# jerinphilip/whisper.tflite

Hardware: AMD Instinct MI355X
Metric: audio-sec/s (RTF) whisper-tiny 30s clips batch=32 at 1/2/4/8 MI355X (higher is better)
Workload: dtype f32 (operands as two fp16 planes, f16 MFMA, f32 accumulate); 1 GPU; whisper-tiny batch=32x30s synthetic mel U(-1,1.5), fp32, random-init weights (BASELINE.json configs[1]); mel resident in HBM -> token ids on host; clips_per_gpu=32, global_batch=32, decoder_positions=30, argmax_steps=27, parallelism=clip-parallel dp1, one RCCL all_gather of id records per 8 batches, pipelined=True, batches_in_flight=10, decoder=2 consecutive steps' batches share one decoder chain (dec_pair, dec_group), last_batches_announced=2, priming_batches=1

## Files before the change

include/wt_debug.h:

```cpp
#ifndef WT_DEBUG_H_
#define WT_DEBUG_H_
#include "wt_capi.h"
#ifdef __cplusplus
extern "C" {
#endif
int wt_dbg_gemm(wt_engine* h, int M, int N, int K, const float* A, const float* W, const float* bias,
                const float* R, const float* pos, int pos_period, int epi, float* C);
int wt_dbg_gemm_planes(wt_engine* h, int M, int N, int K, const float* A, const float* W, const float* bias,
                       const float* R, const float* pos, int pos_period, int epi, int planes_out, int iters, float* C,
                       float* avg_ms, int n_cu );
int wt_dbg_set_forced_ids(wt_engine* h, const int64_t* ids, int clips);
int wt_dbg_set_plane_gemm_mode(int mode);
int wt_dbg_gemm_planes_ln(wt_engine* h, int M, int K, const float* A, const float* W, const float* bias, const float* R,
                          const float* pos, int pos_period, int epi, const float* ln_g, const float* ln_b, int n_cu,
                          float* C, float* ln_out, float* ln_y32, int* fused);
int wt_dbg_encoder_attention_planes(wt_engine* h, int batch, int T, int heads, const float* qkv, int iters, float* out,
                                    float* avg_ms);
int wt_dbg_gemm_bench(wt_engine* h, int M, int N, int K, int epi, int variant, int iters, float* avg_ms);
int wt_dbg_interference(wt_engine* h, const float* d_mel, int batch, int n_enc, int chain_len, int blocks,
                        float* enc_ms, float* chain_ms);
int wt_dbg_concurrency(wt_engine* h, const float* d_mel, int batch, int n_dec, int n_enc, float* dec_ms,
                       float* enc_ms);
int wt_dbg_dec_gemm_bench(wt_engine* h, int kind, int B, int N, int K, int rows, int iters, float* avg_us);
int wt_dbg_dec_gemm(wt_engine* h, int mode, int B, int N, int K, const float* X, const float* W,
                    const float* bias, const float* R, float* Y, int64_t* argmax_out);
int wt_dbg_dec_ln_gemm(wt_engine* h, int B, int N, int K, const float* xin, const int64_t* ids, int pos,
                       const float* tok_emb, const float* pos_emb, int n_vocab, int n_pos,
                       const float* ln_g, const float* ln_b, const float* W, const float* bias,
                       int gelu, float* Y, float* xout);
int wt_dbg_layernorm(wt_engine* h, int M, int d, const float* x, const float* g, const float* b, float* y);
int wt_dbg_encoder_attention(wt_engine* h, int batch, int T, int heads, const float* qkv, float* out);
int wt_dbg_cross_attention(wt_engine* h, int batch, int heads, int T, int chunks, int nq, const float* x,
                           const float* ln_g, const float* ln_b, const float* wq, const float* bq, const float* kc,
                           const float* vc, float* out);
int wt_dbg_cross_absorbed(wt_engine* h, int batch, int heads, int T, int chunks, int nq, const float* qp, const float* E,
                          const float* wv, const float* bv, float* out, int iters, float* avg_us);
int wt_dbg_cross_absorbed_bf16(wt_engine* h, int batch, int heads, int T, int chunks, int nq, const float* qp, const float* E,
                               const float* wv, const float* bv, float* out, int iters, float* avg_us);
int wt_dbg_self_attention(wt_engine* h, int batch, int heads, int cap, int pos, int npos, const float* qkv,
                          float* kcache, float* vcache, float* out);
int wt_dbg_gemm_bf16(wt_engine* h, int M, int N, int K, const float* A, const float* W, const float* bias,
                     const float* R, const float* pos, int pos_period, int epi, int bf16_out, int iters, float* C,
                     float* avg_ms);
int wt_dbg_gemm_bf16_ln(wt_engine* h, int M, int N, int K, const float* A, const float* W, const float* bias, const float* R,
                        const float* ln_g, const float* ln_b, float* C, float* ln_out, float* ln_y32, int* fused);
int wt_dbg_encoder_attention_bf16(wt_engine* h, int batch, int T, int heads, const float* qkv, int iters, float* out,
                                  float* avg_ms);
int wt_dbg_dec_gemm_bf16(wt_engine* h, int mode, int B, int N, int K, const float* X, const float* W, const float* bias,
                         const float* R, float* Y, int64_t* argmax_out);
int wt_dbg_dec_ln_gemm_bf16(wt_engine* h, int B, int N, int K, const float* xin, const int64_t* ids, int pos,
                            const float* tok_emb, const float* pos_emb, int n_vocab, int n_pos, const float* ln_g,
                            const float* ln_b, const float* W, const float* bias, int gelu, float* Y, float* xout);
int wt_dbg_self_attention_bf16(wt_engine* h, int batch, int heads, int cap, int pos, int npos, const float* qkv,
                               float* kcache, float* vcache, float* out);
int wt_dbg_cross_attention_bf16(wt_engine* h, int batch, int heads, int T, int chunks, int nq, const float* x,
                                const float* ln_g, const float* ln_b, const float* wq, const float* bq, const float* kc,
                                const float* vc, float* out);
int wt_dbg_beam_topk(wt_engine* h, int rows, int V, int ldl, int kk, const float* logits, float* m, float* s,
                     uint64_t* keys);
int wt_dbg_beam_step(wt_engine* h, int K, int clips, int c0, int n_live, int pos, int n_prompt, int V, int64_t eot,
                     const float* logits, const int64_t* ids, float* live_sum, int32_t* fin_tok, float* fin_sum,
                     int32_t* fin_len, int32_t* n_fin, int32_t* done, int32_t* parent, int64_t* token, int64_t* ids_next);
int wt_dbg_beam_reorder(wt_engine* h, int src_rows, int dst_rows, int cap, int d, int slabs, int pos, int V,
                        const float* kv_src, float* kv_dst, const int64_t* ids_src, int64_t* ids_dst,
                        const int32_t* parent, const int64_t* token);
// ... 18 lines not shown
```

whisper.tflite_amd/__init__.py:

```python
from __future__ import annotations

import ctypes
import enum
import os
from ctypes import (POINTER, byref, c_char_p, c_float, c_int, c_int32, c_int64, c_long, c_size_t,
                    c_uint64, c_void_p)

import numpy as np

_HERE = os.path.dirname(os.path.abspath(__file__))
LIB_PATH = os.environ.get("WT_LIB_PATH") or os.path.join(_HERE, "lib", "libwhisper-tflite.so")

WT_OK = 0
WT_MAX_IDS = 32
WT_PIPELINE_DEPTH = 24
CHUNK_SAMPLES = 480000
STATUS_NAMES = {0: "WT_OK", 1: "WT_ERR_INVALID_ARG", 2: "WT_ERR_IO", 3: "WT_ERR_FORMAT",
                4: "WT_ERR_UNSUPPORTED", 5: "WT_ERR_DEVICE", 6: "WT_ERR_BUFFER"}

CAPI_SYMBOLS = [
    "wt_device_alloc", "wt_device_free", "wt_device_upload", "wt_device_download", "wt_device_synchronize",
    "wt_engine_create", "wt_engine_destroy", "wt_last_error", "wt_engine_dims",
    "wt_engine_set_option", "wt_engine_get_option", "wt_engine_set_prompt", "wt_transcribe_pcm", "wt_transcribe_long_pcm", "wt_transcribe_file",
    "wt_logmel_batch", "wt_logmel_batch_dev", "wt_encdec_tokens_batch",
    "wt_encdec_tokens_batch_dev", "wt_transcribe_tokens_batch_dev", "wt_pipeline_submit_dev", "wt_pipeline_submit_pcm_dev", "wt_pipeline_collect",
    "wt_encdec_debug_batch",
    "wt_last_timings", "wt_last_beam_scores", "wt_last_kernel_stats", "wt_decode_text", "wt_language_id", "wt_lang_code", "wt_wav_read_legacy",
    "wt_vocab_info", "wt_filters", "wt_write_synthetic_weights", "wt_write_synthetic_vocab",
    "wt_vocab_open", "wt_vocab_close", "wt_vocab_get_info", "wt_vocab_get_filters", "wt_vocab_size", "wt_vocab_token",
    "wt_vocab_decode", "wt_log_mel_spectrogram", "wt_convert_tflite", "wt_shutdown",
]
DEBUG_SYMBOLS = [
    "wt_dbg_cross_absorbed", "wt_dbg_cross_absorbed_bf16", "wt_dbg_gemm_planes_ln", "wt_dbg_gemm", "wt_dbg_gemm_bench", "wt_dbg_dec_gemm_bench", "wt_dbg_dec_gemm", "wt_dbg_dec_ln_gemm", "wt_dbg_layernorm", "wt_dbg_encoder_attention",
    "wt_dbg_cross_attention", "wt_dbg_self_attention", "wt_dbg_interference", "wt_dbg_concurrency",
    "wt_dbg_gemm_planes", "wt_dbg_set_plane_gemm_mode", "wt_dbg_set_forced_ids", "wt_dbg_dec_gemm_bf16", "wt_dbg_dec_ln_gemm_bf16",
    "wt_dbg_self_attention_bf16", "wt_dbg_cross_attention_bf16", "wt_dbg_encoder_attention_planes", "wt_dbg_gemm_bf16", "wt_dbg_gemm_bf16_ln", "wt_dbg_encoder_attention_bf16",
    "wt_dbg_beam_topk", "wt_dbg_beam_step", "wt_dbg_beam_reorder", "wt_dbg_beam_finalize",
    "wt_dbg_dec_gemm_ksplit", "wt_dbg_dec_ln_gemm_rows", "wt_dbg_dec_logits", "wt_dbg_select_token",
]


class WtError(RuntimeError):
    def __init__(self, code: int, message: str):
        super().__init__(f"{STATUS_NAMES.get(code, code)}: {message}")
        self.code = code


class EngineType(enum.IntEnum):
    Monolith = 0
    EncDec = 1


class Dims(ctypes.Structure):
    _fields_ = [(n, c_int32) for n in (
        "n_mels", "n_audio_ctx", "n_audio_state", "n_audio_head", "n_audio_layer",
        "n_vocab", "n_text_ctx", "n_text_state", "n_text_head", "n_text_layer")]


class Timings(ctypes.Structure):
    _fields_ = [("logmel_ms", c_float), ("encoder_ms", c_float), ("cross_kv_ms", c_float),
                ("decoder_ms", c_float), ("total_ms", c_float), ("batch", c_int32),
                ("decoder_steps", c_int32)]


class KernelStat(ctypes.Structure):
    _fields_ = [("name", ctypes.c_char * 48), ("launches", c_int32), ("reserved", c_int32),
                ("ms", ctypes.c_double), ("flops", ctypes.c_double), ("bytes", ctypes.c_double)]


_lib = None


def lib() -> ctypes.CDLL:
    global _lib
    if _lib is None:
        if not os.path.exists(LIB_PATH):
            raise ImportError(
                f"{LIB_PATH} is missing: build it with `make lib` (or __graft_entry__.build()); "
                "there is no Python/CPU fallback for the engine")
        L = ctypes.CDLL(LIB_PATH)
        fp, ip64, ip32 = POINTER(c_float), POINTER(c_int64), POINTER(c_int32)
        L.wt_engine_create.argtypes = [c_int, c_char_p, c_char_p, c_int, c_int, POINTER(c_void_p)]
        L.wt_engine_destroy.argtypes = [c_void_p]
        L.wt_engine_destroy.restype = None
        L.wt_last_error.argtypes = [c_void_p]
        L.wt_last_error.restype = c_char_p
        L.wt_engine_dims.argtypes = [c_void_p, POINTER(Dims)]
        L.wt_engine_set_option.argtypes = [c_void_p, c_char_p, c_long]
# ... 28 lines not shown
        L.wt_vocab_close.restype = None
        L.wt_vocab_get_info.argtypes = [c_void_p, ip32]
        L.wt_vocab_get_filters.argtypes = [c_void_p, fp, c_size_t, ip32, ip32]
        L.wt_vocab_size.argtypes = [c_void_p]
        L.wt_vocab_token.argtypes = [c_void_p, c_int, c_char_p, c_size_t, POINTER(c_size_t)]
        L.wt_vocab_decode.argtypes = [c_void_p, ip64, c_int, c_int, c_char_p, c_size_t, POINTER(c_size_t)]
        L.wt_log_mel_spectrogram.argtypes = [fp, c_int, fp, c_int, c_int, c_int, fp, c_size_t, POINTER(c_int)]
        L.wt_convert_tflite.argtypes = [c_char_p, c_char_p]
        L.wt_dbg_gemm.argtypes = [c_void_p, c_int, c_int, c_int, fp, fp, fp, fp, fp, c_int, c_int, fp]
        L.wt_dbg_gemm_planes.argtypes = [c_void_p, c_int, c_int, c_int, fp, fp, fp, fp, fp, c_int, c_int, c_int, c_int, fp,
                                         POINTER(c_float), c_int]
        L.wt_dbg_encoder_attention_planes.argtypes = [c_void_p, c_int, c_int, c_int, fp, c_int, fp, POINTER(c_float)]
        L.wt_dbg_cross_absorbed.argtypes = [c_void_p, c_int, c_int, c_int, c_int, c_int, fp, fp, fp, fp, fp, c_int, POINTER(c_float)]
        L.wt_dbg_cross_absorbed_bf16.argtypes = L.wt_dbg_cross_absorbed.argtypes
        L.wt_dbg_gemm_planes_ln.argtypes = [c_void_p, c_int, c_int, fp, fp, fp, fp, fp, c_int, c_int, fp, fp, c_int, fp, fp, fp,
                                            POINTER(c_int)]
        L.wt_dbg_gemm_bf16.argtypes = [c_void_p, c_int, c_int, c_int, fp, fp, fp, fp, fp, c_int, c_int, c_int, c_int, fp,
                                       POINTER(c_float)]
        L.wt_dbg_encoder_attention_bf16.argtypes = [c_void_p, c_int, c_int, c_int, fp, c_int, fp, POINTER(c_float)]
        L.wt_dbg_gemm_bf16_ln.argtypes = [c_void_p, c_int, c_int, c_int, fp, fp, fp, fp, fp, fp, fp, fp, fp, POINTER(c_int)]
        L.wt_dbg_gemm_bench.argtypes = [c_void_p, c_int, c_int, c_int, c_int, c_int, c_int, POINTER(c_float)]
        L.wt_dbg_dec_gemm_bench.argtypes = [c_void_p, c_int, c_int, c_int, c_int, c_int, c_int, POINTER(c_float)]
        L.wt_dbg_dec_gemm.argtypes = [c_void_p, c_int, c_int, c_int, c_int, fp, fp, fp, fp, fp, ip64]
        L.wt_dbg_dec_ln_gemm.argtypes = [c_void_p, c_int, c_int, c_int, fp, ip64, c_int, fp, fp,
                                         c_int, c_int, fp, fp, fp, fp, c_int, fp, fp]
        L.wt_dbg_layernorm.argtypes = [c_void_p, c_int, c_int, fp, fp, fp, fp]
        L.wt_device_alloc.argtypes = [c_void_p, ctypes.c_size_t, POINTER(c_void_p)]
        L.wt_device_free.argtypes = [c_void_p, c_void_p]
        L.wt_device_upload.argtypes = [c_void_p, c_void_p, ctypes.c_size_t, c_void_p, ctypes.c_size_t]
        L.wt_device_download.argtypes = [c_void_p, c_void_p, c_void_p, ctypes.c_size_t, ctypes.c_size_t]
        L.wt_device_synchronize.argtypes = [c_void_p]
        L.wt_dbg_set_forced_ids.argtypes = [c_void_p, POINTER(c_int64), c_int]
        L.wt_dbg_dec_gemm_bf16.argtypes = L.wt_dbg_dec_gemm.argtypes
        L.wt_dbg_dec_ln_gemm_bf16.argtypes = L.wt_dbg_dec_ln_gemm.argtypes
        L.wt_dbg_encoder_attention.argtypes = [c_void_p, c_int, c_int, c_int, fp, fp]
        L.wt_dbg_cross_attention.argtypes = [c_void_p, c_int, c_int, c_int, c_int, c_int, fp, fp, fp, fp, fp, fp, fp, fp]
        L.wt_dbg_self_attention.argtypes = [c_void_p, c_int, c_int, c_int, c_int, c_int, fp, fp, fp, fp]
        L.wt_dbg_self_attention_bf16.argtypes = L.wt_dbg_self_attention.argtypes
        L.wt_dbg_cross_attention_bf16.argtypes = L.wt_dbg_cross_attention.argtypes
        u64p = POINTER(c_uint64)
        L.wt_dbg_beam_topk.argtypes = [c_void_p, c_int, c_int, c_int, c_int, fp, fp, fp, u64p]
        L.wt_dbg_beam_step.argtypes = [c_void_p, c_int, c_int, c_int, c_int, c_int, c_int, c_int, c_int64, fp, ip64, fp, ip32,
                                       fp, ip32, ip32, ip32, ip32, ip64, ip64]
        L.wt_dbg_beam_reorder.argtypes = [c_void_p, c_int, c_int, c_int, c_int, c_int, c_int, c_int, fp, fp, ip64, ip64, ip32,
                                          ip64]
        L.wt_dbg_beam_finalize.argtypes = [c_void_p, c_int, c_int, c_int, c_int, c_int, ip64, fp, ip32, fp, ip32, ip32, ip32,
                                           ip64, ip32, fp, ip32]
        L.wt_dbg_dec_gemm_ksplit.argtypes = [c_void_p, c_int, c_int, c_int, c_int, c_int, fp, fp, fp, fp, fp, fp]
        L.wt_dbg_dec_ln_gemm_rows.argtypes = [c_void_p, c_int, c_int, c_int, c_int, c_int, fp, fp, ip64, c_int, c_int, fp, fp,
                                              c_int, c_int, fp, fp, fp, fp, c_int, fp, fp]
        L.wt_dbg_dec_logits.argtypes = [c_void_p, c_int, c_int, c_int, c_int, fp, fp, fp, fp, fp, c_int, fp, u64p]
        L.wt_dbg_select_token.argtypes = [c_void_p, c_int, c_int, u64p, ip64, c_int, c_int, ip32, ip32, c_int64, c_int,
                                          c_int]
        _lib = L
    return _lib


def _f32(a) -> np.ndarray:
    return np.ascontiguousarray(a, dtype=np.float32)


def _fp(a: np.ndarray):
    return a.ctypes.data_as(POINTER(c_float)) if a is not None else None


def _ip32(a: np.ndarray):
    if a.dtype != np.int32 or not a.flags.c_contiguous:
        raise ValueError("expected a contiguous int32 array")
    return a.ctypes.data_as(POINTER(c_int32))


def _ip64(a: np.ndarray):
    if a.dtype != np.int64 or not a.flags.c_contiguous:
        raise ValueError("expected a contiguous int64 array")
    return a.ctypes.data_as(POINTER(c_int64))


def write_synthetic_weights(path: str, arch: str = "tiny", seed: int = 0) -> None:
    rc = lib().wt_write_synthetic_weights(path.encode(), arch.encode(), seed)
    if rc != WT_OK:
        raise WtError(rc, lib().wt_last_error(None).decode())


def write_synthetic_vocab(path: str, n_tokens: int = 50257) -> None:
    rc = lib().wt_write_synthetic_vocab(path.encode(), n_tokens)
    if rc != WT_OK:
        raise WtError(rc, lib().wt_last_error(None).decode())


def language_id(code: str) -> int:
    return lib().wt_language_id(code.encode())


def lang_code(idx: int) -> str:
    return lib().wt_lang_code(idx).decode()


def wav_read_legacy(path: str) -> np.ndarray:
    n = c_size_t(0)
    rc = lib().wt_wav_read_legacy(path.encode(), None, 0, byref(n))
    if rc != WT_OK:
        return np.zeros(0, np.float32)
    out = np.zeros(n.value, np.float32)
    lib().wt_wav_read_legacy(path.encode(), _fp(out), out.size, byref(n))
    return out


class Vocab:

    INFO_KEYS = ("n_vocab", "eot", "sot", "translate", "transcribe", "prev", "solm", "not", "beg")

    def __init__(self, vocab_path: str, multilingual: bool = True):
        self._v = c_void_p()
        rc = lib().wt_vocab_open(os.fsencode(vocab_path), int(bool(multilingual)), byref(self._v))
        if rc != WT_OK:
            self._v = c_void_p()
            raise WtError(rc, lib().wt_last_error(None).decode())

    def close(self) -> None:
        if getattr(self, "_v", None) and self._v.value:
            lib().wt_vocab_close(self._v)
            self._v = c_void_p()

    def __del__(self):
        try:
            self.close()
        except Exception:
            pass
# ... 556 lines not shown
```

whisper.tflite_amd/csrc/capi.cpp:

```cpp
#include "wt_capi.h"

#include <hip/hip_runtime.h>

#include <functional>

#include <cstdio>
#include <cstdlib>
#include <sys/stat.h>
#include <unistd.h>
#include <cmath>
#include <cstring>
#include <memory>
#include <string>
#include <vector>

#include <mutex>

#include "engine.h"
#include "tflite_extract.h"
#include "weights_gen.h"
#include "wt_debug.h"
#include "kernels.h"

struct wt_engine {
// ... 740 lines not shown
}

int wt_write_synthetic_vocab(const char* path, int n_tokens) {
  if (!path || n_tokens < 0) return WT_ERR_INVALID_ARG;
  return guarded(nullptr, [&] {
    wt::write_vocab_file(path, wt::make_slaney_filterbank(80, 400, 16000), wt::make_synthetic_tokens(n_tokens));
  });
}


namespace {
struct DevBuf {
  float* p = nullptr;
  explicit DevBuf(size_t n) { hipchk(hipMalloc(reinterpret_cast<void**>(&p), std::max<size_t>(n, 1) * sizeof(float)), "hipMalloc"); }
  DevBuf(const float* host, size_t n) : DevBuf(n) {
    if (host && n) hipchk(hipMemcpy(p, host, n * sizeof(float), hipMemcpyHostToDevice), "H2D");
  }
  ~DevBuf() { (void)hipFree(p); }
  void to_host(float* host, size_t n) const { hipchk(hipMemcpy(host, p, n * sizeof(float), hipMemcpyDeviceToHost), "D2H"); }
};
}

namespace {
struct DevTiled {
  void* p = nullptr;
  float scale = 1.0f;
  DevTiled(const float* W, int N, int K, bool bf16 = false) {
    const std::vector<unsigned short> planes = bf16 ? wt::tile_weights_bf16(W, N, K) : wt::tile_weights_f16(W, N, K, &scale);
    hipchk(hipMalloc(&p, std::max<size_t>(planes.size(), 1) * 2), "hipMalloc");
    hipchk(hipMemcpy(p, planes.data(), planes.size() * 2, hipMemcpyHostToDevice), "H2D");
  }
  ~DevTiled() { (void)hipFree(p); }
  const unsigned short* w() const { return static_cast<const unsigned short*>(p); }
};
}

int wt_dbg_gemm(wt_engine* h, int M, int N, int K, const float* A, const float* W, const float* bias,
                const float* R, const float* pos, int pos_period, int epi, float* C) {
  if (!h || N % 128 || K % 32) return WT_ERR_INVALID_ARG;
  return guarded(h, [&] {
    DevBuf dA(A, size_t(M) * K), dW(W, size_t(N) * K), dB(bias, N), dC(R ? R : nullptr, size_t(M) * N),
        dP(pos, pos ? size_t(pos_period) * N : 0);
    wt::GemmArgs g;
    g.A = dA.p; g.lda = K; g.W = dW.p; g.bias = dB.p; g.C = dC.p; g.R = dC.p; g.ldc = N;
    g.pos = dP.p; g.pos_period = pos_period > 0 ? pos_period : 1;
    g.M = M; g.N = N; g.K = K; g.variant = int(h->impl->gemm_variant);
    wt::launch_gemm(g, epi, h->impl->stream());
    h->impl->sync();
    dC.to_host(C, size_t(M) * N);
  });
}

namespace {
struct DevPlanes {
  void* p = nullptr;
  long plane = 0;
  DevPlanes(const float* x, size_t n, float scale, size_t pad = 64) : plane(long(n + pad)) {
    std::vector<unsigned short> host(2 * (n + pad), 0);
    for (size_t i = 0; x && i < n; ++i) {
      const float v = x[i] * scale;
      const _Float16 hi = static_cast<_Float16>(v), lo = static_cast<_Float16>(v - static_cast<float>(hi));
      std::memcpy(&host[i], &hi, 2);
      std::memcpy(&host[n + pad + i], &lo, 2);
    }
    hipchk(hipMalloc(&p, host.size() * 2), "hipMalloc");
    hipchk(hipMemcpy(p, host.data(), host.size() * 2, hipMemcpyHostToDevice), "H2D");
  }
  ~DevPlanes() { (void)hipFree(p); }
  unsigned short* ptr() const { return static_cast<unsigned short*>(p); }
  void to_host(float* out, size_t n, float scale) const {
    std::vector<unsigned short> host(size_t(2) * plane);
    hipchk(hipMemcpy(host.data(), p, host.size() * 2, hipMemcpyDeviceToHost), "D2H");
    for (size_t i = 0; i < n; ++i) {
      _Float16 hi, lo;
      std::memcpy(&hi, &host[i], 2);
      std::memcpy(&lo, &host[size_t(plane) + i], 2);
      out[i] = (static_cast<float>(hi) + static_cast<float>(lo)) / scale;
    }
  }
};
struct DevWeightPlanes {
  void* p = nullptr;
  DevWeightPlanes(const float* W, int N, int K, float scale) {
    const std::vector<unsigned short> host = wt::split_weight_planes(W, N, K, K, scale);
    hipchk(hipMalloc(&p, host.size() * 2 + 256), "hipMalloc");
    hipchk(hipMemcpy(p, host.data(), host.size() * 2, hipMemcpyHostToDevice), "H2D");
  }
  ~DevWeightPlanes() { (void)hipFree(p); }
  unsigned short* ptr() const { return static_cast<unsigned short*>(p); }
};
float max_abs(const float* x, size_t n) {
  float m = 0.0f;
  for (size_t i = 0; i < n; ++i) m = std::max(m, std::fabs(x[i]));
  return m;
}
}

int wt_dbg_gemm_planes(wt_engine* h, int M, int N, int K, const float* A, const float* W, const float* bias,
                       const float* R, const float* pos, int pos_period, int epi, int planes_out, int iters, float* C,
                       float* avg_ms, int n_cu) {
  if (!h || !A || !W || !C || N % 128 || K % 32 || M < 1 || n_cu < 0) return WT_ERR_INVALID_ARG;
  return guarded(h, [&] {
    const float sa = wt::f16_scale_for(max_abs(A, size_t(M) * K)), sw = wt::f16_scale_for(max_abs(W, size_t(N) * K));
    const DevPlanes dA(A, size_t(M) * K, sa);
    const DevWeightPlanes dW(W, N, K, sw);
    DevBuf dB(bias, N), dC(R ? R : nullptr, size_t(M) * N), dP(pos, pos ? size_t(pos_period) * N : 0);
    const float out_bound = max_abs(A, size_t(M) * K) * max_abs(W, size_t(N) * K) * float(K) + (bias ? max_abs(bias, N) : 0.0f);
    const float so = wt::f16_scale_for(out_bound);
    DevPlanes dO(nullptr, size_t(M) * N, 1.0f);
    wt::PlaneGemmArgs g;
    g.A = dA.ptr(); g.a_plane = dA.plane; g.lda = K; g.W = dW.ptr(); g.bias = dB.p;
    g.C = dC.p; g.R = dC.p; g.ldc = N; g.pos = dP.p; g.pos_period = pos_period > 0 ? pos_period : 1;
    g.M = M; g.N = N; g.K = K; g.a_scale = sa; g.w_scale = sw; g.n_cu = n_cu;
    if (planes_out) { g.P = dO.ptr(); g.p_plane = dO.plane; g.out_scale[0] = so; }
    hipStream_t st = h->impl->stream();
    wt::launch_gemm_planes(g, epi, st);
    h->impl->sync();
    if (planes_out) dO.to_host(C, size_t(M) * N, so); else dC.to_host(C, size_t(M) * N);
    if (avg_ms && iters > 0) {
      hipEvent_t e0, e1;
      hipchk(hipEventCreate(&e0), "event");
      hipchk(hipEventCreate(&e1), "event");
      for (int i = 0; i < 3; ++i) wt::launch_gemm_planes(g, epi, st);
      hipchk(hipEventRecord(e0, st), "record");
      for (int i = 0; i < iters; ++i) wt::launch_gemm_planes(g, epi, st);
      hipchk(hipEventRecord(e1, st), "record");
      hipchk(hipEventSynchronize(e1), "sync");
      float ms = 0;
      hipchk(hipEventElapsedTime(&ms, e0, e1), "elapsed");
      *avg_ms = ms / iters;
      (void)hipEventDestroy(e0);
      (void)hipEventDestroy(e1);
    }
  });
}

int wt_dbg_set_forced_ids(wt_engine* h, const int64_t* ids, int clips) {
  if (!h || clips < 0 || clips > 4096 || (clips && !ids)) return WT_ERR_INVALID_ARG;
  return guarded(h, [&] {
    h->impl->forced_ids.assign(ids, ids + size_t(clips) * 32);
    for (long long v : h->impl->forced_ids)
      if (v < 0) throw wt::Error(wt::kErrInvalidArg, "forced ids must be token ids");
  });
}

int wt_dbg_set_plane_gemm_mode(int mode) {
  if (mode < 0 || mode > 4) return WT_ERR_INVALID_ARG;
  wt::set_plane_gemm_mode(mode);
  return WT_OK;
}

int wt_dbg_gemm_planes_ln(wt_engine* h, int M, int K, const float* A, const float* W, const float* bias, const float* R,
                          const float* pos, int pos_period, int epi, const float* ln_g, const float* ln_b, int n_cu,
                          float* C, float* ln_out, float* ln_y32, int* fused) {
  const int N = 384;
  if (!h || !A || !W || !C || !ln_g || !ln_b || !ln_out || !fused || K % 32 || M < 1 || n_cu < 0) return WT_ERR_INVALID_ARG;
  return guarded(h, [&] {
    const float sa = wt::f16_scale_for(max_abs(A, size_t(M) * K)), sw = wt::f16_scale_for(max_abs(W, size_t(N) * K));
    const DevPlanes dA(A, size_t(M) * K, sa);
    const DevWeightPlanes dW(W, N, K, sw);
    DevBuf dB(bias, N), dC(R ? R : nullptr, size_t(M) * N), dP(pos, pos ? size_t(pos_period) * N : 0), dG(ln_g, N), dS(ln_b, N),
        dY(size_t(M) * N), dF(1);
    hipchk(hipMemset(dF.p, 0, 4), "memset");
    const float so = 64.0f;
    DevPlanes dO(nullptr, size_t(M) * N, 1.0f);
    wt::PlaneGemmArgs g;
    g.A = dA.ptr(); g.a_plane = dA.plane; g.lda = K; g.W = dW.ptr(); g.bias = dB.p;
    g.C = dC.p; g.R = dC.p; g.ldc = N; g.pos = dP.p; g.pos_period = pos_period > 0 ? pos_period : 1;
    g.M = M; g.N = N; g.K = K; g.a_scale = sa; g.w_scale = sw; g.n_cu = n_cu;
    g.ln_g = dG.p; g.ln_b = dS.p; g.ln_P = dO.ptr(); g.ln_plane = dO.plane; g.ln_scale = so;
    g.ln_y32 = ln_y32 ? dY.p : nullptr; g.nonfinite = reinterpret_cast<int*>(dF.p);
    *fused = wt::launch_gemm_planes(g, epi, h->impl->stream()) ? 1 : 0;
    h->impl->sync();
    dC.to_host(C, size_t(M) * N);
    if (*fused) {
      dO.to_host(ln_out, size_t(M) * N, so);
      if (ln_y32) dY.to_host(ln_y32, size_t(M) * N);
    }
  });
}

int wt_dbg_encoder_attention_planes(wt_engine* h, int batch, int T, int heads, const float* qkv, int iters, float* out,
                                    float* avg_ms) {
  if (!h || !qkv || !out) return WT_ERR_INVALID_ARG;
  return guarded(h, [&] {
    const size_t d = size_t(heads) * 64, rows = size_t(batch) * T;
    float mq = 0.0f, mk = 0.0f, mv = 0.0f;
    for (size_t r = 0; r < rows; ++r) {
      const float* row = qkv + r * 3 * d;
      for (size_t c = 0; c < d; ++c) {
        mq = std::max(mq, std::fabs(row[c]));
        mk = std::max(mk, std::fabs(row[d + c]));
        mv = std::max(mv, std::fabs(row[2 * d + c]));
      }
    }
    constexpr float kQ = 0.125f * 1.44269504088896340736f;
    const float sq = wt::f16_scale_for(mq * kQ), sk = wt::f16_scale_for(mk), sv = wt::f16_scale_for(mv), so = wt::f16_scale_for(mv);
    std::vector<float> scaled(rows * 3 * d);
    for (size_t r = 0; r < rows; ++r)
      for (size_t c = 0; c < 3 * d; ++c)
        scaled[r * 3 * d + c] = qkv[r * 3 * d + c] * (c < d ? kQ * sq : c < 2 * d ? sk : sv);
    const DevPlanes dQ(scaled.data(), scaled.size(), 1.0f);
    DevPlanes dO(nullptr, rows * d, 1.0f);
    hipStream_t st = h->impl->stream();
    wt::launch_encoder_attention_planes(dQ.ptr(), dQ.plane, dO.ptr(), dO.plane, batch, T, heads, sq, sk, sv, so, st);
    h->impl->sync();
    dO.to_host(out, rows * d, so);
    if (avg_ms && iters > 0) {
      hipEvent_t e0, e1;
      hipchk(hipEventCreate(&e0), "event");
      hipchk(hipEventCreate(&e1), "event");
      hipchk(hipEventRecord(e0, st), "record");
      for (int i = 0; i < iters; ++i)
        wt::launch_encoder_attention_planes(dQ.ptr(), dQ.plane, dO.ptr(), dO.plane, batch, T, heads, sq, sk, sv, so, st);
      hipchk(hipEventRecord(e1, st), "record");
      hipchk(hipEventSynchronize(e1), "sync");
      float ms = 0;
      hipchk(hipEventElapsedTime(&ms, e0, e1), "elapsed");
      *avg_ms = ms / iters;
      (void)hipEventDestroy(e0);
      (void)hipEventDestroy(e1);
    }
  });
}

namespace {
struct DevBf16 {
  void* p = nullptr;
  size_t n = 0;
  static unsigned short rne(float f) {
    uint32_t u;
    std::memcpy(&u, &f, 4);
    if ((u & 0x7FFFFFFFu) > 0x7F800000u) return static_cast<unsigned short>((u >> 16) | 0x40u);
    u += 0x7FFFu + ((u >> 16) & 1u);
    return static_cast<unsigned short>(u >> 16);
  }
  DevBf16(const float* x, size_t n_, size_t pad = 256) : n(n_) {
    std::vector<unsigned short> host(n + pad, 0);
    for (size_t i = 0; x && i < n; ++i) host[i] = rne(x[i]);
    hipchk(hipMalloc(&p, host.size() * 2), "hipMalloc");
    hipchk(hipMemcpy(p, host.data(), host.size() * 2, hipMemcpyHostToDevice), "H2D");
  }
  ~DevBf16() { (void)hipFree(p); }
  unsigned short* ptr() const { return static_cast<unsigned short*>(p); }
  void to_host(float* out, size_t count) const {
    std::vector<unsigned short> host(count);
    hipchk(hipMemcpy(host.data(), p, count * 2, hipMemcpyDeviceToHost), "D2H");
    for (size_t i = 0; i < count; ++i) {
      const uint32_t u = uint32_t(host[i]) << 16;
      std::memcpy(&out[i], &u, 4);
    }
  }
};
float time_launches(hipStream_t st, int iters, const std::function<void()>& f) {
  hipEvent_t e0, e1;
  hipchk(hipEventCreate(&e0), "event");
  hipchk(hipEventCreate(&e1), "event");
  for (int i = 0; i < 3; ++i) f();
  hipchk(hipEventRecord(e0, st), "record");
  for (int i = 0; i < iters; ++i) f();
  hipchk(hipEventRecord(e1, st), "record");
  hipchk(hipEventSynchronize(e1), "sync");
  float ms = 0;
  hipchk(hipEventElapsedTime(&ms, e0, e1), "elapsed");
  (void)hipEventDestroy(e0);
  (void)hipEventDestroy(e1);
  return ms / iters;
// ... 673 lines not shown
```

whisper.tflite_amd/csrc/engine.cpp:

```cpp
#include "engine.h"

#include <fcntl.h>
#include <sys/mman.h>
#include <sys/stat.h>
#include <unistd.h>

#include <chrono>
#include <cmath>
#include <complex>
#include <cstdio>
#include <cstdlib>
#include <cstring>
#include <stdexcept>

#include "kernels.h"

namespace wt {

namespace {
void hip_check(hipError_t e, const char* what) {
  if (e != hipSuccess) {
    throw Error(5, std::string("HIP failure in ") + what + ": " + hipGetErrorString(e));
  }
}
// ... 1031 lines not shown
  for (auto& k : kstats_) k.launches = 0, k.ms = 0, k.flops = 0, k.bytes = 0;
  for (size_t i = 0; i < sl.kt_cls.size(); ++i) {
    float ms = 0;
    if (hipEventElapsedTime(&ms, sl.kt_events[2 * i], sl.kt_events[2 * i + 1]) != hipSuccess) continue;
    KernelStat& k = kstats_[sl.kt_cls[i]];
    k.launches += 1;
    k.ms += ms;
    k.flops += sl.kt_flops[i];
    k.bytes += sl.kt_bytes[i];
  }
}


void Engine::require_idle() const {
  if (!inflight_.empty()) throw Error(kErrInvalidArg, "collect the submitted batches before a synchronous call");
}

void Engine::encode(const float* d_mel, int batch) {
  require_idle();
  check_beam_call(false);
  select_stream(false);
  encode_enqueue(d_mel, batch);
}

void Engine::encode_enqueue(const float* d_mel, int batch) {
  if (dims_.n_audio_state == 0) throw Error(kErrUnsupported, "front-end-only engine: no model weights loaded");
  ensure_batch(batch);
  TimerDisarm disarm_on_exit;
  kt_on_ = kernel_timers > 0 && (enc_count_++ % kernel_timers) == 0;
  if (bf16) {
    encode_enqueue_bf16(d_mel, batch);
    return;
  }
  const wtw::Dims& c = dims_;
  const int T0 = mel_frames(), T = c.n_audio_ctx, d = c.n_audio_state, M = batch * T, nm = c.n_mels;
  const long Bw = ws_.batch;
  const int cus = (stream_ == stream_masked_ && stream_masked_) ? enc_cus_masked_ : n_cu_;
  Slot& slot = slots_[enc_slot_];
  if (slot.used) HIPCHK(hipStreamWaitEvent(stream_, slot.dec_done, 0));
  slot.kt_cls.clear();
  slot.kt_flops.clear();
  slot.kt_bytes.clear();
  slot.batch = batch;
  if (!trace_base_ && getenv("WT_TRACE_PIPELINE")) {
    HIPCHK(hipEventCreate(&trace_base_));
    HIPCHK(hipEventRecord(trace_base_, stream_));
  }
  HIPCHK(hipMemsetAsync(slot.d_flag, 0, sizeof(int), stream_));
  HIPCHK(hipEventRecord(slot.enc_begin, stream_));
  unsigned short* const lnp = reinterpret_cast<unsigned short*>(ws_.ln);
  unsigned short* const qkvp = reinterpret_cast<unsigned short*>(ws_.qkv);
  unsigned short* const attp = reinterpret_cast<unsigned short*>(ws_.att);
  unsigned short* const hidp = reinterpret_cast<unsigned short*>(ws_.hid);
  const long melT_plane = Bw * (T0 + 2) * nm + 128, h1p_plane = Bw * (T0 + 2) * d + 128;
  const long ln_plane = Bw * T * d, qkv_plane = Bw * T * 3 * d, hid_plane = Bw * T * 4 * d, cvt_plane = Bw * T * 4 * d;
  const long e_plane = Bw * T * d;
  const bool absorb = absorb_for(batch);
  const int alt = alt_gemm_variant();

  auto plane_gemm = [&](PlaneGemmArgs& g, const GemmScale& sc, int epi, double flops) {
    g.n_cu = cus; g.a_scale = sc.a; g.w_scale = sc.w;
    kt_begin(kKcGemm, flops, 0);
    const bool ln_fused = launch_gemm_planes(g, epi, stream_);
    kt_end();
    return ln_fused;
  };
  bool ln_done = false;
  static const bool no_ln_fuse = getenv("WT_NO_LN_FUSE") != nullptr;
  auto fuse_ln = [&](PlaneGemmArgs& g, const float* gain, const float* shift, float scale) {
    if (no_ln_fuse) return;
    g.ln_g = gain; g.ln_b = shift; g.ln_P = lnp; g.ln_plane = ln_plane; g.ln_scale = scale;
  };
  auto alt_gemm = [&](GemmArgs& g, const GemmScale& sc, int epi, double flops) {
    g.variant = alt; g.a_scale = sc.a; g.w_scale = sc.w;
    kt_begin(kKcGemmAlt, flops, 0);
    launch_gemm(g, epi, stream_);
    kt_end();
  };
  auto to_planes = [&](const float* src, unsigned short* dst, long plane, long rows, int ld, const float* scales, int seg) {
    kt_begin(kKcConvert, 0, 2.0 * rows * ld * 4);
    launch_f32_to_planes(src, dst, plane, rows, ld, scales, seg, stream_);
    kt_end();
  };

  const bool c1p = gemm_on_planes(sc_conv1_), c2p = gemm_on_planes(sc_conv2_);
  kt_begin(kKcTranspose, 0, 2.0 * batch * nm * T0 * 4);
  if (c1p) {
    launch_mel_transpose_planes(d_mel, ws_.melTp, melT_plane, sc_conv1_.a, batch, nm, T0, nm, stream_);
  } else {
    launch_mel_transpose(d_mel, ws_.melT, batch, nm, T0, stream_);
  }
  kt_end();
  if (c1p) {
    PlaneGemmArgs g;
    g.A = ws_.melTp; g.a_plane = melT_plane; g.a_rpb = T0; g.a_bs = long(T0 + 2) * nm; g.lda = nm;
    g.W = conv1_p_.w; g.bias = conv1_b;
    if (c2p) {
      g.P = ws_.h1pp + d; g.p_plane = h1p_plane; g.out_scale[0] = sc_conv2_.a;
    } else {
      g.C = ws_.h1p + d;
    }
    g.c_rpb = T0; g.c_bs = long(T0 + 2) * d; g.ldc = d;
    g.M = batch * T0; g.N = d; g.K = conv1_kpad_p_;
    plane_gemm(g, sc_conv1_, kEpiBias | kEpiGelu, 2.0 * g.M * g.N * (3.0 * nm));
  } else {
    GemmArgs g;
    g.A = ws_.melT; g.a_rpb = T0; g.a_bs = long(T0 + 2) * nm; g.lda = nm;
    g.W = conv1_w; g.bias = conv1_b;
    g.C = ws_.h1p + d; g.c_rpb = T0; g.c_bs = long(T0 + 2) * d; g.ldc = d;
    g.M = batch * T0; g.N = d; g.K = conv1_kpad;
    alt_gemm(g, sc_conv1_, kEpiBias | kEpiGelu, 2.0 * g.M * g.N * (3.0 * nm));
    if (c2p) to_planes(ws_.h1p, ws_.h1pp, h1p_plane, long(batch) * (T0 + 2), d, &sc_conv2_.a, 0);
  }
  if (c2p) {
    PlaneGemmArgs g;
    g.A = ws_.h1pp; g.a_plane = h1p_plane; g.a_rpb = T; g.a_bs = long(T0 + 2) * d; g.lda = 2 * d;
    g.W = conv2_p_.w; g.bias = conv2_b; g.pos = enc_pos; g.pos_period = T;
    g.C = ws_.x; g.ldc = d; g.M = M; g.N = d; g.K = 3 * d;
    if (gemm_on_planes(sc_layers_[0].qkv)) fuse_ln(g, enc_blocks_[0].attn_ln_g, enc_blocks_[0].attn_ln_b, sc_layers_[0].qkv.a);
    ln_done = plane_gemm(g, sc_conv2_, kEpiBias | kEpiGelu | kEpiPos, 2.0 * g.M * g.N * g.K);
  } else {
    GemmArgs g;
    g.A = ws_.h1p; g.a_rpb = T; g.a_bs = long(T0 + 2) * d; g.lda = 2 * d;
    g.W = conv2_w; g.bias = conv2_b; g.pos = enc_pos; g.pos_period = T;
    g.C = ws_.x; g.ldc = d; g.M = M; g.N = d; g.K = 3 * d;
    alt_gemm(g, sc_conv2_, kEpiBias | kEpiGelu | kEpiPos, 2.0 * g.M * g.N * g.K);
  }
  constexpr float kQScale = 0.125f * 1.44269504088896340736f;
  auto layernorm_for = [&](bool planes, float scale, const float* g, const float* b) {
    if (ln_done) {
      ln_done = false;
      return;
    }
    kt_begin(kKcLayerNorm, 0, 2.0 * M * d * 4);
    if (planes) {
      launch_layernorm_planes(ws_.x, lnp, ln_plane, scale, nullptr, g, b, M, d, stream_);
    } else {
      launch_layernorm(ws_.x, ws_.ln, g, b, M, d, stream_);
    }
    kt_end();
  };
  for (int l = 0; l < c.n_audio_layer; ++l) {
    const BlockWeights& w = enc_blocks_[l];
    const EncLayerPlanes& wp = enc_planes_[l];
    const EncLayerScales& sc = sc_layers_[l];
    const bool qp = gemm_on_planes(sc.qkv), op = gemm_on_planes(sc.out), f1p = gemm_on_planes(sc.fc1), f2p = gemm_on_planes(sc.fc2);
    const bool ap = gemm_variant < 0 && attn_variant == 4 && sc.attn_f16_ok && op;
    const int attn_alt = attn_variant == 4 ? 1 : int(attn_variant);

    layernorm_for(qp, sc.qkv.a, w.attn_ln_g, w.attn_ln_b);
    const float qkv_scales[3] = {kQScale * sc.q, sc.k, sc.v};
    const unsigned short* qkv_src = qkvp;
    long qkv_src_plane = qkv_plane;
    if (qp) {
      PlaneGemmArgs q;
      q.A = lnp; q.a_plane = ln_plane; q.lda = d; q.W = wp.qkv.w; q.bias = w.attn.bqkv;
      if (ap) {
        q.P = qkvp; q.p_plane = qkv_plane; q.seg = d;
        q.out_scale[0] = qkv_scales[0]; q.out_scale[1] = qkv_scales[1]; q.out_scale[2] = qkv_scales[2];
      } else {
        q.C = ws_.qkv;
      }
      q.ldc = 3 * d; q.M = M; q.N = 3 * d; q.K = d;
      plane_gemm(q, sc.qkv, kEpiBias, 2.0 * q.M * q.N * q.K);
    } else {
      GemmArgs q;
      q.A = ws_.ln; q.lda = d; q.W = w.attn.wqkv; q.bias = w.attn.bqkv; q.C = ws_.qkv; q.ldc = 3 * d;
      q.M = M; q.N = 3 * d; q.K = d;
      alt_gemm(q, sc.qkv, kEpiBias, 2.0 * q.M * q.N * q.K);
      if (ap) {
        to_planes(ws_.qkv, ws_.cvt, cvt_plane, M, 3 * d, qkv_scales, d);
        qkv_src = ws_.cvt; qkv_src_plane = cvt_plane;
      }
    }
    const unsigned short* att_src = attp;
    long att_src_plane = ln_plane;
    if (ap) {
      kt_begin(kKcEncAttn, 4.0 * batch * c.n_audio_head * double(T) * T * 64, 0);
      launch_encoder_attention_planes(qkv_src, qkv_src_plane, attp, ln_plane, batch, T, c.n_audio_head, sc.q, sc.k, sc.v,
                                      sc.out.a, stream_);
      kt_end();
    } else {
      kt_begin(kKcEncAttnAlt, 4.0 * batch * c.n_audio_head * double(T) * T * 64, 0);
      launch_encoder_attention(ws_.qkv, ws_.att, batch, T, c.n_audio_head, attn_alt, stream_);
      kt_end();
      if (op) {
        to_planes(ws_.att, ws_.cvt, cvt_plane, M, d, &sc.out.a, 0);
        att_src = ws_.cvt; att_src_plane = cvt_plane;
      }
    }
    if (op) {
      PlaneGemmArgs o;
      o.A = att_src; o.a_plane = att_src_plane; o.lda = d; o.W = wp.out.w; o.bias = w.attn.bo;
      o.C = ws_.x; o.R = ws_.x; o.ldc = d; o.M = M; o.N = d; o.K = d;
      if (f1p) fuse_ln(o, w.mlp_ln_g, w.mlp_ln_b, sc.fc1.a);
      ln_done = plane_gemm(o, sc.out, kEpiBias | kEpiResidual, 2.0 * o.M * o.N * o.K);
    } else {
      GemmArgs o;
      o.A = ws_.att; o.lda = d; o.W = w.attn.wo; o.bias = w.attn.bo; o.C = ws_.x; o.R = ws_.x; o.ldc = d;
      o.M = M; o.N = d; o.K = d;
      alt_gemm(o, sc.out, kEpiBias | kEpiResidual, 2.0 * o.M * o.N * o.K);
    }
    layernorm_for(f1p, sc.fc1.a, w.mlp_ln_g, w.mlp_ln_b);
    const unsigned short* hid_src = hidp;
    long hid_src_plane = hid_plane;
    if (f1p) {
      PlaneGemmArgs f1;
      f1.A = lnp; f1.a_plane = ln_plane; f1.lda = d; f1.W = wp.fc1.w; f1.bias = w.b1;
      if (f2p) {
        f1.P = hidp; f1.p_plane = hid_plane; f1.out_scale[0] = sc.fc2.a;
      } else {
        f1.C = ws_.hid;
      }
      f1.ldc = 4 * d; f1.M = M; f1.N = 4 * d; f1.K = d;
      plane_gemm(f1, sc.fc1, kEpiBias | kEpiGelu, 2.0 * f1.M * f1.N * f1.K);
    } else {
      GemmArgs f1;
      f1.A = ws_.ln; f1.lda = d; f1.W = w.w1; f1.bias = w.b1; f1.C = ws_.hid; f1.ldc = 4 * d;
      f1.M = M; f1.N = 4 * d; f1.K = d;
      alt_gemm(f1, sc.fc1, kEpiBias | kEpiGelu, 2.0 * f1.M * f1.N * f1.K);
      if (f2p) {
        to_planes(ws_.hid, ws_.cvt, cvt_plane, M, 4 * d, &sc.fc2.a, 0);
        hid_src = ws_.cvt; hid_src_plane = cvt_plane;
      }
    }
    if (f2p) {
      PlaneGemmArgs f2;
      f2.A = hid_src; f2.a_plane = hid_src_plane; f2.lda = 4 * d; f2.W = wp.fc2.w; f2.bias = w.b2;
      f2.C = ws_.x; f2.R = ws_.x; f2.ldc = d; f2.M = M; f2.N = d; f2.K = 4 * d;
      if (l + 1 < c.n_audio_layer) {
        if (gemm_on_planes(sc_layers_[l + 1].qkv)) fuse_ln(f2, enc_blocks_[l + 1].attn_ln_g, enc_blocks_[l + 1].attn_ln_b, sc_layers_[l + 1].qkv.a);
      } else if (gemm_on_planes(sc_cross_kv_)) {
        fuse_ln(f2, enc_ln_post_g, enc_ln_post_b, sc_cross_kv_.a);
        f2.ln_y32 = ws_.enc_out; f2.nonfinite = slot.d_flag;
        if (absorb && f2.ln_P) {
          f2.ln_P = slot.e_planes; f2.ln_plane = e_plane;
        }
        if (!f2.ln_P) f2.ln_y32 = nullptr, f2.nonfinite = nullptr;
      }
      ln_done = plane_gemm(f2, sc.fc2, kEpiBias | kEpiResidual, 2.0 * f2.M * f2.N * f2.K);
    } else {
      GemmArgs f2;
      f2.A = ws_.hid; f2.lda = 4 * d; f2.W = w.w2; f2.bias = w.b2; f2.C = ws_.x; f2.R = ws_.x; f2.ldc = d;
      f2.M = M; f2.N = d; f2.K = 4 * d;
      alt_gemm(f2, sc.fc2, kEpiBias | kEpiResidual, 2.0 * f2.M * f2.N * f2.K);
    }
  }
  const bool kp = gemm_on_planes(sc_cross_kv_);
  if (ln_done) {
    ln_done = false;
  } else {
    kt_begin(kKcLayerNorm, 0, 2.0 * M * d * 4);
    if (kp) {
      launch_layernorm_planes(ws_.x, absorb ? slot.e_planes : lnp, absorb ? e_plane : ln_plane, sc_cross_kv_.a, ws_.enc_out,
                              enc_ln_post_g, enc_ln_post_b, M, d, stream_, slot.d_flag);
    } else {
      launch_layernorm(ws_.x, ws_.enc_out, enc_ln_post_g, enc_ln_post_b, M, d, stream_, slot.d_flag);
    }
    kt_end();
  }
  HIPCHK(hipMemcpyAsync(slot.h_flag, slot.d_flag, sizeof(int), hipMemcpyDeviceToHost, stream_));
  HIPCHK(hipEventRecord(slot.enc_mid, stream_));
  slot.absorbed = absorb;
  if (absorb) {
  } else if (kp) {
    PlaneGemmArgs g;
    need_cross_kv(slot);
    g.A = lnp; g.a_plane = ln_plane; g.lda = d; g.W = cross_kv_p_.w; g.bias = cross_kv_b;
    g.C = slot.cross_kv; g.M = M; g.N = c.n_text_layer * 2 * d; g.K = d;
    g.c_rpb = T; g.kv_batch = batch; g.kv_heads = c.n_text_head; g.kv_dmodel = d;
    plane_gemm(g, sc_cross_kv_, kEpiBias | kEpiKvLayout, 2.0 * g.M * g.N * g.K);
  } else {
    GemmArgs g;
    need_cross_kv(slot);
    g.A = ws_.enc_out; g.lda = d; g.W = cross_kv_w; g.bias = cross_kv_b; g.C = slot.cross_kv;
    g.M = M; g.N = c.n_text_layer * 2 * d; g.K = d;
    g.c_rpb = T; g.kv_batch = batch; g.kv_heads = c.n_text_head; g.kv_dmodel = d;
    alt_gemm(g, sc_cross_kv_, kEpiBias | kEpiKvLayout, 2.0 * g.M * g.N * g.K);
  }
  HIPCHK(hipEventRecord(slot.enc_done, stream_));
  slot.used = true;
  last_enc_slot_ = enc_slot_;
  enc_slot_ = (enc_slot_ + 1) % kSlots;
}

void Engine::encode_enqueue_bf16(const float* d_mel, int batch) {
  const wtw::Dims& c = dims_;
  const int T0 = mel_frames(), T = c.n_audio_ctx, d = c.n_audio_state, M = batch * T, nm = c.n_mels;
  Slot& slot = slots_[enc_slot_];
  if (slot.used) HIPCHK(hipStreamWaitEvent(stream_, slot.dec_done, 0));
  slot.kt_cls.clear();
  slot.kt_flops.clear();
  slot.kt_bytes.clear();
  slot.batch = batch;
  HIPCHK(hipMemsetAsync(slot.d_flag, 0, sizeof(int), stream_));
  HIPCHK(hipEventRecord(slot.enc_begin, stream_));
  unsigned short* const lnp = reinterpret_cast<unsigned short*>(ws_.ln);
  unsigned short* const qkvp = reinterpret_cast<unsigned short*>(ws_.qkv);
  unsigned short* const attp = reinterpret_cast<unsigned short*>(ws_.att);
  unsigned short* const hidp = reinterpret_cast<unsigned short*>(ws_.hid);

  kt_begin(kKcTranspose, 0, 1.5 * batch * nm * T0 * 4);
  launch_mel_transpose_planes(d_mel, ws_.melTp, 0, 1.0f, batch, nm, T0, nm, stream_, true);
  kt_end();
  {
    PlaneGemmArgs g;
    g.A = ws_.melTp; g.a_rpb = T0; g.a_bs = long(T0 + 2) * nm; g.lda = nm;
    g.W = bf_.conv1; g.bias = conv1_b;
    g.P = ws_.h1pp + d;
    g.c_rpb = T0; g.c_bs = long(T0 + 2) * d; g.ldc = d;
    g.M = batch * T0; g.N = d; g.K = bf_.conv1_kpad;
    kt_begin(kKcGemm, 2.0 * g.M * g.N * (3.0 * nm), 0);
    launch_gemm_bf16_planes(g, kEpiBias | kEpiGelu, stream_);
    kt_end();
  }
  bool have_ln = false;
  {
    PlaneGemmArgs g;
    g.A = ws_.h1pp; g.a_rpb = T; g.a_bs = long(T0 + 2) * d; g.lda = 2 * d;
    g.W = bf_.conv2; g.bias = conv2_b; g.pos = enc_pos; g.pos_period = T;
    g.C = ws_.x; g.ldc = d;
// ... 786 lines not shown
```

whisper.tflite_amd/csrc/k_attention_planes.hip:

```cpp
#include <hip/hip_runtime.h>

#include <cstdlib>

#include "bf16_split.h"
#include "kernels.h"

namespace wt {
namespace {

using half8 = __attribute__((ext_vector_type(8))) _Float16;
using half4 = __attribute__((ext_vector_type(4))) _Float16;
using u32x4 = __attribute__((ext_vector_type(4))) unsigned;
typedef short i16x4 __attribute__((__vector_size__(4 * sizeof(short))));

constexpr int AK = 64;
constexpr int kPlaneBytes = AK * 128;

constexpr float kDefer = 3.0f;
constexpr float kPShift = 12.0f;


using f32x4 = __attribute__((ext_vector_type(4))) float;

template <bool BF>
__global__ __launch_bounds__(256, BF ? 4 : 3) void encoder_attention_planes(const _Float16* __restrict__ qkv, long plane,
                                                                     _Float16* __restrict__ out, long out_plane, int T,
                                                                     int heads, float s_inv, float o_scale) {
  constexpr int NP = BF ? 1 : 2;
  extern __shared__ __attribute__((aligned(16))) unsigned char lds[];
  constexpr int kVOff = 2 * NP * kPlaneBytes;
  using bf16x8 = __attribute__((ext_vector_type(8))) __bf16;

  const int d_model = heads * 64, ld = 3 * d_model;
  const int q_blocks = (T + 127) / 128;
  const int nb = gridDim.x, bid = blockIdx.x;
  const int q8 = nb >> 3, r8 = nb & 7, xcd = bid & 7;
  const int logical = (xcd < r8 ? xcd * (q8 + 1) : r8 * (q8 + 1) + (xcd - r8) * q8) + (bid >> 3);
  const int bh = logical / q_blocks, qb = logical % q_blocks;
  const int b = bh / heads, h = bh % heads;

  const int tid = threadIdx.x, lane = tid & 63, wid = __builtin_amdgcn_readfirstlane(tid >> 6);
  const int c = lane & 15, g = lane >> 4;
  const _Float16* base = qkv + (long)b * T * ld + h * 64;

  half8 qh[2][2], ql[2][2];
#pragma unroll
  for (int qa = 0; qa < 2; ++qa) {
    const int q_row = qb * 128 + wid * 32 + 16 * qa + c;
    const int q_ld = q_row < T ? q_row : T - 1;
#pragma unroll
    for (int ks = 0; ks < 2; ++ks) {
      qh[qa][ks] = *reinterpret_cast<const half8*>(base + (long)q_ld * ld + 32 * ks + 8 * g);
      if (!BF) ql[qa][ks] = *reinterpret_cast<const half8*>(base + plane + (long)q_ld * ld + 32 * ks + 8 * g);
    }
  }

  f32x4 o[4][2];
#pragma unroll
  for (int dg = 0; dg < 4; ++dg)
#pragma unroll
    for (int qa = 0; qa < 2; ++qa) o[dg][qa] = f32x4{0.0f, 0.0f, 0.0f, 0.0f};
  float m_run[2] = {0.0f, 0.0f}, l_run[2] = {0.0f, 0.0f};

  const int drow = 8 * wid + (lane >> 3);
  const int kch = (lane & 7) ^ ((drow >> 1) & 7);
  const int vch = (lane & 7) ^ (((drow >> 1) & 3) << 1);
  const unsigned row_b = 2u * (unsigned)ld;
  const unsigned offK0 = (unsigned)drow * row_b + 2u * (unsigned)(d_model + kch * 8), offK1 = offK0 + 32u * row_b;
  const unsigned offV0 = (unsigned)drow * row_b + 2u * (unsigned)(2 * d_model + vch * 8), offV1 = offV0 + 32u * row_b;
  const int last0 = ((T + AK - 1) / AK - 1) * AK;
  const unsigned c0r = (unsigned)((last0 + drow < T ? last0 + drow : T - 1) - last0);
  const unsigned c1r = (unsigned)((last0 + drow + 32 < T ? last0 + drow + 32 : T - 1) - last0);
  const unsigned offK0c = c0r * row_b + 2u * (unsigned)(d_model + kch * 8), offK1c = c1r * row_b + 2u * (unsigned)(d_model + kch * 8);
  const unsigned offV0c = c0r * row_b + 2u * (unsigned)(2 * d_model + vch * 8), offV1c = c1r * row_b + 2u * (unsigned)(2 * d_model + vch * 8);
  const unsigned lds0 = (unsigned)(size_t)(const __attribute__((address_space(3))) unsigned char*)lds;
  auto dma_tile = [&](const bool is_v, int kt, unsigned char* dst) {
    const unsigned long long sb = reinterpret_cast<unsigned long long>(base) + (unsigned long long)kt * (unsigned long long)(AK * 2) * (unsigned long long)ld;
    const unsigned d = lds0 + (unsigned)(dst - lds) + (unsigned)wid * 1024u;
    const bool lastp = kt * AK + AK > T;
#pragma unroll
// ... 126 lines not shown
          } else {
            split_f16x2(sp[2 * (e & 1)], sp[2 * (e & 1) + 1], &hh, &ll);
          }
          phu[e] = hh;
          plu[e] = ll;
        }
        ph[qa] = __builtin_bit_cast(half8, phu);
        pl[qa] = __builtin_bit_cast(half8, plu);
      }
#pragma unroll
      for (int dg = 0; dg < 4; ++dg) {
        half8 vh, vl;
#pragma unroll
        for (int hh2 = 0; hh2 < 2; ++hh2) {
          const unsigned char* r0 = vlane + (32 * kp + 16 * hh2) * 128 + (((2 * dg + vcp) ^ vsw) << 4);
          const i16x4 a0 = __builtin_amdgcn_ds_read_tr16_b64_v4i16((__attribute__((address_space(3))) i16x4*)(r0));
          const half4 a0h = __builtin_bit_cast(half4, a0);
#pragma unroll
          for (int e = 0; e < 4; ++e) vh[4 * hh2 + e] = a0h[e];
          if constexpr (!BF) {
            const i16x4 a1 = __builtin_amdgcn_ds_read_tr16_b64_v4i16((__attribute__((address_space(3))) i16x4*)(r0 + kPlaneBytes));
            const half4 a1h = __builtin_bit_cast(half4, a1);
#pragma unroll
            for (int e = 0; e < 4; ++e) vl[4 * hh2 + e] = a1h[e];
          }
        }
#pragma unroll
        for (int qa = 0; qa < 2; ++qa) {
          if constexpr (BF) {
            o[dg][qa] = __builtin_amdgcn_mfma_f32_16x16x32_bf16(__builtin_bit_cast(bf16x8, vh), __builtin_bit_cast(bf16x8, ph[qa]), o[dg][qa], 0, 0, 0);
          } else {
            o[dg][qa] = __builtin_amdgcn_mfma_f32_16x16x32_f16(vh, pl[qa], o[dg][qa], 0, 0, 0);
            o[dg][qa] = __builtin_amdgcn_mfma_f32_16x16x32_f16(vl, ph[qa], o[dg][qa], 0, 0, 0);
            o[dg][qa] = __builtin_amdgcn_mfma_f32_16x16x32_f16(vh, ph[qa], o[dg][qa], 0, 0, 0);
          }
        }
      }
    }
    asm volatile("s_waitcnt lgkmcnt(0)" ::: "memory");
    __builtin_amdgcn_s_barrier();
    __builtin_amdgcn_sched_barrier(0);
    if (kt + 1 < n_tiles) dma_tile(true, kt + 1, lds + kVOff);
    if (kt + 2 < n_tiles) dma_tile(false, kt + 2, lds + (kt & 1) * NP * kPlaneBytes);
  }

#pragma unroll
  for (int qa = 0; qa < 2; ++qa) {
    float l = l_run[qa];
    l += __shfl_xor(l, 16, 64);
    l += __shfl_xor(l, 32, 64);
    const int q_row = qb * 128 + wid * 32 + 16 * qa + c;
    if (q_row < T) {
      const float inv = o_scale / l;
      _Float16* orow = out + ((long)b * T + q_row) * d_model + h * 64;
      using u32x2 = __attribute__((ext_vector_type(2))) unsigned;
#pragma unroll
      for (int dg = 0; dg < 4; ++dg) {
        unsigned ah[2], al[2] = {0, 0};
#pragma unroll
        for (int j = 0; j < 2; ++j) {
          if constexpr (BF) {
            ah[j] = pack_bf16x2(o[dg][qa][2 * j] * inv, o[dg][qa][2 * j + 1] * inv);
          } else {
            split_f16x2(o[dg][qa][2 * j] * inv, o[dg][qa][2 * j + 1] * inv, &ah[j], &al[j]);
          }
        }
        *reinterpret_cast<u32x2*>(orow + 16 * dg + 4 * g) = u32x2{ah[0], ah[1]};
        if constexpr (!BF) *reinterpret_cast<u32x2*>(orow + out_plane + 16 * dg + 4 * g) = u32x2{al[0], al[1]};
      }
    }
  }
}

}

void launch_encoder_attention_planes(const unsigned short* qkv, long plane, unsigned short* out, long out_plane,
                                     int batch, int T, int heads, float q_scale, float k_scale, float v_scale,
                                     float out_scale, hipStream_t stream) {
  if (batch < 1 || T < 1 || heads < 1 || (3 * heads * 64) % 8 != 0) throw Error(kErrInvalidArg, "encoder attention: bad shape");
  const int q_blocks = (T + 127) / 128;
  WT_LAUNCH_TIMED(encoder_attention_planes<false>, dim3(batch * heads * q_blocks), dim3(256), 6 * kPlaneBytes, stream,
                     reinterpret_cast<const _Float16*>(qkv), plane, reinterpret_cast<_Float16*>(out), out_plane, T, heads,
                     1.0f / (q_scale * k_scale), out_scale / v_scale);
}

void launch_encoder_attention_bf16(const unsigned short* qkv, unsigned short* out, int batch, int T, int heads,
                                   hipStream_t stream) {
  if (batch < 1 || T < 1 || heads < 1) throw Error(kErrInvalidArg, "encoder attention: bad shape");
  const int q_blocks = (T + 127) / 128;
  WT_LAUNCH_TIMED(encoder_attention_planes<true>, dim3(batch * heads * q_blocks), dim3(256), 3 * kPlaneBytes, stream,
                     reinterpret_cast<const _Float16*>(qkv), 0L, reinterpret_cast<_Float16*>(out), 0L, T, heads,
                     0.125f * 1.44269504088896340736f, 1.0f);
}

}
```

whisper.tflite_amd/csrc/k_gemm_planes.hip:

```cpp
#include <hip/hip_runtime.h>

#include <algorithm>
#include <cstdlib>
#include <cstring>
#include <type_traits>

#include "bf16_split.h"
#include "kernels.h"

namespace wt {

static int g_plane_gemm_mode = -1;
int plane_gemm_mode() {
  if (g_plane_gemm_mode < 0) {
    const char* v = getenv("WT_PLANE_GEMM_MODE");
    g_plane_gemm_mode = v ? atoi(v) : 2;
  }
  return g_plane_gemm_mode;
}
void set_plane_gemm_mode(int m) { g_plane_gemm_mode = m; }

namespace {

using f32x16 = __attribute__((ext_vector_type(16))) float;
using f32x4 = __attribute__((ext_vector_type(4))) float;
using half8 = __attribute__((ext_vector_type(8))) _Float16;
using half4 = __attribute__((ext_vector_type(4))) _Float16;
using u32x4 = __attribute__((ext_vector_type(4))) unsigned;

constexpr int BK = 32;

struct PlaneGemmDev {
  const _Float16* A;
  long a_plane;
  const _Float16* W;
  float* C;
  _Float16* P;
  long p_plane;
  const float* bias;
  const float* R;
  const float* pos;
  int M, N, K;
  int a_rpb;
  long a_bs;
  int lda;
  int c_rpb;
  long c_bs;
  int ldc;
  int pos_period;
  int kv_batch, kv_heads, kv_dmodel;
  float descale;
  float out_scale[3];
  int seg;
  const float* ln_g;
  const float* ln_b;
  _Float16* ln_P;
  long ln_plane;
  float ln_scale;
  float* ln_y32;
  int* nonfinite;
};

__host__ __device__ __forceinline__ constexpr int chunk_swizzle(int row) { return (0 - (row >> 2)) & 3; }

template <int QA, int QW, int NW, int QPW>
__device__ __forceinline__ void setup_stage_dma(const PlaneGemmDev& g, int m0, int n0, int wid, int lane, unsigned (&voff)[QPW],
                                                const unsigned char* (&ubase)[QPW], unsigned (&kstep)[QPW]) {
  const int srow = lane >> 2;
  const int nkt = g.K / BK;
#pragma unroll
  for (int j = 0; j < QPW; ++j) {
    const int q = wid + NW * j;
    if (q < 2 * QA) {
      const bool lo = q >= QA;
      const int row = 16 * (lo ? q - QA : q) + srow;
      const int chunk = (lane & 3) ^ chunk_swizzle(row);
      int m = m0 + row;
      m = m < g.M ? m : g.M - 1;
      voff[j] = (unsigned)(2 * ((lo ? g.a_plane : 0) + (long)(m / g.a_rpb) * g.a_bs + (long)(m % g.a_rpb) * g.lda + chunk * 8));
      ubase[j] = reinterpret_cast<const unsigned char*>(g.A);
      kstep[j] = BK * 2;
    } else {
      const int wq = q - 2 * QA;
      const int rg = wq % QW, plane = wq / QW;
      voff[j] = (unsigned)(lane * 16);
      ubase[j] = reinterpret_cast<const unsigned char*>(g.W) + ((size_t)(n0 / 16 + rg) * nkt * 2 + plane) * 1024;
      kstep[j] = 2048;
    }
  }
}

template <int MI_, int NI_>
struct Acc32 {
  static constexpr int MI = MI_, NI = NI_;
  f32x16 t[MI_][NI_];
  __device__ __forceinline__ void zero() {
#pragma unroll
    for (int i = 0; i < MI_; ++i)
#pragma unroll
      for (int j = 0; j < NI_; ++j)
#pragma unroll
        for (int r = 0; r < 16; ++r) t[i][j][r] = 0.0f;
  }
  __device__ __forceinline__ float get(int mi, int ni, int i) const { return t[mi][ni][i]; }
  __device__ __forceinline__ void set(int mi, int ni, int i, float v) { t[mi][ni][i] = v; }
  __device__ __forceinline__ void stage_write(int mi, int ni, float* stage, int lane, float scale) const {
    const int l31 = lane & 31, lh = lane >> 5;
#pragma unroll
    for (int r = 0; r < 16; ++r) stage[((r & 3) + 8 * (r >> 2) + 4 * lh) * 32 + (l31 ^ (lh * 20))] = t[mi][ni][r] * scale;
  }
};
template <int MI_, int NI_>
struct Acc16 {
  static constexpr int MI = MI_, NI = NI_;
  f32x4 t[2 * MI_][2 * NI_];
  __device__ __forceinline__ void zero() {
#pragma unroll
    for (int i = 0; i < 2 * MI_; ++i)
#pragma unroll
      for (int j = 0; j < 2 * NI_; ++j)
#pragma unroll
        for (int r = 0; r < 4; ++r) t[i][j][r] = 0.0f;
  }
  __device__ __forceinline__ float get(int mi, int ni, int i) const { return t[2 * mi + (i >> 3)][2 * ni + ((i >> 2) & 1)][i & 3]; }
  __device__ __forceinline__ void set(int mi, int ni, int i, float v) { t[2 * mi + (i >> 3)][2 * ni + ((i >> 2) & 1)][i & 3] = v; }
  __device__ __forceinline__ void stage_write(int mi, int ni, float* stage, int lane, float scale) const {
// ... 41 lines not shown
    for (int ni = 0; ni < NI; ++ni)
#pragma unroll
      for (int e = 0; e < CPL; e += 4)
        asm volatile("" : "+v"(bias_all[ni][e]), "+v"(bias_all[ni][e + 1]), "+v"(bias_all[ni][e + 2]), "+v"(bias_all[ni][e + 3]));
    hook();
  }
#pragma unroll
  for (int ni = 0; ni < NI; ++ni) {
    const int n = n0 + (wn * NI + ni) * 32 + c0;
    float bias_v[CPL];
#pragma unroll
    for (int e = 0; e < CPL; ++e) bias_v[e] = bias_all[ni][e];
    const float oscale = PLANES_OUT ? g.out_scale[n / g.seg] : 1.0f;
    const int slab = (EPI & kEpiKvLayout) ? n / g.kv_dmodel : 0, rem = (EPI & kEpiKvLayout) ? n % g.kv_dmodel : 0;
    const int head = rem >> 6, dd = rem & 63;
#pragma unroll
    for (int mi = 0; mi < MI; ++mi) {
      acc.stage_write(mi, ni, stage, lane, g.descale);
      const int mbase = m0 + wm * (32 * MI) + mi * 32;
      const int mb0 = mbase / g.c_rpb, mt0 = mbase % g.c_rpb;
      const int mp0 = (EPI & kEpiPos) ? mbase % g.pos_period : 0;
#pragma unroll
      for (int p = 0; p < 32 / RPS; ++p) {
        const int row = p * RPS + prow;
        float v[CPL];
#pragma unroll
        for (int e = 0; e < CPL; e += 4) {
          const f32x4 t = *reinterpret_cast<const f32x4*>(&stage[row * SLD + ((c0 + e) ^ (((row >> 2) & 1) * 20))]);
          v[e] = t[0], v[e + 1] = t[1], v[e + 2] = t[2], v[e + 3] = t[3];
        }
        if (mbase + row < g.M) {
          int mb = mb0, mt = mt0 + row;
          if (mt >= g.c_rpb) mt -= g.c_rpb, mb += 1;
#pragma unroll
          for (int e = 0; e < CPL; e += 2) {
            v[e] += bias_v[e];
            v[e + 1] += bias_v[e + 1];
            if (EPI & kEpiGelu) {
              const f32x2_t gl = gelu_erf2(f32x2_t{v[e], v[e + 1]});
              v[e] = gl[0];
              v[e + 1] = gl[1];
            }
          }
          if (EPI & kEpiPos) {
            int mp = mp0 + row;
            if (mp >= g.pos_period) mp -= g.pos_period;
#pragma unroll
            for (int e = 0; e < CPL; e += 4) {
              const f32x4 t = *reinterpret_cast<const f32x4*>(g.pos + (long)mp * g.N + n + e);
              v[e] += t[0], v[e + 1] += t[1], v[e + 2] += t[2], v[e + 3] += t[3];
            }
          }
          if (PLANES_OUT) {
            const long o = (long)mb * g.c_bs + (long)mt * g.ldc + n;
            u32x4 hi, lo;
#pragma unroll
            for (int e = 0; e < CPL; e += 2) {
              unsigned h, l;
              split_f16x2(v[e] * oscale, v[e + 1] * oscale, &h, &l);
              hi[e / 2] = h;
              lo[e / 2] = l;
            }
            *reinterpret_cast<u32x4*>(g.P + o) = hi;
            *reinterpret_cast<u32x4*>(g.P + g.p_plane + o) = lo;
          } else if (EPI & kEpiKvLayout) {
            const long o = (((long)slab * g.kv_batch + mb) * g.kv_heads + head) * (long)g.c_rpb * 64 + (long)mt * 64 + dd;
            __builtin_nontemporal_store(f32x4{v[0], v[1], v[2], v[3]}, reinterpret_cast<f32x4*>(g.C + o));
          } else if constexpr ((EPI & kEpiPower) != 0) {
            using f32x2 = __attribute__((ext_vector_type(2))) float;
            const long o = (long)mb * g.c_bs + (long)mt * g.ldc + (n >> 1);
            *reinterpret_cast<f32x2*>(g.C + o) = f32x2{v[0] * v[0] + v[1] * v[1], v[2] * v[2] + v[3] * v[3]};
          } else {
            const long o = (long)mb * g.c_bs + (long)mt * g.ldc + n;
            f32x4 out = {v[0], v[1], v[2], v[3]};
            if (EPI & kEpiResidual) out += *reinterpret_cast<const f32x4*>(g.R + o);
            *reinterpret_cast<f32x4*>(g.C + o) = out;
            if constexpr (LN) {
#pragma unroll
              for (int e = 0; e < 4; ++e) acc.set(mi, ni, 4 * p + e, out[e]);
            }
          }
        } else if constexpr (LN) {
#pragma unroll
          for (int e = 0; e < 4; ++e) acc.set(mi, ni, 4 * p + e, 0.0f);
        }
      }
    }
  }
  if constexpr (LN) {
    float* const part = reinterpret_cast<float*>(smem) + NW * (32 * SLD);
    const int rbase = wm * (32 * MI) + prow;
    float mean[MI][4], rstd[MI][4];
#pragma unroll
    for (int pass = 0; pass < 2; ++pass) {
#pragma unroll
      for (int mi = 0; mi < MI; ++mi)
#pragma unroll
        for (int p = 0; p < 4; ++p) {
          float t = 0.0f;
#pragma unroll
          for (int ni = 0; ni < NI; ++ni)
#pragma unroll
            for (int e = 0; e < 4; ++e) {
              const float x = acc.get(mi, ni, 4 * p + e) - (pass ? mean[mi][p] : 0.0f);
              t += pass ? x * x : x;
            }
          t += __shfl_xor(t, 1, 64);
          t += __shfl_xor(t, 2, 64);
          t += __shfl_xor(t, 4, 64);
          if ((lane & 7) == 0) part[pass * (BM * 4) + (rbase + mi * 32 + p * 8) * 4 + wn] = t;
        }
      __syncthreads();
#pragma unroll
      for (int mi = 0; mi < MI; ++mi)
#pragma unroll
        for (int p = 0; p < 4; ++p) {
          const f32x4 q = *reinterpret_cast<const f32x4*>(&part[pass * (BM * 4) + (rbase + mi * 32 + p * 8) * 4]);
          const float tot = ((q[0] + q[1]) + (q[2] + q[3])) * (1.0f / (float)BN);
          if (pass == 0) {
            mean[mi][p] = tot;
          } else {
            if (g.nonfinite != nullptr && (lane & 7) == 0 && wn == 0 && !(fabsf(mean[mi][p]) <= 3.0e38f && tot <= 3.0e38f)) atomicOr(g.nonfinite, 1);
            rstd[mi][p] = rsqrtf(tot + 1e-5f);
          }
        }
    }
#pragma unroll
    for (int ni = 0; ni < NI; ++ni) {
      const int n = n0 + (wn * NI + ni) * 32 + c0;
      const f32x4 gg = *reinterpret_cast<const f32x4*>(g.ln_g + n), bb = *reinterpret_cast<const f32x4*>(g.ln_b + n);
#pragma unroll
      for (int mi = 0; mi < MI; ++mi)
#pragma unroll
        for (int p = 0; p < 4; ++p) {
          const int m = m0 + rbase + mi * 32 + p * 8;
          if (m >= g.M) continue;
          f32x4 y;
#pragma unroll
          for (int e = 0; e < 4; ++e) y[e] = (acc.get(mi, ni, 4 * p + e) - mean[mi][p]) * rstd[mi][p] * gg[e] + bb[e];
          const long o = (long)m * BN + n;
          if (g.ln_y32 != nullptr) __builtin_nontemporal_store(y, reinterpret_cast<f32x4*>(g.ln_y32 + o));
          unsigned h0, l0, h1, l1;
          split_f16x2(y[0] * g.ln_scale, y[1] * g.ln_scale, &h0, &l0);
          split_f16x2(y[2] * g.ln_scale, y[3] * g.ln_scale, &h1, &l1);
          using u32x2 = __attribute__((ext_vector_type(2))) unsigned;
          *reinterpret_cast<u32x2*>(g.ln_P + o) = u32x2{h0, h1};
          *reinterpret_cast<u32x2*>(g.ln_P + g.ln_plane + o) = u32x2{l0, l1};
        }
    }
  }
}

template <int EPI, bool PLANES_OUT, int WN, int NI, int MI, bool LN = false>
__global__ __launch_bounds__(128 * WN, WN == 2 ? 2 : 2) void gemm_planes_tile(PlaneGemmDev g) {
  static_assert(!LN || (!PLANES_OUT && WN == 4 && NI == 3), "LayerNorm fusion: fp32 output, 384-column tile");
  constexpr int BN = WN * NI * 32, NW = 2 * WN, BM = 64 * MI;
  constexpr int kAPlane = BM * BK * 2, kWPlane = BN * BK * 2;
  constexpr int kStage = 2 * kAPlane + 2 * kWPlane;
  constexpr int QA = BM / 16, QW = BN / 16;
  constexpr int QT = 2 * QA + 2 * QW, QPW = QT / NW;
  static_assert(QT % NW == 0, "whole instructions per wavefront");
  extern __shared__ __attribute__((aligned(16))) unsigned char smem[];

  const int nb = gridDim.x, bid = blockIdx.x;
  const int q8 = nb >> 3, r8 = nb & 7, xcd = bid & 7;
  const int logical = (xcd < r8 ? xcd * (q8 + 1) : r8 * (q8 + 1) + (xcd - r8) * q8) + (bid >> 3);
  const int n_tiles = g.N / BN;
  const int m0 = (logical / n_tiles) * BM;
  const int n0 = (logical % n_tiles) * BN;

  const int tid = threadIdx.x;
  const int lane = tid & 63, wid = __builtin_amdgcn_readfirstlane(tid >> 6);
  const int wm = wid / WN, wn = wid % WN;
  const int l31 = lane & 31, lh = lane >> 5;

  unsigned voff[QPW], kstep[QPW];
  const unsigned char* ubase[QPW];
  const unsigned lds_base = (unsigned)(size_t)(const __attribute__((address_space(3))) unsigned char*)smem;
  setup_stage_dma<QA, QW, NW, QPW>(g, m0, n0, wid, lane, voff, ubase, kstep);
  auto issue_stage = [&](int kt, int buf) {
#pragma unroll
    for (int j = 0; j < QPW; ++j) {
      const unsigned long long sb = reinterpret_cast<unsigned long long>(ubase[j]) + (size_t)kt * kstep[j];
      const unsigned dst = lds_base + (unsigned)(buf * kStage + (wid + NW * j) * 1024);
      lds_dma16_sgpr(voff[j], sb, dst);
    }
  };

  Acc32<MI, NI> accs;
  accs.zero();
  auto& acc = accs.t;

  const int swz = chunk_swizzle(l31);
  const int a_off = (wm * (32 * MI) + l31) * 64, b_off = 2 * kAPlane + (wn * NI * 32 + l31) * 64;
  auto compute = [&](int buf) {
    const unsigned char* base = smem + buf * kStage;
#pragma unroll
    for (int ks = 0; ks < BK / 16; ++ks) {
      const int slot = ((ks * 2 + lh) ^ swz) * 16;
      half8 ah[MI], al[MI], bh[NI], bl[NI];
#pragma unroll
      for (int i = 0; i < MI; ++i) {
        ah[i] = *reinterpret_cast<const half8*>(base + a_off + i * 32 * 64 + slot);
        al[i] = *reinterpret_cast<const half8*>(base + kAPlane + a_off + i * 32 * 64 + slot);
      }
#pragma unroll
      for (int j = 0; j < NI; ++j) {
        bh[j] = *reinterpret_cast<const half8*>(base + b_off + j * 32 * 64 + slot);
        bl[j] = *reinterpret_cast<const half8*>(base + kWPlane + b_off + j * 32 * 64 + slot);
      }
#pragma unroll
      for (int i = 0; i < MI; ++i)
#pragma unroll
        for (int j = 0; j < NI; ++j) acc[i][j] = __builtin_amdgcn_mfma_f32_32x32x16_f16(ah[i], bl[j], acc[i][j], 0, 0, 0);
#pragma unroll
      for (int i = 0; i < MI; ++i)
#pragma unroll
        for (int j = 0; j < NI; ++j) acc[i][j] = __builtin_amdgcn_mfma_f32_32x32x16_f16(al[i], bh[j], acc[i][j], 0, 0, 0);
#pragma unroll
      for (int i = 0; i < MI; ++i)
#pragma unroll
        for (int j = 0; j < NI; ++j) acc[i][j] = __builtin_amdgcn_mfma_f32_32x32x16_f16(ah[i], bh[j], acc[i][j], 0, 0, 0);
    }
  };

  const int nkt = g.K / BK;
  issue_stage(0, 0);
  for (int kt = 0; kt < nkt; ++kt) {
    asm volatile("s_waitcnt vmcnt(0)" ::: "memory");
    __builtin_amdgcn_s_barrier();
    if (kt + 1 < nkt) issue_stage(kt + 1, (kt + 1) & 1);
    compute(kt & 1);
  }
  planes_epilogue<EPI, PLANES_OUT, WN, LN>(g, accs, smem, m0, n0, wid, wm, wn, lane);
}

#ifdef WT_PP_STAMPS
__device__ long long g_pp_stamps[1024 * 8 * 9];
#define PP_STAMP(i)                                  \
  do {                                               \
    const long long t_ = __builtin_readcyclecounter(); \
    st_[i] += t_ - tl_;                              \
    tl_ = t_;                                        \
  } while (0)
#else
#define PP_STAMP(i) \
  do {              \
  } while (0)
#endif

template <int EPI, bool PLANES_OUT, int MI, bool LN = false>
__global__ __launch_bounds__(512, 2) void gemm_planes_pp(PlaneGemmDev g) {
  constexpr int WN = 4, NI = 3;
  static_assert(!LN || !PLANES_OUT, "LayerNorm fusion: fp32 output");
  constexpr int BN = WN * NI * 32, NW = 2 * WN, BM = 64 * MI;
  constexpr int kAPlane = BM * BK * 2, kWPlane = BN * BK * 2;
  constexpr int kStage = 2 * kAPlane + 2 * kWPlane;
  constexpr int QA = BM / 16, QW = BN / 16;
  constexpr int QT = 2 * QA + 2 * QW, QPW = QT / NW;
  static_assert(QT % NW == 0, "whole instructions per wavefront");
#ifdef WT_PP_STAMPS
  const long long t_kernel_ = __builtin_readcyclecounter();
  const long long r_kernel_ = (long long)__builtin_amdgcn_s_memrealtime();
#endif
  extern __shared__ __attribute__((aligned(16))) unsigned char smem[];

  const int nb = gridDim.x, bid = blockIdx.x;
  const int q8 = nb >> 3, r8 = nb & 7, xcd = bid & 7;
  const int logical = (xcd < r8 ? xcd * (q8 + 1) : r8 * (q8 + 1) + (xcd - r8) * q8) + (bid >> 3);
  const int n_tiles = g.N / BN;
  const int m0 = (logical / n_tiles) * BM;
  const int n0 = (logical % n_tiles) * BN;

  const int tid = threadIdx.x;
  const int lane = tid & 63, wid = __builtin_amdgcn_readfirstlane(tid >> 6);
  const int wm = wid / WN, wn = wid % WN;
  const int l31 = lane & 31, lh = lane >> 5;

  unsigned voff[QPW], kstep[QPW];
  const unsigned char* ubase[QPW];
  const unsigned lds_base = (unsigned)(size_t)(const __attribute__((address_space(3))) unsigned char*)smem;
  setup_stage_dma<QA, QW, NW, QPW>(g, m0, n0, wid, lane, voff, ubase, kstep);
  auto issue_stage = [&](int kt, int buf) {
#pragma unroll
    for (int j = 0; j < QPW; ++j) {
      const unsigned long long sb = reinterpret_cast<unsigned long long>(ubase[j]) + (size_t)kt * kstep[j];
      const unsigned dst = lds_base + (unsigned)(buf * kStage + (wid + NW * j) * 1024);
      lds_dma16_sgpr(voff[j], sb, dst);
    }
  };

  Acc32<MI, NI> accs;
  accs.zero();
  auto& acc = accs.t;

  const int swz = chunk_swizzle(l31);
  const int a_off = (wm * (32 * MI) + l31) * 64, b_off = 2 * kAPlane + (wn * NI * 32 + l31) * 64;
  half8 ah[MI], al[MI], bh[NI], bl[NI];
  auto load_frags = [&](int buf, int ks) {
    const unsigned char* base = smem + buf * kStage;
    const int slot = ((ks * 2 + lh) ^ swz) * 16;
#pragma unroll
    for (int i = 0; i < MI; ++i) {
      ah[i] = *reinterpret_cast<const half8*>(base + a_off + i * 32 * 64 + slot);
      al[i] = *reinterpret_cast<const half8*>(base + kAPlane + a_off + i * 32 * 64 + slot);
    }
#pragma unroll
    for (int j = 0; j < NI; ++j) {
      bh[j] = *reinterpret_cast<const half8*>(base + b_off + j * 32 * 64 + slot);
      bl[j] = *reinterpret_cast<const half8*>(base + kWPlane + b_off + j * 32 * 64 + slot);
    }
  };
  auto compute = [&]() {
#pragma unroll
    for (int i = 0; i < MI; ++i)
#pragma unroll
      for (int j = 0; j < NI; ++j) acc[i][j] = __builtin_amdgcn_mfma_f32_32x32x16_f16(ah[i], bl[j], acc[i][j], 0, 0, 0);
#pragma unroll
    for (int i = 0; i < MI; ++i)
#pragma unroll
      for (int j = 0; j < NI; ++j) acc[i][j] = __builtin_amdgcn_mfma_f32_32x32x16_f16(al[i], bh[j], acc[i][j], 0, 0, 0);
#pragma unroll
    for (int i = 0; i < MI; ++i)
#pragma unroll
      for (int j = 0; j < NI; ++j) acc[i][j] = __builtin_amdgcn_mfma_f32_32x32x16_f16(ah[i], bh[j], acc[i][j], 0, 0, 0);
  };
  auto phase_end = [&]() {
    __builtin_amdgcn_sched_barrier(0);
    __builtin_amdgcn_s_barrier();
    __builtin_amdgcn_sched_barrier(0);
  };
  auto reads_done = [&]() { asm volatile("s_waitcnt lgkmcnt(0)" ::: "memory"); };
  auto dma_done = [&]() { asm volatile("s_waitcnt vmcnt(0)" ::: "memory"); };

  const int nkt = g.K / BK;
  issue_stage(0, 0);
  if (nkt > 1) {
    issue_stage(1, 1);
    asm volatile("s_waitcnt vmcnt(%0)" ::"n"(QPW) : "memory");
  } else {
    dma_done();
  }
  phase_end();
  if (wm == 1) phase_end();
  load_frags(0, 0);
  reads_done();
  phase_end();
#ifdef WT_PP_STAMPS
  long long st_[9] = {0, 0, 0, 0, 0, 0, 0, 0, 0};
  long long tl_ = __builtin_readcyclecounter();
  const long long t_begin_ = tl_;
  st_[5] = tl_ - t_kernel_;
#endif
  for (int kt = 0; kt < nkt; ++kt) {
    compute();
    phase_end();
    PP_STAMP(0);
    load_frags(kt & 1, 1);
    reads_done();
    if (wm == 1) dma_done();
    phase_end();
    PP_STAMP(1);
    compute();
    if (wm == 0) dma_done();
    phase_end();
    PP_STAMP(2);
    if (kt + 1 < nkt) {
      if (kt + 2 < nkt) issue_stage(kt + 2, kt & 1);
      load_frags((kt + 1) & 1, 0);
      reads_done();
    }
    phase_end();
    PP_STAMP(3);
  }
  if (wm == 0) phase_end();
#ifdef WT_PP_STAMPS
  const long long t_loop_end_ = __builtin_readcyclecounter();
  st_[4] = t_loop_end_ - t_begin_;
#endif
  planes_epilogue<EPI, PLANES_OUT, WN, LN>(g, accs, smem, m0, n0, wid, wm, wn, lane);
#ifdef WT_PP_STAMPS
  {
    const long long t_end_ = __builtin_readcyclecounter();
    st_[6] = t_end_ - t_loop_end_;
    st_[7] = t_end_ - t_kernel_;
    st_[8] = (long long)__builtin_amdgcn_s_memrealtime() - r_kernel_;
    if (lane == 0 && blockIdx.x < 1024)
      for (int i = 0; i < 9; ++i) g_pp_stamps[(blockIdx.x * 8 + wid) * 9 + i] = st_[i];
  }
#endif
}

template <int EPI, bool PLANES_OUT, bool LN = false>
__global__ __launch_bounds__(512, 2) void gemm_planes_pp16(PlaneGemmDev g) {
  constexpr int WN = 4, NI = 3, MI = 3;
  static_assert(!LN || !PLANES_OUT, "LayerNorm fusion: fp32 output");
  constexpr int BN = WN * NI * 32, NW = 2 * WN, BM = 64 * MI;
  constexpr int kAPlane = BM * BK * 2, kWPlane = BN * BK * 2;
  constexpr int kStage = 2 * kAPlane + 2 * kWPlane;
  constexpr int QA = BM / 16, QW = BN / 16;
  constexpr int QT = 2 * QA + 2 * QW, QPW = QT / NW;
  static_assert(QT % NW == 0, "whole instructions per wavefront");
#ifdef WT_PP_STAMPS
  const long long t_kernel_ = __builtin_readcyclecounter();
  const long long r_kernel_ = (long long)__builtin_amdgcn_s_memrealtime();
#endif
  extern __shared__ __attribute__((aligned(16))) unsigned char smem[];

  const int nb = gridDim.x, bid = blockIdx.x;
  const int q8 = nb >> 3, r8 = nb & 7, xcd = bid & 7;
  const int logical = (xcd < r8 ? xcd * (q8 + 1) : r8 * (q8 + 1) + (xcd - r8) * q8) + (bid >> 3);
  const int n_tiles = g.N / BN;
  const int m0 = (logical / n_tiles) * BM;
  const int n0 = (logical % n_tiles) * BN;

  const int tid = threadIdx.x;
  const int lane = tid & 63, wid = __builtin_amdgcn_readfirstlane(tid >> 6);
  const int wm = wid / WN, wn = wid % WN;

  unsigned voff[QPW], kstep[QPW];
  const unsigned char* ubase[QPW];
  const unsigned lds_base = (unsigned)(size_t)(const __attribute__((address_space(3))) unsigned char*)smem;
  setup_stage_dma<QA, QW, NW, QPW>(g, m0, n0, wid, lane, voff, ubase, kstep);
  auto issue_stage = [&](int kt, int buf) {
#pragma unroll
    for (int j = 0; j < QPW; ++j) {
      const unsigned long long sb = reinterpret_cast<unsigned long long>(ubase[j]) + (size_t)kt * kstep[j];
      const unsigned dst = lds_base + (unsigned)(buf * kStage + (wid + NW * j) * 1024);
      lds_dma16_sgpr(voff[j], sb, dst);
    }
  };

  Acc16<MI, NI> accs;
  accs.zero();
  auto& acc = accs.t;

  const int fc = lane & 15, fq = lane >> 4;
  const int frag = fc * 64 + ((fq ^ chunk_swizzle(fc)) * 16);
  const int a_off = wm * (32 * MI) * 64 + frag, b_off = 2 * kAPlane + wn * (NI * 32) * 64 + frag;
  half8 ah[3], al[3], bh[6], bl[6];
  auto load_b = [&](int buf) {
    const unsigned char* base = smem + buf * kStage + b_off;
#pragma unroll
    for (int j = 0; j < 6; ++j) {
      bh[j] = *reinterpret_cast<const half8*>(base + j * 1024);
      bl[j] = *reinterpret_cast<const half8*>(base + kWPlane + j * 1024);
    }
  };
  auto load_a = [&](int buf, int half) {
    const unsigned char* base = smem + buf * kStage + a_off + half * 3 * 1024;
#pragma unroll
    for (int i = 0; i < 3; ++i) {
      ah[i] = *reinterpret_cast<const half8*>(base + i * 1024);
      al[i] = *reinterpret_cast<const half8*>(base + kAPlane + i * 1024);
    }
  };
  auto compute = [&](auto half_c) {
    constexpr int H = decltype(half_c)::value;
#pragma unroll
    for (int i = 0; i < 3; ++i)
#pragma unroll
      for (int j = 0; j < 6; ++j) acc[3 * H + i][j] = __builtin_amdgcn_mfma_f32_16x16x32_f16(ah[i], bl[j], acc[3 * H + i][j], 0, 0, 0);
#pragma unroll
    for (int i = 0; i < 3; ++i)
#pragma unroll
      for (int j = 0; j < 6; ++j) acc[3 * H + i][j] = __builtin_amdgcn_mfma_f32_16x16x32_f16(al[i], bh[j], acc[3 * H + i][j], 0, 0, 0);
#pragma unroll
    for (int i = 0; i < 3; ++i)
#pragma unroll
      for (int j = 0; j < 6; ++j) acc[3 * H + i][j] = __builtin_amdgcn_mfma_f32_16x16x32_f16(ah[i], bh[j], acc[3 * H + i][j], 0, 0, 0);
  };
  using H0 = std::integral_constant<int, 0>;
  using H1 = std::integral_constant<int, 1>;
  auto phase_end = [&]() {
    __builtin_amdgcn_sched_barrier(0);
    __builtin_amdgcn_s_barrier();
    __builtin_amdgcn_sched_barrier(0);
  };
  auto reads_done = [&]() { asm volatile("s_waitcnt lgkmcnt(0)" ::: "memory"); };
  auto dma_done = [&]() { asm volatile("s_waitcnt vmcnt(0)" ::: "memory"); };

  const int nkt = g.K / BK;
  issue_stage(0, 0);
  if (nkt > 1) {
    issue_stage(1, 1);
    asm volatile("s_waitcnt vmcnt(%0)" ::"n"(QPW) : "memory");
  } else {
    dma_done();
  }
  phase_end();
  if (wm == 1) phase_end();
  load_b(0);
  load_a(0, 0);
  reads_done();
  phase_end();
#ifdef WT_PP_STAMPS
  long long st_[9] = {0, 0, 0, 0, 0, 0, 0, 0, 0};
  long long tl_ = __builtin_readcyclecounter();
  const long long t_begin_ = tl_;
  st_[5] = tl_ - t_kernel_;
#endif
  for (int kt = 0; kt < nkt; ++kt) {
    compute(H0{});
    phase_end();
    PP_STAMP(0);
    load_a(kt & 1, 1);
    reads_done();
    if (wm == 1) dma_done();
    phase_end();
    PP_STAMP(1);
    compute(H1{});
    if (wm == 0) dma_done();
    phase_end();
    PP_STAMP(2);
    if (kt + 1 < nkt) {
      if (kt + 2 < nkt) issue_stage(kt + 2, kt & 1);
      load_b((kt + 1) & 1);
      load_a((kt + 1) & 1, 0);
      reads_done();
    }
    phase_end();
    PP_STAMP(3);
  }
  if (wm == 0) phase_end();
#ifdef WT_PP_STAMPS
  const long long t_loop_end_ = __builtin_readcyclecounter();
  st_[4] = t_loop_end_ - t_begin_;
#endif
  planes_epilogue<EPI, PLANES_OUT, WN, LN>(g, accs, smem, m0, n0, wid, wm, wn, lane);
#ifdef WT_PP_STAMPS
  {
    const long long t_end_ = __builtin_readcyclecounter();
    st_[6] = t_end_ - t_loop_end_;
    st_[7] = t_end_ - t_kernel_;
    st_[8] = (long long)__builtin_amdgcn_s_memrealtime() - r_kernel_;
    if (lane == 0 && blockIdx.x < 1024)
      for (int i = 0; i < 9; ++i) g_pp_stamps[(blockIdx.x * 8 + wid) * 9 + i] = st_[i];
  }
#endif
}

template <int EPI>
__global__ __launch_bounds__(512, 2) void gemm_planes_pp16_persist(PlaneGemmDev g, int total_tiles) {
  constexpr int WN = 4, NI = 3, MI = 3;
  constexpr bool PLANES_OUT = true;
  static_assert((EPI & ~(kEpiBias | kEpiGelu)) == 0, "bias / GELU epilogues with plane output");
  constexpr int BN = WN * NI * 32, NW = 2 * WN, BM = 64 * MI;
  constexpr int kAPlane = BM * BK * 2, kWPlane = BN * BK * 2;
  constexpr int kStage = 2 * kAPlane + 2 * kWPlane;
  constexpr int QA = BM / 16, QW = BN / 16;
  constexpr int QT = 2 * QA + 2 * QW, QPW = QT / NW;
  constexpr int kEpiStores = MI * NI * 4;
  extern __shared__ __attribute__((aligned(16))) unsigned char smem[];

  const int grid = gridDim.x, bid = blockIdx.x;
  const int q8 = total_tiles >> 3, r8 = total_tiles & 7;
  const int n_tiles = g.N / BN;
  const int tid = threadIdx.x;
  const int lane = tid & 63, wid = __builtin_amdgcn_readfirstlane(tid >> 6);
  const int wm = wid / WN, wn = wid % WN;

  unsigned voff[QPW], kstep[QPW];
  const unsigned char* ubase[QPW];
  const unsigned lds_base = (unsigned)(size_t)(const __attribute__((address_space(3))) unsigned char*)smem;
  int m0 = 0, n0 = 0;
  auto set_tile = [&](int vid) {
    const int xcd = vid & 7;
    const int logical = (xcd < r8 ? xcd * (q8 + 1) : r8 * (q8 + 1) + (xcd - r8) * q8) + (vid >> 3);
    m0 = (logical / n_tiles) * BM;
    n0 = (logical % n_tiles) * BN;
    setup_stage_dma<QA, QW, NW, QPW>(g, m0, n0, wid, lane, voff, ubase, kstep);
  };
  auto issue_stage = [&](int kt) {
    const int buf = (kt + 1) & 1;
#pragma unroll
    for (int j = 0; j < QPW; ++j) {
      const unsigned long long sb = reinterpret_cast<unsigned long long>(ubase[j]) + (size_t)kt * kstep[j];
      lds_dma16_sgpr(voff[j], sb, lds_base + (unsigned)(buf * kStage + (wid + NW * j) * 1024));
    }
  };

  Acc16<MI, NI> accs;
  auto& acc = accs.t;
  const int fc = lane & 15, fq = lane >> 4;
  const int frag = fc * 64 + ((fq ^ chunk_swizzle(fc)) * 16);
  const int a_off = wm * (32 * MI) * 64 + frag, b_off = 2 * kAPlane + wn * (NI * 32) * 64 + frag;
  half8 ah[3], al[3], bh[6], bl[6];
  auto load_b = [&](int kt) {
    const unsigned char* base = smem + ((kt + 1) & 1) * kStage + b_off;
#pragma unroll
    for (int j = 0; j < 6; ++j) {
      bh[j] = *reinterpret_cast<const half8*>(base + j * 1024);
      bl[j] = *reinterpret_cast<const half8*>(base + kWPlane + j * 1024);
    }
  };
  auto load_a = [&](int kt, int half) {
    const unsigned char* base = smem + ((kt + 1) & 1) * kStage + a_off + half * 3 * 1024;
#pragma unroll
    for (int i = 0; i < 3; ++i) {
      ah[i] = *reinterpret_cast<const half8*>(base + i * 1024);
      al[i] = *reinterpret_cast<const half8*>(base + kAPlane + i * 1024);
    }
  };
  auto compute = [&](auto half_c) {
    constexpr int H = decltype(half_c)::value;
#pragma unroll
    for (int i = 0; i < 3; ++i)
#pragma unroll
      for (int j = 0; j < 6; ++j) acc[3 * H + i][j] = __builtin_amdgcn_mfma_f32_16x16x32_f16(ah[i], bl[j], acc[3 * H + i][j], 0, 0, 0);
#pragma unroll
    for (int i = 0; i < 3; ++i)
#pragma unroll
      for (int j = 0; j < 6; ++j) acc[3 * H + i][j] = __builtin_amdgcn_mfma_f32_16x16x32_f16(al[i], bh[j], acc[3 * H + i][j], 0, 0, 0);
#pragma unroll
    for (int i = 0; i < 3; ++i)
#pragma unroll
      for (int j = 0; j < 6; ++j) acc[3 * H + i][j] = __builtin_amdgcn_mfma_f32_16x16x32_f16(ah[i], bh[j], acc[3 * H + i][j], 0, 0, 0);
  };
  using H0 = std::integral_constant<int, 0>;
  using H1 = std::integral_constant<int, 1>;
  auto phase_end = [&]() {
    __builtin_amdgcn_sched_barrier(0);
    __builtin_amdgcn_s_barrier();
    __builtin_amdgcn_sched_barrier(0);
  };
  auto reads_done = [&]() { asm volatile("s_waitcnt lgkmcnt(0)" ::: "memory"); };
  auto dma_done = [&]() { asm volatile("s_waitcnt vmcnt(0)" ::: "memory"); };

  const int nkt = g.K / BK;
  int vid = bid;
  set_tile(vid);
  issue_stage(0);
  issue_stage(1);
  asm volatile("s_waitcnt vmcnt(%0)" ::"n"(QPW) : "memory");
  phase_end();
  for (;;) {
    if (wm == 1) phase_end();
    accs.zero();
    load_b(0);
    load_a(0, 0);
    reads_done();
    phase_end();
    for (int kt = 0; kt < nkt; ++kt) {
      compute(H0{});
      phase_end();
      load_a(kt, 1);
      reads_done();
      if (wm == 1) dma_done();
      phase_end();
      compute(H1{});
      if (wm == 0) dma_done();
      phase_end();
      if (kt + 1 < nkt) {
        if (kt + 2 < nkt) issue_stage(kt + 2);
        load_b(kt + 1);
        load_a(kt + 1, 0);
        reads_done();
      }
      phase_end();
    }
    if (wm == 0) phase_end();
    const int m_cur = m0, n_cur = n0;
    const int next = vid + grid;
    const bool has_next = next < total_tiles;
    const bool whole = m_cur + BM <= g.M;
    auto prefetch = [&]() {
      if (has_next) {
        set_tile(next);
        issue_stage(0);
      }
    };
    planes_epilogue<EPI, PLANES_OUT, WN, false>(g, accs, smem, m_cur, n_cur, wid, wm, wn, lane, ActiveEpilogueHook<decltype(prefetch)>{prefetch});
    if (!has_next) break;
    if (whole) {
      asm volatile("s_waitcnt vmcnt(%0)" ::"n"(kEpiStores) : "memory");
    } else {
      dma_done();
    }
    phase_end();
    issue_stage(1);
    vid = next;
  }
}

template <int EPI, bool PLANES_OUT, int WN, int NI, int MI = 3, bool LN = false>
void launch_planes_shape(const PlaneGemmDev& g, hipStream_t s, int n_cu = 0) {
  constexpr int BN = WN * NI * 32, BM = 64 * MI;
  const int blocks = ((g.M + BM - 1) / BM) * (g.N / BN);
  constexpr size_t smem = 2 * (2 * BM * BK * 2 + 2 * BN * BK * 2);
  static const bool raised = [] {
    (void)hipFuncSetAttribute(reinterpret_cast<const void*>(&gemm_planes_tile<EPI, PLANES_OUT, WN, NI, MI, LN>),
                              hipFuncAttributeMaxDynamicSharedMemorySize, 160 * 1024);
    return true;
  }();
  (void)raised;
  if constexpr (WN == 4 && NI == 3 && MI == 3) {
    if constexpr (PLANES_OUT && !LN && (EPI & ~(kEpiBias | kEpiGelu)) == 0) {
      const int cu = n_cu > 0 ? n_cu : 256;
      if (plane_gemm_mode() == 2 && cu % 8 == 0 && blocks >= 2 * cu && (g.K / BK) % 2 == 0 && g.K / BK >= 4) {
        static const bool raised_p = [] {
          (void)hipFuncSetAttribute(reinterpret_cast<const void*>(&gemm_planes_pp16_persist<EPI>), hipFuncAttributeMaxDynamicSharedMemorySize,
                                    160 * 1024);
          return true;
        }();
        (void)raised_p;
        WT_LAUNCH_TIMED((gemm_planes_pp16_persist<EPI>), dim3(cu), dim3(512), smem, s, g, blocks);
        return;
      }
    }
    if (plane_gemm_mode() == 2 || plane_gemm_mode() == 4) {
      static const bool raised_pp16 = [] {
        (void)hipFuncSetAttribute(reinterpret_cast<const void*>(&gemm_planes_pp16<EPI, PLANES_OUT, LN>),
                                  hipFuncAttributeMaxDynamicSharedMemorySize, 160 * 1024);
        return true;
      }();
      (void)raised_pp16;
      WT_LAUNCH_TIMED((gemm_planes_pp16<EPI, PLANES_OUT, LN>), dim3(blocks), dim3(512), smem, s, g);
      return;
    }
    if (plane_gemm_mode() == 1) {
      static const bool raised_pp = [] {
        (void)hipFuncSetAttribute(reinterpret_cast<const void*>(&gemm_planes_pp<EPI, PLANES_OUT, MI, LN>),
                                  hipFuncAttributeMaxDynamicSharedMemorySize, 160 * 1024);
        return true;
      }();
      (void)raised_pp;
      WT_LAUNCH_TIMED((gemm_planes_pp<EPI, PLANES_OUT, MI, LN>), dim3(blocks), dim3(512), smem, s, g);
      return;
    }
  }
  WT_LAUNCH_TIMED((gemm_planes_tile<EPI, PLANES_OUT, WN, NI, MI, LN>), dim3(blocks), dim3(128 * WN), smem, s, g);
}

template <int EPI, bool PLANES_OUT>
bool launch_planes(const PlaneGemmDev& g, int n_cu, hipStream_t s) {
  static const int forced = [] {
    const char* v = getenv("WT_PLANE_TILE");
    return v ? atoi(v) : 0;
  }();
  const int cu = n_cu > 0 ? n_cu : 256;
  auto rounds = [&](long tiles) { return (tiles + cu - 1) / cu; };
  const long rt192 = (g.M + 191) / 192, rt256 = (g.M + 255) / 256;
  const bool can_wide = g.N % 384 == 0;
  const double c_wide = can_wide ? 192.0 * 3 * rounds(rt192 * (g.N / 384)) : 1e30;
  const double c_tall = can_wide ? 256.0 * 3 * 1.08 * rounds(rt256 * (g.N / 384)) : 1e30;
  const double c_narrow = 192.0 * 1.1 * rounds(rt192 * (g.N / 128));
  int pick = c_wide <= c_narrow ? (c_tall < c_wide ? 2 : 1) : (c_tall < c_narrow ? 2 : 0);
  if (forced == 128) pick = 0;
  if (forced == 384 && can_wide) pick = 1;
  if (forced == 256 && can_wide) pick = 2;
  if constexpr (!PLANES_OUT && (EPI == (kEpiBias | kEpiResidual) || EPI == (kEpiBias | kEpiGelu | kEpiPos))) {
    if (g.ln_P != nullptr && g.N == 384 && pick != 0) {
      if (pick == 2) {
        launch_planes_shape<EPI, false, 4, 3, 4, true>(g, s);
      } else {
        launch_planes_shape<EPI, false, 4, 3, 3, true>(g, s);
      }
      return true;
    }
  }
  if (pick == 2) {
    launch_planes_shape<EPI, PLANES_OUT, 4, 3, 4>(g, s);
  } else if (pick == 1) {
    launch_planes_shape<EPI, PLANES_OUT, 4, 3, 3>(g, s, n_cu);
  } else {
    launch_planes_shape<EPI, PLANES_OUT, 2, 2, 3>(g, s);
  }
  return false;
}

}

std::vector<unsigned short> split_weight_planes(const float* W, int N, int K, int Kpad, float scale) {
  if (N % 16 != 0 || Kpad % 32 != 0 || K > Kpad) throw Error(kErrInvalidArg, "split_weight_planes: N % 16, Kpad % 32");
  std::vector<unsigned short> out(size_t(2) * N * Kpad, 0);
  const int nkt = Kpad / 32;
  for (int n = 0; n < N; ++n) {
    const int rg = n / 16, r = n % 16;
    for (int k = 0; k < K; ++k) {
      const float v = W[size_t(n) * K + k] * scale;
      const _Float16 h = static_cast<_Float16>(v);
      const _Float16 l = static_cast<_Float16>(v - static_cast<float>(h));
      const int kt = k / 32, c = (k % 32) / 8, e = k % 8;
      const size_t blk = (size_t(rg) * nkt + kt) * 2 * 512;
      const size_t at = size_t(r * 4 + (c ^ chunk_swizzle(r))) * 8 + e;
      std::memcpy(out.data() + blk + at, &h, 2);
      std::memcpy(out.data() + blk + 512 + at, &l, 2);
    }
  }
  return out;
}

bool launch_gemm_planes(const PlaneGemmArgs& a, int epi, hipStream_t s) {
  PlaneGemmDev g{};
  g.A = reinterpret_cast<const _Float16*>(a.A); g.a_plane = a.a_plane;
  g.W = reinterpret_cast<const _Float16*>(a.W);
  g.C = a.C; g.P = reinterpret_cast<_Float16*>(a.P); g.p_plane = a.p_plane;
  g.bias = a.bias; g.R = a.R; g.pos = a.pos;
  g.M = a.M; g.N = a.N; g.K = a.K;
  g.a_rpb = a.a_rpb; g.a_bs = a.a_bs; g.lda = a.lda;
  g.c_rpb = a.c_rpb; g.c_bs = a.c_bs; g.ldc = a.ldc;
  g.pos_period = a.pos_period;
  g.kv_batch = a.kv_batch; g.kv_heads = a.kv_heads; g.kv_dmodel = a.kv_dmodel;
  g.descale = 1.0f / (a.a_scale * a.w_scale);
  g.out_scale[0] = a.out_scale[0]; g.out_scale[1] = a.out_scale[1]; g.out_scale[2] = a.out_scale[2];
  g.seg = a.seg > 0 ? a.seg : a.N;
  g.ln_g = a.ln_g; g.ln_b = a.ln_b; g.ln_P = reinterpret_cast<_Float16*>(a.ln_P); g.ln_plane = a.ln_plane;
  g.ln_scale = a.ln_scale; g.ln_y32 = a.ln_y32; g.nonfinite = a.nonfinite;
  if (a.ln_P && (!a.ln_g || !a.ln_b || a.P || a.c_rpb < a.M || a.ldc != a.N || !(a.ln_scale > 0.0f))) {
    throw Error(kErrInvalidArg, "plane GEMM LayerNorm fusion: needs gain and shift, fp32 output, contiguous [M][N] rows");
  }
  const bool planes = a.P != nullptr;
  if (a.N % 128 != 0 || a.K % BK != 0 || a.M < 1 || a.c_rpb < 32 || a.pos_period < (epi & kEpiPos ? 32 : 1) || a.lda % 8 != 0 ||
      a.a_bs % 8 != 0 || a.ldc % 8 != 0 || a.c_bs % 8 != 0 || (planes && (g.seg % 8 != 0 || (a.N + g.seg - 1) / g.seg > 3)) ||
      (!planes && !a.C) || !(a.a_scale > 0.0f) || !(a.w_scale > 0.0f)) {
    throw Error(kErrInvalidArg, "plane GEMM shape outside the kernel contract");
  }
  {
    const long a_span = a.a_plane + (long)((a.M - 1) / a.a_rpb) * a.a_bs + (long)std::min(a.a_rpb, a.M) * a.lda + a.K + 64;
    if (a.a_plane < 0 || a.a_bs < 0 || 2 * a_span >= (1L << 32)) {
      throw Error(kErrInvalidArg, "plane GEMM operand spans more than the 4 GiB its 32-bit offsets reach");
    }
  }
  switch (epi | (planes ? 256 : 0)) {
    case kEpiBias: return launch_planes<kEpiBias, false>(g, a.n_cu, s);
    case kEpiBias | kEpiGelu: return launch_planes<kEpiBias | kEpiGelu, false>(g, a.n_cu, s);
    case kEpiBias | kEpiResidual: return launch_planes<kEpiBias | kEpiResidual, false>(g, a.n_cu, s);
    case kEpiBias | kEpiGelu | kEpiPos: return launch_planes<kEpiBias | kEpiGelu | kEpiPos, false>(g, a.n_cu, s);
    case kEpiBias | kEpiKvLayout: return launch_planes<kEpiBias | kEpiKvLayout, false>(g, a.n_cu, s);
    case kEpiBias | kEpiPower: return launch_planes<kEpiBias | kEpiPower, false>(g, a.n_cu, s);
    case kEpiBias | 256: return launch_planes<kEpiBias, true>(g, a.n_cu, s);
    case kEpiBias | kEpiGelu | 256: return launch_planes<kEpiBias | kEpiGelu, true>(g, a.n_cu, s);
    default: throw Error(kErrInvalidArg, "unsupported plane GEMM epilogue combination");
  }
}

}
```

whisper.tflite_amd/csrc/k_misc.hip:

```cpp
#include <hip/hip_runtime.h>

#include <algorithm>

#include "bf16_split.h"
#include "kernels.h"

namespace wt {
namespace {

__device__ __forceinline__ float wave_sum(float v) {
#pragma unroll
  for (int off = 32; off >= 1; off >>= 1) v += __shfl_xor(v, off, 64);
  return v;
}

template <int PER>
__global__ __launch_bounds__(256) void layernorm_rows(const float* __restrict__ x,
                                                      float* __restrict__ y,
                                                      const float* __restrict__ g,
                                                      const float* __restrict__ b, int M, int d,
                                                      int* __restrict__ nonfinite) {
  const int lane = threadIdx.x & 63;
  const long row = (long)blockIdx.x * 4 + (threadIdx.x >> 6);
  if (row >= M) return;
  const float* xr = x + row * d;
  float v[PER];
  float s = 0.0f;
#pragma unroll
  for (int i = 0; i < PER; ++i) {
    const int c = lane + 64 * i;
    v[i] = c < d ? xr[c] : 0.0f;
    s += v[i];
  }
  const float mean = wave_sum(s) / (float)d;
  float q = 0.0f;
#pragma unroll
  for (int i = 0; i < PER; ++i) {
    const int c = lane + 64 * i;
    const float t = c < d ? v[i] - mean : 0.0f;
    q += t * t;
  }
  const float var = wave_sum(q) / (float)d;
  if (nonfinite != nullptr && lane == 0 && !(fabsf(mean) <= 3.0e38f && var <= 3.0e38f)) atomicOr(nonfinite, 1);
  const float rstd = rsqrtf(var + 1e-5f);
  float* yr = y + row * d;
#pragma unroll
  for (int i = 0; i < PER; ++i) {
    const int c = lane + 64 * i;
    if (c < d) yr[c] = (v[i] - mean) * rstd * g[c] + b[c];
  }
}

template <int PER, bool BF>
__global__ __launch_bounds__(256) void layernorm_rows_planes(const float* __restrict__ x, _Float16* __restrict__ yp,
                                                             long plane, float scale, float* __restrict__ y32,
                                                             const float* __restrict__ g, const float* __restrict__ b,
                                                             int M, int d, int* __restrict__ nonfinite) {
  using f32x4 = __attribute__((ext_vector_type(4))) float;
  using half4 = __attribute__((ext_vector_type(4))) _Float16;
  const int l32 = threadIdx.x & 31;
  const long row = (long)blockIdx.x * 8 + (threadIdx.x >> 5);
  if (row >= M) return;
  const float* xr = x + row * d;
  f32x4 v[PER], gg[PER], bb[PER];
  float s = 0.0f;
#pragma unroll
  for (int i = 0; i < PER; ++i) {
    const int c = (l32 + 32 * i) * 4;
    v[i] = *reinterpret_cast<const f32x4*>(xr + c);
    gg[i] = *reinterpret_cast<const f32x4*>(g + c);
    bb[i] = *reinterpret_cast<const f32x4*>(b + c);
    s += (v[i][0] + v[i][1]) + (v[i][2] + v[i][3]);
  }
#pragma unroll
  for (int off = 16; off >= 1; off >>= 1) s += __shfl_xor(s, off, 64);
  const float mean = s / (float)d;
  float q = 0.0f;
#pragma unroll
  for (int i = 0; i < PER; ++i)
#pragma unroll
    for (int e = 0; e < 4; ++e) {
      const float t = v[i][e] - mean;
      q += t * t;
    }
#pragma unroll
  for (int off = 16; off >= 1; off >>= 1) q += __shfl_xor(q, off, 64);
  const float var = q / (float)d;
  if (nonfinite != nullptr && l32 == 0 && !(fabsf(mean) <= 3.0e38f && var <= 3.0e38f)) atomicOr(nonfinite, 1);
  const float rstd = rsqrtf(var + 1e-5f);
#pragma unroll
  for (int i = 0; i < PER; ++i) {
    const int c = (l32 + 32 * i) * 4;
    f32x4 y;
    half4 hi, lo;
#pragma unroll
    for (int e = 0; e < 4; ++e) {
      y[e] = (v[i][e] - mean) * rstd * gg[i][e] + bb[i][e];
      if (!BF) {
        _Float16 h, l;
        split_f16(y[e] * scale, &h, &l);
        hi[e] = h;
        lo[e] = l;
      }
    }
    if (y32 != nullptr) __builtin_nontemporal_store(y, reinterpret_cast<f32x4*>(y32 + row * d + c));
    if (BF) {
      using u32x2 = __attribute__((ext_vector_type(2))) unsigned;
      *reinterpret_cast<u32x2*>(yp + row * d + c) = u32x2{pack_bf16x2(y[0], y[1]), pack_bf16x2(y[2], y[3])};
    } else {
      *reinterpret_cast<half4*>(yp + row * d + c) = hi;
      *reinterpret_cast<half4*>(yp + plane + row * d + c) = lo;
    }
  }
}

struct SegScales {
  float s[3];
};
__global__ __launch_bounds__(256) void f32_to_planes(const float* __restrict__ x, _Float16* __restrict__ yp, long plane,
                                                     SegScales sc, int seg, int ld, long n4) {
  using f32x4 = __attribute__((ext_vector_type(4))) float;
  using u32x2 = __attribute__((ext_vector_type(2))) unsigned;
  for (long i = (long)blockIdx.x * 256 + threadIdx.x; i < n4; i += (long)gridDim.x * 256) {
    const f32x4 v = *reinterpret_cast<const f32x4*>(x + 4 * i);
    const int col = (int)((4 * i) % ld);
    const float s = sc.s[col / seg];
    unsigned h0, l0, h1, l1;
    split_f16x2(v[0] * s, v[1] * s, &h0, &l0);
    split_f16x2(v[2] * s, v[3] * s, &h1, &l1);
    *reinterpret_cast<u32x2*>(yp + 4 * i) = u32x2{h0, h1};
    *reinterpret_cast<u32x2*>(yp + plane + 4 * i) = u32x2{l0, l1};
  }
}

__global__ __launch_bounds__(256) void pcm_to_planes(const float* __restrict__ x, _Float16* __restrict__ yp, long plane, float scale,
                                                     float limit, long n4_per_clip, long out_stride, long total4) {
  using f32x4 = __attribute__((ext_vector_type(4))) float;
  using u32x2 = __attribute__((ext_vector_type(2))) unsigned;
  for (long i = (long)blockIdx.x * 256 + threadIdx.x; i < total4; i += (long)gridDim.x * 256) {
    const long b = i / n4_per_clip, j = i - b * n4_per_clip;
    f32x4 v = *reinterpret_cast<const f32x4*>(x + 4 * i);
#pragma unroll
    for (int e = 0; e < 4; ++e) {
      const float c = fminf(fmaxf(v[e], -limit), limit);
      v[e] = (v[e] != v[e] ? v[e] : c) * scale;
    }
    unsigned h0, l0, h1, l1;
    split_f16x2(v[0], v[1], &h0, &l0);
    split_f16x2(v[2], v[3], &h1, &l1);
    const long o = b * out_stride + 4 * j;
    *reinterpret_cast<u32x2*>(yp + o) = u32x2{h0, h1};
    *reinterpret_cast<u32x2*>(yp + plane + o) = u32x2{l0, l1};
  }
}

template <bool BF>
__global__ __launch_bounds__(256) void mel_transpose_planes(const float* __restrict__ mel, _Float16* __restrict__ out,
                                                            long plane, float scale, int C, int T, int ld) {
  __shared__ float tile[32][33];
  const int b = blockIdx.z, t0 = blockIdx.x * 32, c0 = blockIdx.y * 32;
  const int tx = threadIdx.x & 31, ty = threadIdx.x >> 5;
  const float* src = mel + (long)b * C * T;
  _Float16* dst = out + (long)b * (T + 2) * ld;
#pragma unroll
  for (int i = 0; i < 4; ++i) {
    const int c = c0 + ty + 8 * i, t = t0 + tx;
    tile[ty + 8 * i][tx] = (c < C && t < T) ? src[(long)c * T + t] : 0.0f;
  }
  __syncthreads();
#pragma unroll
  for (int i = 0; i < 4; ++i) {
    const int t = t0 + ty + 8 * i, c = c0 + tx;
    if (c < C && t < T) {
      if (BF) {
        const unsigned pk = pack_bf16x2(tile[tx][ty + 8 * i], 0.0f);
        reinterpret_cast<unsigned short*>(dst)[(long)(t + 1) * ld + c] = (unsigned short)(pk & 0xFFFFu);
      } else {
        _Float16 h, l;
        split_f16(tile[tx][ty + 8 * i] * scale, &h, &l);
        dst[(long)(t + 1) * ld + c] = h;
        dst[plane + (long)(t + 1) * ld + c] = l;
      }
    }
  }
// ... 89 lines not shown
  for (long i = (long)blockIdx.x * 256 + threadIdx.x; i < per_clip; i += (long)gridDim.x * 256) {
    float v = p[i];
    if ((double)v < floor_v) v = (float)floor_v;
    p[i] = (float)(((double)v + 4.0) / 4.0);
  }
}

__global__ __launch_bounds__(256) void select_token(const unsigned long long* __restrict__ best,
                                                    int n_tiles, long long* ids, int ids_stride,
                                                    int pos, int* n_ids, int* finished, long long eot,
                                                    int stop_at_eot, int keep_ids) {
  __shared__ unsigned long long wmax[4];
  const int b = blockIdx.x;
  unsigned long long p = 0ull;
  for (int t = threadIdx.x; t < n_tiles; t += 256) {
    const unsigned long long v = best[(long)b * n_tiles + t];
    p = v > p ? v : p;
  }
#pragma unroll
  for (int off = 32; off >= 1; off >>= 1) {
    const unsigned long long o = __shfl_xor(p, off, 64);
    p = o > p ? o : p;
  }
  if ((threadIdx.x & 63) == 0) wmax[threadIdx.x >> 6] = p;
  __syncthreads();
  if (threadIdx.x != 0) return;
  for (int w = 1; w < 4; ++w) p = wmax[w] > p ? wmax[w] : p;
  const long long tok = (long long)(unsigned)(p & 0xffffffffull);
  if (!keep_ids) ids[(long)b * ids_stride + pos + 1] = tok;
  if (!finished[b]) {
    n_ids[b] = pos + 2;
    if (stop_at_eot && tok == eot) finished[b] = 1;
  }
}

}

void launch_layernorm(const float* x, float* y, const float* g, const float* b, int M, int d,
                      hipStream_t s, int* nonfinite) {
  const int blocks = (M + 3) / 4;
  if (d <= 128) {
    hipLaunchKernelGGL(layernorm_rows<2>, dim3(blocks), dim3(256), 0, s, x, y, g, b, M, d, nonfinite);
  } else if (d <= 384) {
    hipLaunchKernelGGL(layernorm_rows<6>, dim3(blocks), dim3(256), 0, s, x, y, g, b, M, d, nonfinite);
  } else if (d <= 512) {
    hipLaunchKernelGGL(layernorm_rows<8>, dim3(blocks), dim3(256), 0, s, x, y, g, b, M, d, nonfinite);
  } else {
    throw Error(kErrFormat, "LayerNorm kernel supports rows of at most 512 elements");
  }
}

template <bool BF>
static void launch_ln_planes(const float* x, _Float16* y, long plane, float scale, float* y32, const float* g, const float* b,
                             int M, int d, hipStream_t s, int* nonfinite) {
  const int blocks = (M + 7) / 8;
  if (d == 128) {
    hipLaunchKernelGGL((layernorm_rows_planes<1, BF>), dim3(blocks), dim3(256), 0, s, x, y, plane, scale, y32, g, b, M, d, nonfinite);
  } else if (d == 384) {
    hipLaunchKernelGGL((layernorm_rows_planes<3, BF>), dim3(blocks), dim3(256), 0, s, x, y, plane, scale, y32, g, b, M, d, nonfinite);
  } else if (d == 512) {
    hipLaunchKernelGGL((layernorm_rows_planes<4, BF>), dim3(blocks), dim3(256), 0, s, x, y, plane, scale, y32, g, b, M, d, nonfinite);
  } else {
    throw Error(kErrFormat, "LayerNorm plane kernel supports rows of 128, 384 or 512 elements");
  }
}

void launch_layernorm_planes(const float* x, unsigned short* yp, long plane, float scale, float* y32, const float* g,
                             const float* b, int M, int d, hipStream_t s, int* nonfinite, bool bf16) {
  _Float16* y = reinterpret_cast<_Float16*>(yp);
  if (bf16) {
    launch_ln_planes<true>(x, y, plane, scale, y32, g, b, M, d, s, nonfinite);
  } else {
    launch_ln_planes<false>(x, y, plane, scale, y32, g, b, M, d, s, nonfinite);
  }
}

void launch_f32_to_planes(const float* x, unsigned short* yp, long plane, long M, int ld, const float* scales, int seg,
                          hipStream_t s) {
  if (seg <= 0) seg = ld;
  if (M < 1 || ld % 4 != 0 || seg % 4 != 0 || (ld + seg - 1) / seg > 3) throw Error(kErrInvalidArg, "f32_to_planes: bad shape");
  SegScales sc{{scales[0], (ld + seg - 1) / seg > 1 ? scales[1] : 1.0f, (ld + seg - 1) / seg > 2 ? scales[2] : 1.0f}};
  const long n4 = M * ld / 4;
  const unsigned blocks = (unsigned)std::min<long>((n4 + 255) / 256, 256 * 32);
  hipLaunchKernelGGL(f32_to_planes, dim3(blocks), dim3(256), 0, s, x, reinterpret_cast<_Float16*>(yp), plane, sc, seg, ld, n4);
}

void launch_pcm_to_planes(const float* pcm, unsigned short* yp, long plane, float scale, float limit, int batch, long n,
                          long out_stride, hipStream_t s) {
  if (batch < 1 || n < 4 || n % 4 != 0 || out_stride % 8 != 0 || out_stride < n || !(scale > 0.0f) || !(limit > 0.0f)) {
    throw Error(kErrInvalidArg, "pcm_to_planes: bad shape");
  }
  const long total4 = (long)batch * (n / 4);
  const unsigned blocks = (unsigned)std::min<long>((total4 + 255) / 256, 256 * 32);
  hipLaunchKernelGGL(pcm_to_planes, dim3(blocks), dim3(256), 0, s, pcm, reinterpret_cast<_Float16*>(yp), plane, scale, limit, n / 4,
                     out_stride, total4);
}

void launch_mel_transpose_planes(const float* mel, unsigned short* out, long plane, float scale, int batch, int n_mels,
                                 int T, int ld, hipStream_t s, bool bf16) {
  const dim3 grid((T + 31) / 32, (n_mels + 31) / 32, batch);
  if (bf16) {
    hipLaunchKernelGGL(mel_transpose_planes<true>, grid, dim3(256), 0, s, mel, reinterpret_cast<_Float16*>(out), plane, scale,
                       n_mels, T, ld);
  } else {
    hipLaunchKernelGGL(mel_transpose_planes<false>, grid, dim3(256), 0, s, mel, reinterpret_cast<_Float16*>(out), plane, scale,
                       n_mels, T, ld);
  }
}

__global__ void chain_probe(float* p) {
  if (threadIdx.x == 0) p[blockIdx.x] += 1.0f;
}

void launch_chain_probe(float* p, int blocks, hipStream_t stream) {
  hipLaunchKernelGGL(chain_probe, dim3(blocks), dim3(64), 0, stream, p);
}

void launch_mel_transpose(const float* mel, float* melT, int batch, int n_mels, int T,
                          hipStream_t s) {
  hipLaunchKernelGGL(mel_transpose, dim3((T + 31) / 32, (n_mels + 31) / 32, batch), dim3(256), 0, s,
                     mel, melT, n_mels, T);
}

void launch_log_clipmax(const float* melacc, int ld, float* logmel, unsigned* clip_max, int batch,
                        int n_mel, int T, hipStream_t s, int t_valid) {
  hipLaunchKernelGGL(log_clipmax, dim3((T + 31) / 32, (n_mel + 31) / 32, batch), dim3(256), 0, s,
                     melacc, ld, logmel, clip_max, n_mel, T, t_valid < 0 ? T : t_valid);
}

void launch_mel_normalize(float* logmel, const unsigned* clip_max, int batch, int n_mel, int T,
                          hipStream_t s) {
  hipLaunchKernelGGL(mel_normalize, dim3(64, batch), dim3(256), 0, s, logmel, clip_max,
                     (long)n_mel * T);
}

void launch_select_token(const unsigned long long* best, int n_tiles, long long* ids, int ids_stride,
                         int pos, int* n_ids, int* finished, long long eot, int stop_at_eot, int batch,
// ... 20 lines not shown
```

whisper.tflite_amd/csrc/kernels.h:

```cpp
#pragma once
#include <hip/hip_runtime.h>
#include <hip/hip_ext.h>

#include <cstdint>
#include <vector>

#include "error.h"

namespace wt {

struct LaunchTimer {
  hipEvent_t start = nullptr, stop = nullptr;
};
extern thread_local LaunchTimer g_launch_timer;

#define WT_LAUNCH_TIMED(kernel, grid, block, smem, stream, ...)                                                      \
  do {                                                                                                                \
    if (::wt::g_launch_timer.start) {                                                                                 \
      hipExtLaunchKernelGGL(kernel, grid, block, smem, stream, ::wt::g_launch_timer.start, ::wt::g_launch_timer.stop, \
                            0, __VA_ARGS__);                                                                          \
    } else {                                                                                                          \
      hipLaunchKernelGGL(kernel, grid, block, smem, stream, __VA_ARGS__);                                             \
    }                                                                                                                 \
  } while (0)

enum GemmEpi : int {
  kEpiBias = 1,
  kEpiGelu = 2,
  kEpiResidual = 4,
  kEpiPos = 8,
  kEpiKvLayout = 16,
  kEpiPower = 32
};

struct GemmArgs {
  const float* A = nullptr;
  const float* W = nullptr;
  float* C = nullptr;
  const float* bias = nullptr;
  const float* R = nullptr;
  const float* pos = nullptr;
  int M = 0, N = 0, K = 0;
  int a_rpb = 1 << 30;
  long a_bs = 0;
  int lda = 0;
  int c_rpb = 1 << 30;
  long c_bs = 0;
  int ldc = 0;
  int pos_period = 1;
  int kv_batch = 0, kv_heads = 0, kv_dmodel = 0;
  int variant = -1;
  float a_scale = 1.0f, w_scale = 64.0f;
};
void launch_gemm(const GemmArgs& a, int epi, hipStream_t s);
float f16_scale_for(float bound);
int gemm_occupancy(int variant);
bool gemm_variant_supported(int variant);

struct PlaneGemmArgs {
  const unsigned short* A = nullptr;
  long a_plane = 0;
  const unsigned short* W = nullptr;
  float* C = nullptr;
  unsigned short* P = nullptr;
  long p_plane = 0;
  const float* bias = nullptr;
  const float* R = nullptr;
  const float* pos = nullptr;
  int M = 0, N = 0, K = 0;
  int a_rpb = 1 << 30;
  long a_bs = 0;
  int lda = 0;
  int c_rpb = 1 << 30;
  long c_bs = 0;
  int ldc = 0;
  int pos_period = 1;
  int kv_batch = 0, kv_heads = 0, kv_dmodel = 0;
  float a_scale = 1.0f, w_scale = 1.0f;
  float out_scale[3] = {1.0f, 1.0f, 1.0f};
  int seg = 0;
  int n_cu = 256;
  const float *ln_g = nullptr, *ln_b = nullptr;
  unsigned short* ln_P = nullptr;
  long ln_plane = 0;
  float ln_scale = 1.0f;
  float* ln_y32 = nullptr;
  int* nonfinite = nullptr;
};
bool launch_gemm_planes(const PlaneGemmArgs& a, int epi, hipStream_t s);
int plane_gemm_mode();
void set_plane_gemm_mode(int m);
bool launch_gemm_bf16_planes(const PlaneGemmArgs& a, int epi, hipStream_t s);
std::vector<unsigned short> round_weights_bf16(const float* W, int N, int K, int Kpad);
std::vector<unsigned short> split_weight_planes(const float* W, int N, int K, int Kpad, float scale);

enum DecPro : int {
  kProNone = 0,
  kProLn = 1,
  kProCombine = 2
};
enum DecEpi : int {
  kDecResid = 0,
  kDecBias = 1,
  kDecBiasGelu = 2,
  kDecLogits = 3
};
struct DecGemmArgs {
  int logits_blocks = 0;
  const unsigned short* Wt = nullptr;
  float w_scale = 1.0f;
  int N = 0, K = 0, B = 0;
  int M = 0;
  const float* X = nullptr;
  int ldx = 0;
  const float* xin = nullptr;
  float* xout = nullptr;
  const float* ln_g = nullptr;
  const float* ln_b = nullptr;
  const long long* ids = nullptr;
  int ids_stride = 0, pos = 0;
  const float* tok_emb = nullptr;
  const float* pos_emb = nullptr;
  int n_vocab = 0;
  const float* cross_ws = nullptr;
  int heads = 0, chunks = 0;
  const float* bias = nullptr;
  const float* R = nullptr;
  float* Y = nullptr;
  int ldy = 0;
  unsigned long long* best = nullptr;
  int best_stride = 0;
  int ksplit = 1;
  float* part = nullptr;
  const float* xpart = nullptr;
  bool bf16 = false;
};
void launch_dec_gemm(const DecGemmArgs& a, int pro, int epi, hipStream_t s);
void launch_dec_finalize_ln(const float* xin, const float* g, const float* b, float* y, int B, int K,
                            hipStream_t s, const float* xpart = nullptr);

void launch_layernorm(const float* x, float* y, const float* g, const float* b, int M, int d,
                      hipStream_t s, int* nonfinite = nullptr);
void launch_layernorm_planes(const float* x, unsigned short* yp, long plane, float scale, float* y32, const float* g,
                             const float* b, int M, int d, hipStream_t s, int* nonfinite = nullptr, bool bf16 = false);

void launch_spin(int microseconds, hipStream_t s);

void launch_f32_to_planes(const float* x, unsigned short* yp, long plane, long M, int ld, const float* scales, int seg,
                          hipStream_t s);
void launch_pcm_to_planes(const float* pcm, unsigned short* yp, long plane, float scale, float limit, int batch, long n,
                          long out_stride, hipStream_t s);

void launch_encoder_attention(const float* qkv, float* out, int batch, int T, int heads, int variant,
                              hipStream_t stream, float q_scale = 1.0f, float k_scale = 1.0f, float v_scale = 1.0f);
void launch_encoder_attention_planes(const unsigned short* qkv, long plane, unsigned short* out, long out_plane,
                                     int batch, int T, int heads, float q_scale, float k_scale, float v_scale,
                                     float out_scale, hipStream_t stream);
void launch_encoder_attention_bf16(const unsigned short* qkv, unsigned short* out, int batch, int T, int heads,
                                   hipStream_t stream);

void launch_chain_probe(float* p, int blocks, hipStream_t stream);
void launch_mel_transpose(const float* mel, float* melT, int batch, int n_mels, int T,
                          hipStream_t s);
void launch_mel_transpose_planes(const float* mel, unsigned short* out, long plane, float scale, int batch, int n_mels,
                                 int T, int ld, hipStream_t s, bool bf16 = false);
constexpr int kClipMaxStride = 32, kClipMaxWays = 4;
void launch_log_clipmax(const float* melacc, int ld, float* logmel, unsigned* clip_max, int batch,
                        int n_mel, int T, hipStream_t s, int t_valid = -1);
void launch_mel_normalize(float* logmel, const unsigned* clip_max, int batch, int n_mel, int T,
                          hipStream_t s);

void launch_self_attention(const float* qkv, void* kcache, void* vcache, int cap, int pos0, int npos, float* out,
                           int batch, int heads, hipStream_t s, bool bf16 = false);
struct CrossAttnArgs {
  const float* x = nullptr;
  const float *ln_g = nullptr, *ln_b = nullptr, *wq_t = nullptr, *bq = nullptr;
  const void *kc = nullptr, *vc = nullptr;
  float* ws = nullptr;
  int batch = 0, heads = 0, T = 0, chunks = 1, nq = 1;
  bool bf16 = false;
};
void launch_cross_attention(const CrossAttnArgs& a, hipStream_t s);
struct CrossAbsorbedArgs {
  const float* qp = nullptr;
  const unsigned short* e = nullptr;
  const unsigned short* e2 = nullptr;
  const unsigned short* e3 = nullptr;
  const unsigned short* e4 = nullptr;
  int split = 0;
  long e_plane = 0;
  float e_scale = 1.0f;
  float* ws = nullptr;
  int batch = 0, heads = 0, d_model = 0, T = 0, chunks = 1, nq = 1, p0 = 0;
  bool bf16 = false;
};
void launch_cross_absorbed(const CrossAbsorbedArgs& a, hipStream_t s);
int cross_absorbed_max_nq(int heads);
void launch_cross_absorbed_combine(const float* ws, const float* wv_t, const float* bv, float* out, int rows, int heads,
                                   int chunks, int d_model, hipStream_t s);
void launch_select_token(const unsigned long long* best, int n_tiles, long long* ids, int ids_stride,
                         int pos, int* n_ids, int* finished, long long eot, int stop_at_eot, int batch,
                         hipStream_t s, bool keep_ids = false);

constexpr int kBeamMax = 8;
constexpr int kBeamChunk = 4096;
constexpr int kBeamMaxChunks = 16;
constexpr int kBeamClipsMax = 64;
struct BeamPart {
  float m, s;
  unsigned long long key[kBeamMax + 1];
// ... 48 lines not shown
```

Measured before the change: 148,300 audio-sec/s.

## Interleave fp16 hi/lo planes in 32-element lines for encoder activations

Changes the storage of the two fp16 planes (hi and lo) for several encoder activation buffers from two separate planes to an interleaved layout, where each 32-element hi line is followed by its matching lo line. The writers (LayerNorm, conversion, conv GEMM epilogue, attention output) and the GEMM A-operand readers are updated to use this layout. The aim is to improve locality so that one contiguous fetch brings both planes, cutting separate memory streams and TLB/cache pressure. It adds offset arithmetic and requires row lengths that are multiples of 32, and it extends the debug API with pack/unpack helpers.

```diff
diff --git a/include/wt_debug.h b/include/wt_debug.h
--- a/include/wt_debug.h
+++ b/include/wt_debug.h
@@ -11,6 +11,9 @@
                        float* avg_ms, int n_cu );
 int wt_dbg_set_forced_ids(wt_engine* h, const int64_t* ids, int clips);
 int wt_dbg_set_plane_gemm_mode(int mode);
+int wt_dbg_set_plane_layout(int interleaved);
+int wt_dbg_planes_pack(const float* x, size_t n, float scale, int interleaved, uint16_t* out);
+int wt_dbg_planes_unpack(const uint16_t* planes, size_t n, float scale, int interleaved, float* out);
 int wt_dbg_gemm_planes_ln(wt_engine* h, int M, int K, const float* A, const float* W, const float* bias, const float* R,
                           const float* pos, int pos_period, int epi, const float* ln_g, const float* ln_b, int n_cu,
                           float* C, float* ln_out, float* ln_y32, int* fused);
diff --git a/whisper.tflite_amd/__init__.py b/whisper.tflite_amd/__init__.py
--- a/whisper.tflite_amd/__init__.py
+++ b/whisper.tflite_amd/__init__.py
@@ -33,7 +33,8 @@
 DEBUG_SYMBOLS = [
     "wt_dbg_cross_absorbed", "wt_dbg_cross_absorbed_bf16", "wt_dbg_gemm_planes_ln", "wt_dbg_gemm", "wt_dbg_gemm_bench", "wt_dbg_dec_gemm_bench", "wt_dbg_dec_gemm", "wt_dbg_dec_ln_gemm", "wt_dbg_layernorm", "wt_dbg_encoder_attention",
     "wt_dbg_cross_attention", "wt_dbg_self_attention", "wt_dbg_interference", "wt_dbg_concurrency",
-    "wt_dbg_gemm_planes", "wt_dbg_set_plane_gemm_mode", "wt_dbg_set_forced_ids", "wt_dbg_dec_gemm_bf16", "wt_dbg_dec_ln_gemm_bf16",
+    "wt_dbg_gemm_planes", "wt_dbg_set_plane_gemm_mode", "wt_dbg_set_plane_layout", "wt_dbg_planes_pack", "wt_dbg_planes_unpack",
+    "wt_dbg_set_forced_ids", "wt_dbg_dec_gemm_bf16", "wt_dbg_dec_ln_gemm_bf16",
     "wt_dbg_self_attention_bf16", "wt_dbg_cross_attention_bf16", "wt_dbg_encoder_attention_planes", "wt_dbg_gemm_bf16", "wt_dbg_gemm_bf16_ln", "wt_dbg_encoder_attention_bf16",
     "wt_dbg_beam_topk", "wt_dbg_beam_step", "wt_dbg_beam_reorder", "wt_dbg_beam_finalize",
     "wt_dbg_dec_gemm_ksplit", "wt_dbg_dec_ln_gemm_rows", "wt_dbg_dec_logits", "wt_dbg_select_token",
@@ -168,6 +169,10 @@
         L.wt_dbg_dec_logits.argtypes = [c_void_p, c_int, c_int, c_int, c_int, fp, fp, fp, fp, fp, c_int, fp, u64p]
         L.wt_dbg_select_token.argtypes = [c_void_p, c_int, c_int, u64p, ip64, c_int, c_int, ip32, ip32, c_int64, c_int,
                                           c_int]
+        L.wt_dbg_set_plane_layout.argtypes = [c_int]
+        u16p = POINTER(ctypes.c_uint16)
+        L.wt_dbg_planes_pack.argtypes = [fp, c_size_t, c_float, c_int, u16p]
+        L.wt_dbg_planes_unpack.argtypes = [u16p, c_size_t, c_float, c_int, fp]
         _lib = L
     return _lib
 
@@ -190,6 +195,32 @@
     if a.dtype != np.int64 or not a.flags.c_contiguous:
         raise ValueError("expected a contiguous int64 array")
     return a.ctypes.data_as(POINTER(c_int64))
+
+
+def set_plane_layout(interleaved: bool) -> None:
+    rc = lib().wt_dbg_set_plane_layout(int(bool(interleaved)))
+    if rc != WT_OK:
+        raise WtError(rc, "wt_dbg_set_plane_layout")
+
+
+def planes_pack(x, scale: float, interleaved: bool) -> np.ndarray:
+    x = _f32(x).ravel()
+    out = np.zeros(2 * x.size + 128, np.uint16)
+    rc = lib().wt_dbg_planes_pack(_fp(x), x.size, scale, int(bool(interleaved)), out.ctypes.data_as(POINTER(ctypes.c_uint16)))
+    if rc != WT_OK:
+        raise WtError(rc, "wt_dbg_planes_pack")
+    return out
+
+
+def planes_unpack(planes: np.ndarray, n: int, scale: float, interleaved: bool) -> np.ndarray:
+    planes = np.ascontiguousarray(planes, dtype=np.uint16)
+    if planes.size < 2 * n + 128:
+        raise ValueError("planes_unpack: buffer shorter than 2 n + 128")
+    out = np.zeros(n, np.float32)
+    rc = lib().wt_dbg_planes_unpack(planes.ctypes.data_as(POINTER(ctypes.c_uint16)), n, scale, int(bool(interleaved)), _fp(out))
+    if rc != WT_OK:
+        raise WtError(rc, "wt_dbg_planes_unpack")
+    return out
 
 
 def write_synthetic_weights(path: str, arch: str = "tiny", seed: int = 0) -> None:
diff --git a/whisper.tflite_amd/csrc/capi.cpp b/whisper.tflite_amd/csrc/capi.cpp
--- a/whisper.tflite_amd/csrc/capi.cpp
+++ b/whisper.tflite_amd/csrc/capi.cpp
@@ -816,31 +816,56 @@
 }
 
 namespace {
+bool g_dbg_planes_il = true;
+struct PlaneIndex {
+  size_t n, pad;
+  bool il;
+  size_t hi(size_t i) const { return il ? size_t(wt::il_offset(long(i))) : i; }
+  size_t lo(size_t i) const { return il ? hi(i) + 32 : n + pad + i; }
+};
+void pack_planes(const float* x, size_t n, float scale, bool il, size_t pad, unsigned short* host ) {
+  const PlaneIndex ix{n, pad, il};
+  for (size_t i = 0; x && i < n; ++i) {
+    const float v = x[i] * scale;
+    const _Float16 hi = static_cast<_Float16>(v), lo = static_cast<_Float16>(v - static_cast<float>(hi));
+    std::memcpy(&host[ix.hi(i)], &hi, 2);
+    std::memcpy(&host[ix.lo(i)], &lo, 2);
+  }
+}
+void unpack_planes(const unsigned short* host, size_t n, float scale, bool il, size_t pad, float* out) {
+  const PlaneIndex ix{n, pad, il};
+  for (size_t i = 0; i < n; ++i) {
+    _Float16 hi, lo;
+    std::memcpy(&hi, &host[ix.hi(i)], 2);
+    std::memcpy(&lo, &host[ix.lo(i)], 2);
+    out[i] = (static_cast<float>(hi) + static_cast<float>(lo)) / scale;
+  }
+}
 struct DevPlanes {
   void* p = nullptr;
   long plane = 0;
-  DevPlanes(const float* x, size_t n, float scale, size_t pad = 64) : plane(long(n + pad)) {
+  size_t n = 0, pad = 0;
+  bool il = false;
+  DevPlanes(const float* x, size_t n_, float scale, bool il_ = false, size_t pad_ = 64)
+      : plane(long(n_ + pad_)), n(n_), pad(pad_), il(il_) {
+    if (il && n % 32 != 0) throw wt::Error(wt::kErrInvalidArg, "interleaved planes: whole 32-element lines");
     std::vector<unsigned short> host(2 * (n + pad), 0);
-    for (size_t i = 0; x && i < n; ++i) {
-      const float v = x[i] * scale;
-      const _Float16 hi = static_cast<_Float16>(v), lo = static_cast<_Float16>(v - static_cast<float>(hi));
-      std::memcpy(&host[i], &hi, 2);
-      std::memcpy(&host[n + pad + i], &lo, 2);
-    }
+    pack_planes(x, n, scale, il, pad, host.data());
     hipchk(hipMalloc(&p, host.size() * 2), "hipMalloc");
     hipchk(hipMemcpy(p, host.data(), host.size() * 2, hipMemcpyHostToDevice), "H2D");
   }
   ~DevPlanes() { (void)hipFree(p); }
   unsigned short* ptr() const { return static_cast<unsigned short*>(p); }
-  void to_host(float* out, size_t n, float scale) const {
-    std::vector<unsigned short> host(size_t(2) * plane);
+  void to_host(float* out, size_t m, float scale) const {
+    std::vector<unsigned short> host(2 * (n + pad));
     hipchk(hipMemcpy(host.data(), p, host.size() * 2, hipMemcpyDeviceToHost), "D2H");
-    for (size_t i = 0; i < n; ++i) {
-      _Float16 hi, lo;
-      std::memcpy(&hi, &host[i], 2);
-      std::memcpy(&lo, &host[size_t(plane) + i], 2);
-      out[i] = (static_cast<float>(hi) + static_cast<float>(lo)) / scale;
-    }
+    for (size_t i = 0; i < pad; ++i) {
+      const size_t a = il ? 2 * n + i : n + i, b = il ? 2 * n + pad + i : 2 * n + pad + i;
+      if (host[a] != 0 || host[b] != 0) throw wt::Error(wt::kErrDevice, "a kernel wrote past the end of its output planes");
+    }
+    std::vector<float> all(n);
+    unpack_planes(host.data(), n, scale, il, pad, all.data());
+    std::copy(all.begin(), all.begin() + std::min(m, n), out);
   }
 };
 struct DevWeightPlanes {
@@ -866,17 +891,18 @@
   if (!h || !A || !W || !C || N % 128 || K % 32 || M < 1 || n_cu < 0) return WT_ERR_INVALID_ARG;
   return guarded(h, [&] {
     const float sa = wt::f16_scale_for(max_abs(A, size_t(M) * K)), sw = wt::f16_scale_for(max_abs(W, size_t(N) * K));
-    const DevPlanes dA(A, size_t(M) * K, sa);
+    const bool il = g_dbg_planes_il;
+    const DevPlanes dA(A, size_t(M) * K, sa, il);
     const DevWeightPlanes dW(W, N, K, sw);
     DevBuf dB(bias, N), dC(R ? R : nullptr, size_t(M) * N), dP(pos, pos ? size_t(pos_period) * N : 0);
     const float out_bound = max_abs(A, size_t(M) * K) * max_abs(W, size_t(N) * K) * float(K) + (bias ? max_abs(bias, N) : 0.0f);
     const float so = wt::f16_scale_for(out_bound);
-    DevPlanes dO(nullptr, size_t(M) * N, 1.0f);
+    DevPlanes dO(nullptr, size_t(M) * N, 1.0f, il);
     wt::PlaneGemmArgs g;
-    g.A = dA.ptr(); g.a_plane = dA.plane; g.lda = K; g.W = dW.ptr(); g.bias = dB.p;
+    g.A = dA.ptr(); g.a_plane = dA.plane; g.a_il = il; g.lda = K; g.W = dW.ptr(); g.bias = dB.p;
     g.C = dC.p; g.R = dC.p; g.ldc = N; g.pos = dP.p; g.pos_period = pos_period > 0 ? pos_period : 1;
     g.M = M; g.N = N; g.K = K; g.a_scale = sa; g.w_scale = sw; g.n_cu = n_cu;
-    if (planes_out) { g.P = dO.ptr(); g.p_plane = dO.plane; g.out_scale[0] = so; }
+    if (planes_out) { g.P = dO.ptr(); g.p_plane = dO.plane; g.p_il = il; g.out_scale[0] = so; }
     hipStream_t st = h->impl->stream();
     wt::launch_gemm_planes(g, epi, st);
     h->impl->sync();
@@ -914,6 +940,25 @@
   return WT_OK;
 }
 
+int wt_dbg_set_plane_layout(int interleaved) {
+  if (interleaved != 0 && interleaved != 1) return WT_ERR_INVALID_ARG;
+  g_dbg_planes_il = interleaved != 0;
+  return WT_OK;
+}
+
+int wt_dbg_planes_pack(const float* x, size_t n, float scale, int interleaved, uint16_t* out) {
+  if (!x || !out || (interleaved && n % 32 != 0) || !(scale > 0.0f)) return WT_ERR_INVALID_ARG;
+  std::fill(out, out + 2 * n + 128, uint16_t(0));
+  pack_planes(x, n, scale, interleaved != 0, 64, out);
+  return WT_OK;
+}
+
+int wt_dbg_planes_unpack(const uint16_t* planes, size_t n, float scale, int interleaved, float* out) {
+  if (!planes || !out || (interleaved && n % 32 != 0) || !(scale > 0.0f)) return WT_ERR_INVALID_ARG;
+  unpack_planes(planes, n, scale, interleaved != 0, 64, out);
+  return WT_OK;
+}
+
 int wt_dbg_gemm_planes_ln(wt_engine* h, int M, int K, const float* A, const float* W, const float* bias, const float* R,
                           const float* pos, int pos_period, int epi, const float* ln_g, const float* ln_b, int n_cu,
                           float* C, float* ln_out, float* ln_y32, int* fused) {
@@ -921,18 +966,19 @@
   if (!h || !A || !W || !C || !ln_g || !ln_b || !ln_out || !fused || K % 32 || M < 1 || n_cu < 0) return WT_ERR_INVALID_ARG;
   return guarded(h, [&] {
     const float sa = wt::f16_scale_for(max_abs(A, size_t(M) * K)), sw = wt::f16_scale_for(max_abs(W, size_t(N) * K));
-    const DevPlanes dA(A, size_t(M) * K, sa);
+    const bool il = g_dbg_planes_il;
+    const DevPlanes dA(A, size_t(M) * K, sa, il);
     const DevWeightPlanes dW(W, N, K, sw);
     DevBuf dB(bias, N), dC(R ? R : nullptr, size_t(M) * N), dP(pos, pos ? size_t(pos_period) * N : 0), dG(ln_g, N), dS(ln_b, N),
         dY(size_t(M) * N), dF(1);
     hipchk(hipMemset(dF.p, 0, 4), "memset");
     const float so = 64.0f;
-    DevPlanes dO(nullptr, size_t(M) * N, 1.0f);
+    DevPlanes dO(nullptr, size_t(M) * N, 1.0f, il);
     wt::PlaneGemmArgs g;
-    g.A = dA.ptr(); g.a_plane = dA.plane; g.lda = K; g.W = dW.ptr(); g.bias = dB.p;
+    g.A = dA.ptr(); g.a_plane = dA.plane; g.a_il = il; g.lda = K; g.W = dW.ptr(); g.bias = dB.p;
     g.C = dC.p; g.R = dC.p; g.ldc = N; g.pos = dP.p; g.pos_period = pos_period > 0 ? pos_period : 1;
     g.M = M; g.N = N; g.K = K; g.a_scale = sa; g.w_scale = sw; g.n_cu = n_cu;
-    g.ln_g = dG.p; g.ln_b = dS.p; g.ln_P = dO.ptr(); g.ln_plane = dO.plane; g.ln_scale = so;
+    g.ln_g = dG.p; g.ln_b = dS.p; g.ln_P = dO.ptr(); g.ln_plane = dO.plane; g.ln_il = il; g.ln_scale = so;
     g.ln_y32 = ln_y32 ? dY.p : nullptr; g.nonfinite = reinterpret_cast<int*>(dF.p);
     *fused = wt::launch_gemm_planes(g, epi, h->impl->stream()) ? 1 : 0;
     h->impl->sync();
@@ -965,9 +1011,9 @@
       for (size_t c = 0; c < 3 * d; ++c)
         scaled[r * 3 * d + c] = qkv[r * 3 * d + c] * (c < d ? kQ * sq : c < 2 * d ? sk : sv);
     const DevPlanes dQ(scaled.data(), scaled.size(), 1.0f);
-    DevPlanes dO(nullptr, rows * d, 1.0f);
+    DevPlanes dO(nullptr, rows * d, 1.0f, g_dbg_planes_il);
     hipStream_t st = h->impl->stream();
-    wt::launch_encoder_attention_planes(dQ.ptr(), dQ.plane, dO.ptr(), dO.plane, batch, T, heads, sq, sk, sv, so, st);
+    wt::launch_encoder_attention_planes(dQ.ptr(), dQ.plane, dO.ptr(), dO.plane, batch, T, heads, sq, sk, sv, so, st, dO.il);
     h->impl->sync();
     dO.to_host(out, rows * d, so);
     if (avg_ms && iters > 0) {
@@ -976,7 +1022,7 @@
       hipchk(hipEventCreate(&e1), "event");
       hipchk(hipEventRecord(e0, st), "record");
       for (int i = 0; i < iters; ++i)
-        wt::launch_encoder_attention_planes(dQ.ptr(), dQ.plane, dO.ptr(), dO.plane, batch, T, heads, sq, sk, sv, so, st);
+        wt::launch_encoder_attention_planes(dQ.ptr(), dQ.plane, dO.ptr(), dO.plane, batch, T, heads, sq, sk, sv, so, st, dO.il);
       hipchk(hipEventRecord(e1, st), "record");
       hipchk(hipEventSynchronize(e1), "sync");
       float ms = 0;
diff --git a/whisper.tflite_amd/csrc/engine.cpp b/whisper.tflite_amd/csrc/engine.cpp
--- a/whisper.tflite_amd/csrc/engine.cpp
+++ b/whisper.tflite_amd/csrc/engine.cpp
@@ -1107,8 +1107,8 @@
   unsigned short* const qkvp = reinterpret_cast<unsigned short*>(ws_.qkv);
   unsigned short* const attp = reinterpret_cast<unsigned short*>(ws_.att);
   unsigned short* const hidp = reinterpret_cast<unsigned short*>(ws_.hid);
-  const long melT_plane = Bw * (T0 + 2) * nm + 128, h1p_plane = Bw * (T0 + 2) * d + 128;
-  const long ln_plane = Bw * T * d, qkv_plane = Bw * T * 3 * d, hid_plane = Bw * T * 4 * d, cvt_plane = Bw * T * 4 * d;
+  const long melT_plane = Bw * (T0 + 2) * nm + 128;
+  const long qkv_plane = Bw * T * 3 * d, cvt_plane = Bw * T * 4 * d;
   const long e_plane = Bw * T * d;
   const bool absorb = absorb_for(batch);
   const int alt = alt_gemm_variant();
@@ -1124,7 +1124,7 @@
   static const bool no_ln_fuse = getenv("WT_NO_LN_FUSE") != nullptr;
   auto fuse_ln = [&](PlaneGemmArgs& g, const float* gain, const float* shift, float scale) {
     if (no_ln_fuse) return;
-    g.ln_g = gain; g.ln_b = shift; g.ln_P = lnp; g.ln_plane = ln_plane; g.ln_scale = scale;
+    g.ln_g = gain; g.ln_b = shift; g.ln_P = lnp; g.ln_il = true; g.ln_scale = scale;
   };
   auto alt_gemm = [&](GemmArgs& g, const GemmScale& sc, int epi, double flops) {
     g.variant = alt; g.a_scale = sc.a; g.w_scale = sc.w;
@@ -1132,9 +1132,10 @@
     launch_gemm(g, epi, stream_);
     kt_end();
   };
-  auto to_planes = [&](const float* src, unsigned short* dst, long plane, long rows, int ld, const float* scales, int seg) {
+  auto to_planes = [&](const float* src, unsigned short* dst, long plane, long rows, int ld, const float* scales, int seg,
+                       bool il) {
     kt_begin(kKcConvert, 0, 2.0 * rows * ld * 4);
-    launch_f32_to_planes(src, dst, plane, rows, ld, scales, seg, stream_);
+    launch_f32_to_planes(src, dst, plane, rows, ld, scales, seg, stream_, il);
     kt_end();
   };
 
@@ -1151,7 +1152,7 @@
     g.A = ws_.melTp; g.a_plane = melT_plane; g.a_rpb = T0; g.a_bs = long(T0 + 2) * nm; g.lda = nm;
     g.W = conv1_p_.w; g.bias = conv1_b;
     if (c2p) {
-      g.P = ws_.h1pp + d; g.p_plane = h1p_plane; g.out_scale[0] = sc_conv2_.a;
+      g.P = ws_.h1pp + il_offset(d); g.p_il = true; g.out_scale[0] = sc_conv2_.a;
     } else {
       g.C = ws_.h1p + d;
     }
@@ -1165,11 +1166,11 @@
     g.C = ws_.h1p + d; g.c_rpb = T0; g.c_bs = long(T0 + 2) * d; g.ldc = d;
     g.M = batch * T0; g.N = d; g.K = conv1_kpad;
     alt_gemm(g, sc_conv1_, kEpiBias | kEpiGelu, 2.0 * g.M * g.N * (3.0 * nm));
-    if (c2p) to_planes(ws_.h1p, ws_.h1pp, h1p_plane, long(batch) * (T0 + 2), d, &sc_conv2_.a, 0);
+    if (c2p) to_planes(ws_.h1p, ws_.h1pp, 0, long(batch) * (T0 + 2), d, &sc_conv2_.a, 0, true);
   }
   if (c2p) {
     PlaneGemmArgs g;
-    g.A = ws_.h1pp; g.a_plane = h1p_plane; g.a_rpb = T; g.a_bs = long(T0 + 2) * d; g.lda = 2 * d;
+    g.A = ws_.h1pp; g.a_il = true; g.a_rpb = T; g.a_bs = long(T0 + 2) * d; g.lda = 2 * d;
     g.W = conv2_p_.w; g.bias = conv2_b; g.pos = enc_pos; g.pos_period = T;
     g.C = ws_.x; g.ldc = d; g.M = M; g.N = d; g.K = 3 * d;
     if (gemm_on_planes(sc_layers_[0].qkv)) fuse_ln(g, enc_blocks_[0].attn_ln_g, enc_blocks_[0].attn_ln_b, sc_layers_[0].qkv.a);
@@ -1189,7 +1190,7 @@
     }
     kt_begin(kKcLayerNorm, 0, 2.0 * M * d * 4);
     if (planes) {
-      launch_layernorm_planes(ws_.x, lnp, ln_plane, scale, nullptr, g, b, M, d, stream_);
+      launch_layernorm_planes(ws_.x, lnp, 0, scale, nullptr, g, b, M, d, stream_, nullptr, false, true);
     } else {
       launch_layernorm(ws_.x, ws_.ln, g, b, M, d, stream_);
     }
@@ -1209,7 +1210,7 @@
     long qkv_src_plane = qkv_plane;
     if (qp) {
       PlaneGemmArgs q;
-      q.A = lnp; q.a_plane = ln_plane; q.lda = d; q.W = wp.qkv.w; q.bias = w.attn.bqkv;
+      q.A = lnp; q.a_il = true; q.lda = d; q.W = wp.qkv.w; q.bias = w.attn.bqkv;
       if (ap) {
         q.P = qkvp; q.p_plane = qkv_plane; q.seg = d;
         q.out_scale[0] = qkv_scales[0]; q.out_scale[1] = qkv_scales[1]; q.out_scale[2] = qkv_scales[2];
@@ -1224,29 +1225,28 @@
       q.M = M; q.N = 3 * d; q.K = d;
       alt_gemm(q, sc.qkv, kEpiBias, 2.0 * q.M * q.N * q.K);
       if (ap) {
-        to_planes(ws_.qkv, ws_.cvt, cvt_plane, M, 3 * d, qkv_scales, d);
+        to_planes(ws_.qkv, ws_.cvt, cvt_plane, M, 3 * d, qkv_scales, d, false);
         qkv_src = ws_.cvt; qkv_src_plane = cvt_plane;
       }
     }
     const unsigned short* att_src = attp;
-    long att_src_plane = ln_plane;
     if (ap) {
       kt_begin(kKcEncAttn, 4.0 * batch * c.n_audio_head * double(T) * T * 64, 0);
-      launch_encoder_attention_planes(qkv_src, qkv_src_plane, attp, ln_plane, batch, T, c.n_audio_head, sc.q, sc.k, sc.v,
-                                      sc.out.a, stream_);
+      launch_encoder_attention_planes(qkv_src, qkv_src_plane, attp, 0, batch, T, c.n_audio_head, sc.q, sc.k, sc.v,
+                                      sc.out.a, stream_, true);
       kt_end();
     } else {
       kt_begin(kKcEncAttnAlt, 4.0 * batch * c.n_audio_head * double(T) * T * 64, 0);
       launch_encoder_attention(ws_.qkv, ws_.att, batch, T, c.n_audio_head, attn_alt, stream_);
       kt_end();
       if (op) {
-        to_planes(ws_.att, ws_.cvt, cvt_plane, M, d, &sc.out.a, 0);
-        att_src = ws_.cvt; att_src_plane = cvt_plane;
+        to_planes(ws_.att, ws_.cvt, 0, M, d, &sc.out.a, 0, true);
+        att_src = ws_.cvt;
       }
     }
     if (op) {
       PlaneGemmArgs o;
-      o.A = att_src; o.a_plane = att_src_plane; o.lda = d; o.W = wp.out.w; o.bias = w.attn.bo;
+      o.A = att_src; o.a_il = true; o.lda = d; o.W = wp.out.w; o.bias = w.attn.bo;
       o.C = ws_.x; o.R = ws_.x; o.ldc = d; o.M = M; o.N = d; o.K = d;
       if (f1p) fuse_ln(o, w.mlp_ln_g, w.mlp_ln_b, sc.fc1.a);
       ln_done = plane_gemm(o, sc.out, kEpiBias | kEpiResidual, 2.0 * o.M * o.N * o.K);
@@ -1258,12 +1258,11 @@
     }
     layernorm_for(f1p, sc.fc1.a, w.mlp_ln_g, w.mlp_ln_b);
     const unsigned short* hid_src = hidp;
-    long hid_src_plane = hid_plane;
     if (f1p) {
       PlaneGemmArgs f1;
-      f1.A = lnp; f1.a_plane = ln_plane; f1.lda = d; f1.W = wp.fc1.w; f1.bias = w.b1;
+      f1.A = lnp; f1.a_il = true; f1.lda = d; f1.W = wp.fc1.w; f1.bias = w.b1;
       if (f2p) {
-        f1.P = hidp; f1.p_plane = hid_plane; f1.out_scale[0] = sc.fc2.a;
+        f1.P = hidp; f1.p_il = true; f1.out_scale[0] = sc.fc2.a;
       } else {
         f1.C = ws_.hid;
       }
@@ -1275,13 +1274,13 @@
       f1.M = M; f1.N = 4 * d; f1.K = d;
       alt_gemm(f1, sc.fc1, kEpiBias | kEpiGelu, 2.0 * f1.M * f1.N * f1.K);
       if (f2p) {
-        to_planes(ws_.hid, ws_.cvt, cvt_plane, M, 4 * d, &sc.fc2.a, 0);
-        hid_src = ws_.cvt; hid_src_plane = cvt_plane;
+        to_planes(ws_.hid, ws_.cvt, 0, M, 4 * d, &sc.fc2.a, 0, true);
+        hid_src = ws_.cvt;
       }
     }
     if (f2p) {
       PlaneGemmArgs f2;
-      f2.A = hid_src; f2.a_plane = hid_src_plane; f2.lda = 4 * d; f2.W = wp.fc2.w; f2.bias = w.b2;
+      f2.A = hid_src; f2.a_il = true; f2.lda = 4 * d; f2.W = wp.fc2.w; f2.bias = w.b2;
       f2.C = ws_.x; f2.R = ws_.x; f2.ldc = d; f2.M = M; f2.N = d; f2.K = 4 * d;
       if (l + 1 < c.n_audio_layer) {
         if (gemm_on_planes(sc_layers_[l + 1].qkv)) fuse_ln(f2, enc_blocks_[l + 1].attn_ln_g, enc_blocks_[l + 1].attn_ln_b, sc_layers_[l + 1].qkv.a);
@@ -1289,7 +1288,7 @@
         fuse_ln(f2, enc_ln_post_g, enc_ln_post_b, sc_cross_kv_.a);
         f2.ln_y32 = ws_.enc_out; f2.nonfinite = slot.d_flag;
         if (absorb && f2.ln_P) {
-          f2.ln_P = slot.e_planes; f2.ln_plane = e_plane;
+          f2.ln_P = slot.e_planes; f2.ln_plane = e_plane; f2.ln_il = false;
         }
         if (!f2.ln_P) f2.ln_y32 = nullptr, f2.nonfinite = nullptr;
       }
@@ -1307,8 +1306,8 @@
   } else {
     kt_begin(kKcLayerNorm, 0, 2.0 * M * d * 4);
     if (kp) {
-      launch_layernorm_planes(ws_.x, absorb ? slot.e_planes : lnp, absorb ? e_plane : ln_plane, sc_cross_kv_.a, ws_.enc_out,
-                              enc_ln_post_g, enc_ln_post_b, M, d, stream_, slot.d_flag);
+      launch_layernorm_planes(ws_.x, absorb ? slot.e_planes : lnp, absorb ? e_plane : 0, sc_cross_kv_.a, ws_.enc_out,
+                              enc_ln_post_g, enc_ln_post_b, M, d, stream_, slot.d_flag, false, !absorb);
     } else {
       launch_layernorm(ws_.x, ws_.enc_out, enc_ln_post_g, enc_ln_post_b, M, d, stream_, slot.d_flag);
     }
@@ -1321,7 +1320,7 @@
   } else if (kp) {
     PlaneGemmArgs g;
     need_cross_kv(slot);
-    g.A = lnp; g.a_plane = ln_plane; g.lda = d; g.W = cross_kv_p_.w; g.bias = cross_kv_b;
+    g.A = lnp; g.a_il = true; g.lda = d; g.W = cross_kv_p_.w; g.bias = cross_kv_b;
     g.C = slot.cross_kv; g.M = M; g.N = c.n_text_layer * 2 * d; g.K = d;
     g.c_rpb = T; g.kv_batch = batch; g.kv_heads = c.n_text_head; g.kv_dmodel = d;
     plane_gemm(g, sc_cross_kv_, kEpiBias | kEpiKvLayout, 2.0 * g.M * g.N * g.K);
diff --git a/whisper.tflite_amd/csrc/k_attention_planes.hip b/whisper.tflite_amd/csrc/k_attention_planes.hip
--- a/whisper.tflite_amd/csrc/k_attention_planes.hip
+++ b/whisper.tflite_amd/csrc/k_attention_planes.hip
@@ -25,7 +25,7 @@
 template <bool BF>
 __global__ __launch_bounds__(256, BF ? 4 : 3) void encoder_attention_planes(const _Float16* __restrict__ qkv, long plane,
                                                                      _Float16* __restrict__ out, long out_plane, int T,
-                                                                     int heads, float s_inv, float o_scale) {
+                                                                     int heads, float s_inv, float o_scale, long out_ilmask) {
   constexpr int NP = BF ? 1 : 2;
   extern __shared__ __attribute__((aligned(16))) unsigned char lds[];
   constexpr int kVOff = 2 * NP * kPlaneBytes;
@@ -258,7 +258,7 @@
     const int q_row = qb * 128 + wid * 32 + 16 * qa + c;
     if (q_row < T) {
       const float inv = o_scale / l;
-      _Float16* orow = out + ((long)b * T + q_row) * d_model + h * 64;
+      const long orow = ((long)b * T + q_row) * d_model + h * 64;
       using u32x2 = __attribute__((ext_vector_type(2))) unsigned;
 #pragma unroll
       for (int dg = 0; dg < 4; ++dg) {
@@ -271,8 +271,9 @@
             split_f16x2(o[dg][qa][2 * j] * inv, o[dg][qa][2 * j + 1] * inv, &ah[j], &al[j]);
           }
         }
-        *reinterpret_cast<u32x2*>(orow + 16 * dg + 4 * g) = u32x2{ah[0], ah[1]};
-        if constexpr (!BF) *reinterpret_cast<u32x2*>(orow + out_plane + 16 * dg + 4 * g) = u32x2{al[0], al[1]};
+        const long f = orow + 16 * dg + 4 * g, o = f + (f & out_ilmask);
+        *reinterpret_cast<u32x2*>(out + o) = u32x2{ah[0], ah[1]};
+        if constexpr (!BF) *reinterpret_cast<u32x2*>(out + out_plane + o) = u32x2{al[0], al[1]};
       }
     }
   }
@@ -282,12 +283,12 @@
 
 void launch_encoder_attention_planes(const unsigned short* qkv, long plane, unsigned short* out, long out_plane,
                                      int batch, int T, int heads, float q_scale, float k_scale, float v_scale,
-                                     float out_scale, hipStream_t stream) {
+                                     float out_scale, hipStream_t stream, bool out_il) {
   if (batch < 1 || T < 1 || heads < 1 || (3 * heads * 64) % 8 != 0) throw Error(kErrInvalidArg, "encoder attention: bad shape");
   const int q_blocks = (T + 127) / 128;
   WT_LAUNCH_TIMED(encoder_attention_planes<false>, dim3(batch * heads * q_blocks), dim3(256), 6 * kPlaneBytes, stream,
-                     reinterpret_cast<const _Float16*>(qkv), plane, reinterpret_cast<_Float16*>(out), out_plane, T, heads,
-                     1.0f / (q_scale * k_scale), out_scale / v_scale);
+                     reinterpret_cast<const _Float16*>(qkv), plane, reinterpret_cast<_Float16*>(out), out_il ? 32L : out_plane, T,
+                     heads, 1.0f / (q_scale * k_scale), out_scale / v_scale, out_il ? ~31L : 0L);
 }
 
 void launch_encoder_attention_bf16(const unsigned short* qkv, unsigned short* out, int batch, int T, int heads,
@@ -296,7 +297,7 @@
   const int q_blocks = (T + 127) / 128;
   WT_LAUNCH_TIMED(encoder_attention_planes<true>, dim3(batch * heads * q_blocks), dim3(256), 3 * kPlaneBytes, stream,
                      reinterpret_cast<const _Float16*>(qkv), 0L, reinterpret_cast<_Float16*>(out), 0L, T, heads,
-                     0.125f * 1.44269504088896340736f, 1.0f);
-}
-
-}
+                     0.125f * 1.44269504088896340736f, 1.0f, 0L);
+}
+
+}
diff --git a/whisper.tflite_amd/csrc/k_gemm_planes.hip b/whisper.tflite_amd/csrc/k_gemm_planes.hip
--- a/whisper.tflite_amd/csrc/k_gemm_planes.hip
+++ b/whisper.tflite_amd/csrc/k_gemm_planes.hip
@@ -37,6 +37,7 @@
   float* C;
   _Float16* P;
   long p_plane;
+  long p_ilmask;
   const float* bias;
   const float* R;
   const float* pos;
@@ -56,14 +57,16 @@
   const float* ln_b;
   _Float16* ln_P;
   long ln_plane;
+  long ln_ilmask;
   float ln_scale;
   float* ln_y32;
   int* nonfinite;
 };
 
 __host__ __device__ __forceinline__ constexpr int chunk_swizzle(int row) { return (0 - (row >> 2)) & 3; }
-
-template <int QA, int QW, int NW, int QPW>
+__host__ __device__ __forceinline__ constexpr int il_chunk_swizzle(int row) { return (row >> 1) & 7; }
+
+template <int QA, int QW, int NW, int QPW, bool AIL>
 __device__ __forceinline__ void setup_stage_dma(const PlaneGemmDev& g, int m0, int n0, int wid, int lane, unsigned (&voff)[QPW],
                                                 const unsigned char* (&ubase)[QPW], unsigned (&kstep)[QPW]) {
   const int srow = lane >> 2;
@@ -71,7 +74,15 @@
 #pragma unroll
   for (int j = 0; j < QPW; ++j) {
     const int q = wid + NW * j;
-    if (q < 2 * QA) {
+    if (AIL && q < 2 * QA) {
+      const int row = 8 * q + (lane >> 3);
+      const int chunk = (lane & 7) ^ il_chunk_swizzle(row);
+      int m = m0 + row;
+      m = m < g.M ? m : g.M - 1;
+      voff[j] = (unsigned)(2 * (2 * ((long)(m / g.a_rpb) * g.a_bs + (long)(m % g.a_rpb) * g.lda) + chunk * 8));
+      ubase[j] = reinterpret_cast<const unsigned char*>(g.A);
+      kstep[j] = 2 * BK * 2;
+    } else if (q < 2 * QA) {
       const bool lo = q >= QA;
       const int row = 16 * (lo ? q - QA : q) + srow;
       const int chunk = (lane & 3) ^ chunk_swizzle(row);
@@ -219,7 +230,7 @@
             }
           }
           if (PLANES_OUT) {
-            const long o = (long)mb * g.c_bs + (long)mt * g.ldc + n;
+            const long f = (long)mb * g.c_bs + (long)mt * g.ldc + n, o = f + (f & g.p_ilmask);
             u32x4 hi, lo;
 #pragma unroll
             for (int e = 0; e < CPL; e += 2) {
@@ -305,20 +316,20 @@
           f32x4 y;
 #pragma unroll
           for (int e = 0; e < 4; ++e) y[e] = (acc.get(mi, ni, 4 * p + e) - mean[mi][p]) * rstd[mi][p] * gg[e] + bb[e];
-          const long o = (long)m * BN + n;
+          const long o = (long)m * BN + n, op = o + (o & g.ln_ilmask);
           if (g.ln_y32 != nullptr) __builtin_nontemporal_store(y, reinterpret_cast<f32x4*>(g.ln_y32 + o));
           unsigned h0, l0, h1, l1;
           split_f16x2(y[0] * g.ln_scale, y[1] * g.ln_scale, &h0, &l0);
           split_f16x2(y[2] * g.ln_scale, y[3] * g.ln_scale, &h1, &l1);
           using u32x2 = __attribute__((ext_vector_type(2))) unsigned;
-          *reinterpret_cast<u32x2*>(g.ln_P + o) = u32x2{h0, h1};
-          *reinterpret_cast<u32x2*>(g.ln_P + g.ln_plane + o) = u32x2{l0, l1};
+          *reinterpret_cast<u32x2*>(g.ln_P + op) = u32x2{h0, h1};
+          *reinterpret_cast<u32x2*>(g.ln_P + g.ln_plane + op) = u32x2{l0, l1};
         }
     }
   }
 }
 
-template <int EPI, bool PLANES_OUT, int WN, int NI, int MI, bool LN = false>
+template <int EPI, bool PLANES_OUT, int WN, int NI, int MI, bool LN = false, bool AIL = false>
 __global__ __launch_bounds__(128 * WN, WN == 2 ? 2 : 2) void gemm_planes_tile(PlaneGemmDev g) {
   static_assert(!LN || (!PLANES_OUT && WN == 4 && NI == 3), "LayerNorm fusion: fp32 output, 384-column tile");
   constexpr int BN = WN * NI * 32, NW = 2 * WN, BM = 64 * MI;
@@ -344,7 +355,7 @@
   unsigned voff[QPW], kstep[QPW];
   const unsigned char* ubase[QPW];
   const unsigned lds_base = (unsigned)(size_t)(const __attribute__((address_space(3))) unsigned char*)smem;
-  setup_stage_dma<QA, QW, NW, QPW>(g, m0, n0, wid, lane, voff, ubase, kstep);
+  setup_stage_dma<QA, QW, NW, QPW, AIL>(g, m0, n0, wid, lane, voff, ubase, kstep);
   auto issue_stage = [&](int kt, int buf) {
 #pragma unroll
     for (int j = 0; j < QPW; ++j) {
@@ -358,18 +369,21 @@
   accs.zero();
   auto& acc = accs.t;
 
-  const int swz = chunk_swizzle(l31);
-  const int a_off = (wm * (32 * MI) + l31) * 64, b_off = 2 * kAPlane + (wn * NI * 32 + l31) * 64;
+  constexpr int kARow = AIL ? 128 : 64;
+  const int swz = chunk_swizzle(l31), swz8 = il_chunk_swizzle(l31);
+  const int a_off = (wm * (32 * MI) + l31) * kARow, b_off = 2 * kAPlane + (wn * NI * 32 + l31) * 64;
   auto compute = [&](int buf) {
     const unsigned char* base = smem + buf * kStage;
 #pragma unroll
     for (int ks = 0; ks < BK / 16; ++ks) {
       const int slot = ((ks * 2 + lh) ^ swz) * 16;
+      const int a_hi = AIL ? ((ks * 2 + lh) ^ swz8) * 16 : slot;
+      const int a_lo = AIL ? a_hi ^ 64 : kAPlane + slot;
       half8 ah[MI], al[MI], bh[NI], bl[NI];
 #pragma unroll
       for (int i = 0; i < MI; ++i) {
-        ah[i] = *reinterpret_cast<const half8*>(base + a_off + i * 32 * 64 + slot);
-        al[i] = *reinterpret_cast<const half8*>(base + kAPlane + a_off + i * 32 * 64 + slot);
+        ah[i] = *reinterpret_cast<const half8*>(base + a_off + i * 32 * kARow + a_hi);
+        al[i] = *reinterpret_cast<const half8*>(base + a_off + i * 32 * kARow + a_lo);
       }
 #pragma unroll
       for (int j = 0; j < NI; ++j) {
@@ -416,7 +430,7 @@
   } while (0)
 #endif
 
-template <int EPI, bool PLANES_OUT, int MI, bool LN = false>
+template <int EPI, bool PLANES_OUT, int MI, bool LN = false, bool AIL = false>
 __global__ __launch_bounds__(512, 2) void gemm_planes_pp(PlaneGemmDev g) {
   constexpr int WN = 4, NI = 3;
   static_assert(!LN || !PLANES_OUT, "LayerNorm fusion: fp32 output");
@@ -447,7 +461,7 @@
   unsigned voff[QPW], kstep[QPW];
   const unsigned char* ubase[QPW];
   const unsigned lds_base = (unsigned)(size_t)(const __attribute__((address_space(3))) unsigned char*)smem;
-  setup_stage_dma<QA, QW, NW, QPW>(g, m0, n0, wid, lane, voff, ubase, kstep);
+  setup_stage_dma<QA, QW, NW, QPW, AIL>(g, m0, n0, wid, lane, voff, ubase, kstep);
   auto issue_stage = [&](int kt, int buf) {
 #pragma unroll
     for (int j = 0; j < QPW; ++j) {
@@ -461,16 +475,19 @@
   accs.zero();
   auto& acc = accs.t;
 
-  const int swz = chunk_swizzle(l31);
-  const int a_off = (wm * (32 * MI) + l31) * 64, b_off = 2 * kAPlane + (wn * NI * 32 + l31) * 64;
+  constexpr int kARow = AIL ? 128 : 64;
+  const int swz = chunk_swizzle(l31), swz8 = il_chunk_swizzle(l31);
+  const int a_off = (wm * (32 * MI) + l31) * kARow, b_off = 2 * kAPlane + (wn * NI * 32 + l31) * 64;
   half8 ah[MI], al[MI], bh[NI], bl[NI];
   auto load_frags = [&](int buf, int ks) {
     const unsigned char* base = smem + buf * kStage;
     const int slot = ((ks * 2 + lh) ^ swz) * 16;
+    const int a_hi = AIL ? ((ks * 2 + lh) ^ swz8) * 16 : slot;
+    const int a_lo = AIL ? a_hi ^ 64 : kAPlane + slot;
 #pragma unroll
     for (int i = 0; i < MI; ++i) {
-      ah[i] = *reinterpret_cast<const half8*>(base + a_off + i * 32 * 64 + slot);
-      al[i] = *reinterpret_cast<const half8*>(base + kAPlane + a_off + i * 32 * 64 + slot);
+      ah[i] = *reinterpret_cast<const half8*>(base + a_off + i * 32 * kARow + a_hi);
+      al[i] = *reinterpret_cast<const half8*>(base + a_off + i * 32 * kARow + a_lo);
     }
 #pragma unroll
     for (int j = 0; j < NI; ++j) {
@@ -558,7 +575,7 @@
 #endif
 }
 
-template <int EPI, bool PLANES_OUT, bool LN = false>
+template <int EPI, bool PLANES_OUT, bool LN = false, bool AIL = false>
 __global__ __launch_bounds__(512, 2) void gemm_planes_pp16(PlaneGemmDev g) {
   constexpr int WN = 4, NI = 3, MI = 3;
   static_assert(!LN || !PLANES_OUT, "LayerNorm fusion: fp32 output");
@@ -588,7 +605,7 @@
   unsigned voff[QPW], kstep[QPW];
   const unsigned char* ubase[QPW];
   const unsigned lds_base = (unsigned)(size_t)(const __attribute__((address_space(3))) unsigned char*)smem;
-  setup_stage_dma<QA, QW, NW, QPW>(g, m0, n0, wid, lane, voff, ubase, kstep);
+  setup_stage_dma<QA, QW, NW, QPW, AIL>(g, m0, n0, wid, lane, voff, ubase, kstep);
   auto issue_stage = [&](int kt, int buf) {
 #pragma unroll
     for (int j = 0; j < QPW; ++j) {
@@ -604,7 +621,9 @@
 
   const int fc = lane & 15, fq = lane >> 4;
   const int frag = fc * 64 + ((fq ^ chunk_swizzle(fc)) * 16);
-  const int a_off = wm * (32 * MI) * 64 + frag, b_off = 2 * kAPlane + wn * (NI * 32) * 64 + frag;
+  constexpr int kARow = AIL ? 128 : 64;
+  const int a_hi = AIL ? fc * 128 + ((fq ^ il_chunk_swizzle(fc)) * 16) : frag, a_lo = AIL ? a_hi ^ 64 : frag + kAPlane;
+  const int a_off = wm * (32 * MI) * kARow, b_off = 2 * kAPlane + wn * (NI * 32) * 64 + frag;
   half8 ah[3], al[3], bh[6], bl[6];
   auto load_b = [&](int buf) {
     const unsigned char* base = smem + buf * kStage + b_off;
@@ -615,11 +634,11 @@
     }
   };
   auto load_a = [&](int buf, int half) {
-    const unsigned char* base = smem + buf * kStage + a_off + half * 3 * 1024;
+    const unsigned char* base = smem + buf * kStage + a_off + half * 3 * 16 * kARow;
 #pragma unroll
     for (int i = 0; i < 3; ++i) {
-      ah[i] = *reinterpret_cast<const half8*>(base + i * 1024);
-      al[i] = *reinterpret_cast<const half8*>(base + kAPlane + i * 1024);
+      ah[i] = *reinterpret_cast<const half8*>(base + a_hi + i * 16 * kARow);
+      al[i] = *reinterpret_cast<const half8*>(base + a_lo + i * 16 * kARow);
     }
   };
   auto compute = [&](auto half_c) {
@@ -707,7 +726,7 @@
 #endif
 }
 
-template <int EPI>
+template <int EPI, bool AIL = false>
 __global__ __launch_bounds__(512, 2) void gemm_planes_pp16_persist(PlaneGemmDev g, int total_tiles) {
   constexpr int WN = 4, NI = 3, MI = 3;
   constexpr bool PLANES_OUT = true;
@@ -736,7 +755,7 @@
     const int logical = (xcd < r8 ? xcd * (q8 + 1) : r8 * (q8 + 1) + (xcd - r8) * q8) + (vid >> 3);
     m0 = (logical / n_tiles) * BM;
     n0 = (logical % n_tiles) * BN;
-    setup_stage_dma<QA, QW, NW, QPW>(g, m0, n0, wid, lane, voff, ubase, kstep);
+    setup_stage_dma<QA, QW, NW, QPW, AIL>(g, m0, n0, wid, lane, voff, ubase, kstep);
   };
   auto issue_stage = [&](int kt) {
     const int buf = (kt + 1) & 1;
@@ -751,7 +770,9 @@
   auto& acc = accs.t;
   const int fc = lane & 15, fq = lane >> 4;
   const int frag = fc * 64 + ((fq ^ chunk_swizzle(fc)) * 16);
-  const int a_off = wm * (32 * MI) * 64 + frag, b_off = 2 * kAPlane + wn * (NI * 32) * 64 + frag;
+  constexpr int kARow = AIL ? 128 : 64;
+  const int a_hi = AIL ? fc * 128 + ((fq ^ il_chunk_swizzle(fc)) * 16) : frag, a_lo = AIL ? a_hi ^ 64 : frag + kAPlane;
+  const int a_off = wm * (32 * MI) * kARow, b_off = 2 * kAPlane + wn * (NI * 32) * 64 + frag;
   half8 ah[3], al[3], bh[6], bl[6];
   auto load_b = [&](int kt) {
     const unsigned char* base = smem + ((kt + 1) & 1) * kStage + b_off;
@@ -762,11 +783,11 @@
     }
   };
   auto load_a = [&](int kt, int half) {
-    const unsigned char* base = smem + ((kt + 1) & 1) * kStage + a_off + half * 3 * 1024;
+    const unsigned char* base = smem + ((kt + 1) & 1) * kStage + a_off + half * 3 * 16 * kARow;
 #pragma unroll
     for (int i = 0; i < 3; ++i) {
-      ah[i] = *reinterpret_cast<const half8*>(base + i * 1024);
-      al[i] = *reinterpret_cast<const half8*>(base + kAPlane + i * 1024);
+      ah[i] = *reinterpret_cast<const half8*>(base + a_hi + i * 16 * kARow);
+      al[i] = *reinterpret_cast<const half8*>(base + a_lo + i * 16 * kARow);
     }
   };
   auto compute = [&](auto half_c) {
@@ -850,13 +871,13 @@
   }
 }
 
-template <int EPI, bool PLANES_OUT, int WN, int NI, int MI = 3, bool LN = false>
+template <int EPI, bool PLANES_OUT, int WN, int NI, int MI, bool LN, bool AIL>
 void launch_planes_shape(const PlaneGemmDev& g, hipStream_t s, int n_cu = 0) {
   constexpr int BN = WN * NI * 32, BM = 64 * MI;
   const int blocks = ((g.M + BM - 1) / BM) * (g.N / BN);
   constexpr size_t smem = 2 * (2 * BM * BK * 2 + 2 * BN * BK * 2);
   static const bool raised = [] {
-    (void)hipFuncSetAttribute(reinterpret_cast<const void*>(&gemm_planes_tile<EPI, PLANES_OUT, WN, NI, MI, LN>),
+    (void)hipFuncSetAttribute(reinterpret_cast<const void*>(&gemm_planes_tile<EPI, PLANES_OUT, WN, NI, MI, LN, AIL>),
                               hipFuncAttributeMaxDynamicSharedMemorySize, 160 * 1024);
     return true;
   }();
@@ -866,40 +887,40 @@
       const int cu = n_cu > 0 ? n_cu : 256;
       if (plane_gemm_mode() == 2 && cu % 8 == 0 && blocks >= 2 * cu && (g.K / BK) % 2 == 0 && g.K / BK >= 4) {
         static const bool raised_p = [] {
-          (void)hipFuncSetAttribute(reinterpret_cast<const void*>(&gemm_planes_pp16_persist<EPI>), hipFuncAttributeMaxDynamicSharedMemorySize,
+          (void)hipFuncSetAttribute(reinterpret_cast<const void*>(&gemm_planes_pp16_persist<EPI, AIL>), hipFuncAttributeMaxDynamicSharedMemorySize,
                                     160 * 1024);
           return true;
         }();
         (void)raised_p;
-        WT_LAUNCH_TIMED((gemm_planes_pp16_persist<EPI>), dim3(cu), dim3(512), smem, s, g, blocks);
+        WT_LAUNCH_TIMED((gemm_planes_pp16_persist<EPI, AIL>), dim3(cu), dim3(512), smem, s, g, blocks);
         return;
       }
     }
     if (plane_gemm_mode() == 2 || plane_gemm_mode() == 4) {
       static const bool raised_pp16 = [] {
-        (void)hipFuncSetAttribute(reinterpret_cast<const void*>(&gemm_planes_pp16<EPI, PLANES_OUT, LN>),
+        (void)hipFuncSetAttribute(reinterpret_cast<const void*>(&gemm_planes_pp16<EPI, PLANES_OUT, LN, AIL>),
                                   hipFuncAttributeMaxDynamicSharedMemorySize, 160 * 1024);
         return true;
       }();
       (void)raised_pp16;
-      WT_LAUNCH_TIMED((gemm_planes_pp16<EPI, PLANES_OUT, LN>), dim3(blocks), dim3(512), smem, s, g);
+      WT_LAUNCH_TIMED((gemm_planes_pp16<EPI, PLANES_OUT, LN, AIL>), dim3(blocks), dim3(512), smem, s, g);
       return;
     }
     if (plane_gemm_mode() == 1) {
       static const bool raised_pp = [] {
-        (void)hipFuncSetAttribute(reinterpret_cast<const void*>(&gemm_planes_pp<EPI, PLANES_OUT, MI, LN>),
+        (void)hipFuncSetAttribute(reinterpret_cast<const void*>(&gemm_planes_pp<EPI, PLANES_OUT, MI, LN, AIL>),
                                   hipFuncAttributeMaxDynamicSharedMemorySize, 160 * 1024);
         return true;
       }();
       (void)raised_pp;
-      WT_LAUNCH_TIMED((gemm_planes_pp<EPI, PLANES_OUT, MI, LN>), dim3(blocks), dim3(512), smem, s, g);
+      WT_LAUNCH_TIMED((gemm_planes_pp<EPI, PLANES_OUT, MI, LN, AIL>), dim3(blocks), dim3(512), smem, s, g);
       return;
     }
   }
-  WT_LAUNCH_TIMED((gemm_planes_tile<EPI, PLANES_OUT, WN, NI, MI, LN>), dim3(blocks), dim3(128 * WN), smem, s, g);
-}
-
-template <int EPI, bool PLANES_OUT>
+  WT_LAUNCH_TIMED((gemm_planes_tile<EPI, PLANES_OUT, WN, NI, MI, LN, AIL>), dim3(blocks), dim3(128 * WN), smem, s, g);
+}
+
+template <int EPI, bool PLANES_OUT, bool AIL>
 bool launch_planes(const PlaneGemmDev& g, int n_cu, hipStream_t s) {
   static const int forced = [] {
     const char* v = getenv("WT_PLANE_TILE");
@@ -919,19 +940,19 @@
   if constexpr (!PLANES_OUT && (EPI == (kEpiBias | kEpiResidual) || EPI == (kEpiBias | kEpiGelu | kEpiPos))) {
     if (g.ln_P != nullptr && g.N == 384 && pick != 0) {
       if (pick == 2) {
-        launch_planes_shape<EPI, false, 4, 3, 4, true>(g, s);
+        launch_planes_shape<EPI, false, 4, 3, 4, true, AIL>(g, s);
       } else {
-        launch_planes_shape<EPI, false, 4, 3, 3, true>(g, s);
+        launch_planes_shape<EPI, false, 4, 3, 3, true, AIL>(g, s);
       }
       return true;
     }
   }
   if (pick == 2) {
-    launch_planes_shape<EPI, PLANES_OUT, 4, 3, 4>(g, s);
+    launch_planes_shape<EPI, PLANES_OUT, 4, 3, 4, false, AIL>(g, s);
   } else if (pick == 1) {
-    launch_planes_shape<EPI, PLANES_OUT, 4, 3, 3>(g, s, n_cu);
+    launch_planes_shape<EPI, PLANES_OUT, 4, 3, 3, false, AIL>(g, s, n_cu);
   } else {
-    launch_planes_shape<EPI, PLANES_OUT, 2, 2, 3>(g, s);
+    launch_planes_shape<EPI, PLANES_OUT, 2, 2, 3, false, AIL>(g, s);
   }
   return false;
 }
@@ -962,7 +983,7 @@
   PlaneGemmDev g{};
   g.A = reinterpret_cast<const _Float16*>(a.A); g.a_plane = a.a_plane;
   g.W = reinterpret_cast<const _Float16*>(a.W);
-  g.C = a.C; g.P = reinterpret_cast<_Float16*>(a.P); g.p_plane = a.p_plane;
+  g.C = a.C; g.P = reinterpret_cast<_Float16*>(a.P); g.p_plane = a.p_il ? 32 : a.p_plane; g.p_ilmask = a.p_il ? ~31L : 0L;
   g.bias = a.bias; g.R = a.R; g.pos = a.pos;
   g.M = a.M; g.N = a.N; g.K = a.K;
   g.a_rpb = a.a_rpb; g.a_bs = a.a_bs; g.lda = a.lda;
@@ -972,7 +993,8 @@
   g.descale = 1.0f / (a.a_scale * a.w_scale);
   g.out_scale[0] = a.out_scale[0]; g.out_scale[1] = a.out_scale[1]; g.out_scale[2] = a.out_scale[2];
   g.seg = a.seg > 0 ? a.seg : a.N;
-  g.ln_g = a.ln_g; g.ln_b = a.ln_b; g.ln_P = reinterpret_cast<_Float16*>(a.ln_P); g.ln_plane = a.ln_plane;
+  g.ln_g = a.ln_g; g.ln_b = a.ln_b; g.ln_P = reinterpret_cast<_Float16*>(a.ln_P);
+  g.ln_plane = a.ln_il ? 32 : a.ln_plane; g.ln_ilmask = a.ln_il ? ~31L : 0L;
   g.ln_scale = a.ln_scale; g.ln_y32 = a.ln_y32; g.nonfinite = a.nonfinite;
   if (a.ln_P && (!a.ln_g || !a.ln_b || a.P || a.c_rpb < a.M || a.ldc != a.N || !(a.ln_scale > 0.0f))) {
     throw Error(kErrInvalidArg, "plane GEMM LayerNorm fusion: needs gain and shift, fp32 output, contiguous [M][N] rows");
@@ -983,23 +1005,35 @@
       (!planes && !a.C) || !(a.a_scale > 0.0f) || !(a.w_scale > 0.0f)) {
     throw Error(kErrInvalidArg, "plane GEMM shape outside the kernel contract");
   }
+  if ((a.a_il && (a.lda % 32 != 0 || a.a_bs % 32 != 0)) || (a.p_il && planes && (a.ldc % 32 != 0 || a.c_bs % 32 != 0)) ||
+      (a.ln_il && a.ln_P && a.N % 32 != 0) || (a.a_il && epi == (kEpiBias | kEpiPower))) {
+    throw Error(kErrInvalidArg, "plane GEMM: interleaved planes need rows of whole 32-element lines");
+  }
   {
-    const long a_span = a.a_plane + (long)((a.M - 1) / a.a_rpb) * a.a_bs + (long)std::min(a.a_rpb, a.M) * a.lda + a.K + 64;
-    if (a.a_plane < 0 || a.a_bs < 0 || 2 * a_span >= (1L << 32)) {
+    const long rows = (long)((a.M - 1) / a.a_rpb) * a.a_bs + (long)std::min(a.a_rpb, a.M) * a.lda;
+    const long a_span = a.a_il ? 2 * (rows + a.K) + 64 : a.a_plane + rows + a.K + 64;
+    if ((!a.a_il && a.a_plane < 0) || a.a_bs < 0 || 2 * a_span >= (1L << 32)) {
       throw Error(kErrInvalidArg, "plane GEMM operand spans more than the 4 GiB its 32-bit offsets reach");
     }
   }
-  switch (epi | (planes ? 256 : 0)) {
-    case kEpiBias: return launch_planes<kEpiBias, false>(g, a.n_cu, s);
-    case kEpiBias | kEpiGelu: return launch_planes<kEpiBias | kEpiGelu, false>(g, a.n_cu, s);
-    case kEpiBias | kEpiResidual: return launch_planes<kEpiBias | kEpiResidual, false>(g, a.n_cu, s);
-    case kEpiBias | kEpiGelu | kEpiPos: return launch_planes<kEpiBias | kEpiGelu | kEpiPos, false>(g, a.n_cu, s);
-    case kEpiBias | kEpiKvLayout: return launch_planes<kEpiBias | kEpiKvLayout, false>(g, a.n_cu, s);
-    case kEpiBias | kEpiPower: return launch_planes<kEpiBias | kEpiPower, false>(g, a.n_cu, s);
-    case kEpiBias | 256: return launch_planes<kEpiBias, true>(g, a.n_cu, s);
-    case kEpiBias | kEpiGelu | 256: return launch_planes<kEpiBias | kEpiGelu, true>(g, a.n_cu, s);
-    default: throw Error(kErrInvalidArg, "unsupported plane GEMM epilogue combination");
-  }
-}
-
-}
+  auto run = [&](auto ail) -> bool {
+    constexpr bool AIL = decltype(ail)::value;
+    switch (epi | (planes ? 256 : 0)) {
+      case kEpiBias: return launch_planes<kEpiBias, false, AIL>(g, a.n_cu, s);
+      case kEpiBias | kEpiGelu: return launch_planes<kEpiBias | kEpiGelu, false, AIL>(g, a.n_cu, s);
+      case kEpiBias | kEpiResidual: return launch_planes<kEpiBias | kEpiResidual, false, AIL>(g, a.n_cu, s);
+      case kEpiBias | kEpiGelu | kEpiPos: return launch_planes<kEpiBias | kEpiGelu | kEpiPos, false, AIL>(g, a.n_cu, s);
+      case kEpiBias | kEpiKvLayout: return launch_planes<kEpiBias | kEpiKvLayout, false, AIL>(g, a.n_cu, s);
+      case kEpiBias | 256: return launch_planes<kEpiBias, true, AIL>(g, a.n_cu, s);
+      case kEpiBias | kEpiGelu | 256: return launch_planes<kEpiBias | kEpiGelu, true, AIL>(g, a.n_cu, s);
+      default: break;
+    }
+    if constexpr (!AIL) {
+      if (epi == (kEpiBias | kEpiPower) && !planes) return launch_planes<kEpiBias | kEpiPower, false, false>(g, a.n_cu, s);
+    }
+    throw Error(kErrInvalidArg, "unsupported plane GEMM epilogue combination");
+  };
+  return a.a_il ? run(std::true_type{}) : run(std::false_type{});
+}
+
+}
diff --git a/whisper.tflite_amd/csrc/k_misc.hip b/whisper.tflite_amd/csrc/k_misc.hip
--- a/whisper.tflite_amd/csrc/k_misc.hip
+++ b/whisper.tflite_amd/csrc/k_misc.hip
@@ -55,7 +55,7 @@
 __global__ __launch_bounds__(256) void layernorm_rows_planes(const float* __restrict__ x, _Float16* __restrict__ yp,
                                                              long plane, float scale, float* __restrict__ y32,
                                                              const float* __restrict__ g, const float* __restrict__ b,
-                                                             int M, int d, int* __restrict__ nonfinite) {
+                                                             int M, int d, int* __restrict__ nonfinite, long ilmask) {
   using f32x4 = __attribute__((ext_vector_type(4))) float;
   using half4 = __attribute__((ext_vector_type(4))) _Float16;
   const int l32 = threadIdx.x & 31;
@@ -108,8 +108,9 @@
       using u32x2 = __attribute__((ext_vector_type(2))) unsigned;
       *reinterpret_cast<u32x2*>(yp + row * d + c) = u32x2{pack_bf16x2(y[0], y[1]), pack_bf16x2(y[2], y[3])};
     } else {
-      *reinterpret_cast<half4*>(yp + row * d + c) = hi;
-      *reinterpret_cast<half4*>(yp + plane + row * d + c) = lo;
+      const long o = row * d + c + ((row * d + c) & ilmask);
+      *reinterpret_cast<half4*>(yp + o) = hi;
+      *reinterpret_cast<half4*>(yp + plane + o) = lo;
     }
   }
 }
@@ -118,7 +119,7 @@
   float s[3];
 };
 __global__ __launch_bounds__(256) void f32_to_planes(const float* __restrict__ x, _Float16* __restrict__ yp, long plane,
-                                                     SegScales sc, int seg, int ld, long n4) {
+                                                     SegScales sc, int seg, int ld, long n4, long ilmask) {
   using f32x4 = __attribute__((ext_vector_type(4))) float;
   using u32x2 = __attribute__((ext_vector_type(2))) unsigned;
   for (long i = (long)blockIdx.x * 256 + threadIdx.x; i < n4; i += (long)gridDim.x * 256) {
@@ -128,8 +129,9 @@
     unsigned h0, l0, h1, l1;
     split_f16x2(v[0] * s, v[1] * s, &h0, &l0);
     split_f16x2(v[2] * s, v[3] * s, &h1, &l1);
-    *reinterpret_cast<u32x2*>(yp + 4 * i) = u32x2{h0, h1};
-    *reinterpret_cast<u32x2*>(yp + plane + 4 * i) = u32x2{l0, l1};
+    const long o = 4 * i + ((4 * i) & ilmask);
+    *reinterpret_cast<u32x2*>(yp + o) = u32x2{h0, h1};
+    *reinterpret_cast<u32x2*>(yp + plane + o) = u32x2{l0, l1};
   }
 }
 
@@ -325,37 +327,41 @@
 
 template <bool BF>
 static void launch_ln_planes(const float* x, _Float16* y, long plane, float scale, float* y32, const float* g, const float* b,
-                             int M, int d, hipStream_t s, int* nonfinite) {
+                             int M, int d, hipStream_t s, int* nonfinite, long ilmask) {
   const int blocks = (M + 7) / 8;
   if (d == 128) {
-    hipLaunchKernelGGL((layernorm_rows_planes<1, BF>), dim3(blocks), dim3(256), 0, s, x, y, plane, scale, y32, g, b, M, d, nonfinite);
+    hipLaunchKernelGGL((layernorm_rows_planes<1, BF>), dim3(blocks), dim3(256), 0, s, x, y, plane, scale, y32, g, b, M, d, nonfinite, ilmask);
   } else if (d == 384) {
-    hipLaunchKernelGGL((layernorm_rows_planes<3, BF>), dim3(blocks), dim3(256), 0, s, x, y, plane, scale, y32, g, b, M, d, nonfinite);
+    hipLaunchKernelGGL((layernorm_rows_planes<3, BF>), dim3(blocks), dim3(256), 0, s, x, y, plane, scale, y32, g, b, M, d, nonfinite, ilmask);
   } else if (d == 512) {
-    hipLaunchKernelGGL((layernorm_rows_planes<4, BF>), dim3(blocks), dim3(256), 0, s, x, y, plane, scale, y32, g, b, M, d, nonfinite);
+    hipLaunchKernelGGL((layernorm_rows_planes<4, BF>), dim3(blocks), dim3(256), 0, s, x, y, plane, scale, y32, g, b, M, d, nonfinite, ilmask);
   } else {
     throw Error(kErrFormat, "LayerNorm plane kernel supports rows of 128, 384 or 512 elements");
   }
 }
 
 void launch_layernorm_planes(const float* x, unsigned short* yp, long plane, float scale, float* y32, const float* g,
-                             const float* b, int M, int d, hipStream_t s, int* nonfinite, bool bf16) {
+                             const float* b, int M, int d, hipStream_t s, int* nonfinite, bool bf16, bool il) {
   _Float16* y = reinterpret_cast<_Float16*>(yp);
   if (bf16) {
-    launch_ln_planes<true>(x, y, plane, scale, y32, g, b, M, d, s, nonfinite);
+    if (il) throw Error(kErrInvalidArg, "LayerNorm planes: the bf16 form has one plane");
+    launch_ln_planes<true>(x, y, plane, scale, y32, g, b, M, d, s, nonfinite, 0);
   } else {
-    launch_ln_planes<false>(x, y, plane, scale, y32, g, b, M, d, s, nonfinite);
+    launch_ln_planes<false>(x, y, il ? 32 : plane, scale, y32, g, b, M, d, s, nonfinite, il ? ~31L : 0L);
   }
 }
 
 void launch_f32_to_planes(const float* x, unsigned short* yp, long plane, long M, int ld, const float* scales, int seg,
-                          hipStream_t s) {
+                          hipStream_t s, bool il) {
   if (seg <= 0) seg = ld;
-  if (M < 1 || ld % 4 != 0 || seg % 4 != 0 || (ld + seg - 1) / seg > 3) throw Error(kErrInvalidArg, "f32_to_planes: bad shape");
+  if (M < 1 || ld % 4 != 0 || seg % 4 != 0 || (ld + seg - 1) / seg > 3 || (il && ld % 32 != 0)) {
+    throw Error(kErrInvalidArg, "f32_to_planes: bad shape");
+  }
   SegScales sc{{scales[0], (ld + seg - 1) / seg > 1 ? scales[1] : 1.0f, (ld + seg - 1) / seg > 2 ? scales[2] : 1.0f}};
   const long n4 = M * ld / 4;
   const unsigned blocks = (unsigned)std::min<long>((n4 + 255) / 256, 256 * 32);
-  hipLaunchKernelGGL(f32_to_planes, dim3(blocks), dim3(256), 0, s, x, reinterpret_cast<_Float16*>(yp), plane, sc, seg, ld, n4);
+  hipLaunchKernelGGL(f32_to_planes, dim3(blocks), dim3(256), 0, s, x, reinterpret_cast<_Float16*>(yp), il ? 32L : plane, sc, seg, ld, n4,
+                     il ? ~31L : 0L);
 }
 
 void launch_pcm_to_planes(const float* pcm, unsigned short* yp, long plane, float scale, float limit, int batch, long n,
diff --git a/whisper.tflite_amd/csrc/kernels.h b/whisper.tflite_amd/csrc/kernels.h
--- a/whisper.tflite_amd/csrc/kernels.h
+++ b/whisper.tflite_amd/csrc/kernels.h
@@ -57,13 +57,17 @@
 int gemm_occupancy(int variant);
 bool gemm_variant_supported(int variant);
 
+__host__ __device__ constexpr long il_offset(long f) { return f + (f & ~31L); }
+
 struct PlaneGemmArgs {
   const unsigned short* A = nullptr;
   long a_plane = 0;
+  bool a_il = false;
   const unsigned short* W = nullptr;
   float* C = nullptr;
   unsigned short* P = nullptr;
   long p_plane = 0;
+  bool p_il = false;
   const float* bias = nullptr;
   const float* R = nullptr;
   const float* pos = nullptr;
@@ -83,6 +87,7 @@
   const float *ln_g = nullptr, *ln_b = nullptr;
   unsigned short* ln_P = nullptr;
   long ln_plane = 0;
+  bool ln_il = false;
   float ln_scale = 1.0f;
   float* ln_y32 = nullptr;
   int* nonfinite = nullptr;
@@ -142,12 +147,13 @@
 void launch_layernorm(const float* x, float* y, const float* g, const float* b, int M, int d,
                       hipStream_t s, int* nonfinite = nullptr);
 void launch_layernorm_planes(const float* x, unsigned short* yp, long plane, float scale, float* y32, const float* g,
-                             const float* b, int M, int d, hipStream_t s, int* nonfinite = nullptr, bool bf16 = false);
+                             const float* b, int M, int d, hipStream_t s, int* nonfinite = nullptr, bool bf16 = false,
+                             bool il = false);
 
 void launch_spin(int microseconds, hipStream_t s);
 
 void launch_f32_to_planes(const float* x, unsigned short* yp, long plane, long M, int ld, const float* scales, int seg,
-                          hipStream_t s);
+                          hipStream_t s, bool il = false);
 void launch_pcm_to_planes(const float* pcm, unsigned short* yp, long plane, float scale, float limit, int batch, long n,
                           long out_stride, hipStream_t s);
 
@@ -155,7 +161,7 @@
                               hipStream_t stream, float q_scale = 1.0f, float k_scale = 1.0f, float v_scale = 1.0f);
 void launch_encoder_attention_planes(const unsigned short* qkv, long plane, unsigned short* out, long out_plane,
                                      int batch, int T, int heads, float q_scale, float k_scale, float v_scale,
-                                     float out_scale, hipStream_t stream);
+                                     float out_scale, hipStream_t stream, bool out_il = false);
 void launch_encoder_attention_bf16(const unsigned short* qkv, unsigned short* out, int batch, int T, int heads,
                                    hipStream_t stream);
 
```

Result: faster. 149,900 audio-sec/s, median of 6 (+1.1%).
